# jopohl/urh

Measured on NVIDIA H100. Metric: MSamples/s IQ demod+digitize (complex64), higher is better.
Workload: dtype f32

## Files before the change

### urh_b200/csrc/center.cu

```cuda
#include "dense.cuh"
#include "tilescan.cuh"

#include <math.h>
#include <stdlib.h>

int urh_window_var_bitwise(urh_ctx* ctx, const float* d_x, int64_t n, const int64_t* d_prefix, int64_t t0, int64_t t1, int64_t r0,
                           int64_t r1, float* h_out2);

struct CenStats {
    double sum, sumsq;
    float mn, mx;
    long long cnt;
};

__global__ void __launch_bounds__(URH_WARPS_PER_BLOCK * 32)
k_tile_stats_f32(const float* __restrict__ x, int64_t n, int64_t ntiles, UrhTileStats* __restrict__ ts) {
    const int lane = threadIdx.x & 31;
    const int64_t tile = (int64_t)blockIdx.x * URH_WARPS_PER_BLOCK + (threadIdx.x >> 5);
    if (tile >= ntiles) return;
    const int64_t base = tile * URH_TILE;
    UrhStatAcc acc;
    acc.init();
    acc.all_noise = false;
    if (base + URH_TILE <= n && (((uintptr_t)x) & 15) == 0) {
        const float4* p = (const float4*)(x + base) + lane;
        constexpr int ITERS = URH_TILE / 128;
        float4 cur[4], nxt[4];
#pragma unroll
        for (int j = 0; j < 4; j++) cur[j] = __ldg(p + j * 32);
        for (int it = 0; it < ITERS; it += 4) {
            if (it + 4 < ITERS) {
#pragma unroll
                for (int j = 0; j < 4; j++) nxt[j] = __ldg(p + (it + 4 + j) * 32);
            }
#pragma unroll
            for (int j = 0; j < 4; j++) {
                acc.add(cur[j].x); acc.add(cur[j].y); acc.add(cur[j].z); acc.add(cur[j].w);
            }
#pragma unroll
            for (int j = 0; j < 4; j++) cur[j] = nxt[j];
        }
    } else {
        for (int j = lane; j < URH_TILE; j += 32)
            if (base + j < n) acc.add(x[base + j]);
    }
    acc.store(ts + tile, lane);
}

struct ScanKept {
    const UrhTileStats* ts;
    int64_t* prefix;
    __device__ __forceinline__ int64_t load(int64_t t) const { return ts[t].cnt; }
    __device__ __forceinline__ void post(int64_t t, const int64_t& excl, const int64_t&) const { prefix[t] = excl; }
};
struct CenAddI64 {
    __device__ __forceinline__ int64_t operator()(int64_t a, int64_t b) const { return a + b; }
};

static int kept_prefix(urh_ctx* ctx, const UrhTileStats* ts, int64_t ntiles, int64_t* prefix) {
    ScanKept fk;
    fk.ts = ts; fk.prefix = prefix;
    return urhts::scan<int64_t, CenAddI64, ScanKept>(ctx, ntiles, (int64_t)0, CenAddI64(), fk, prefix + ntiles);
}

__global__ void k_find_window_tiles(const int64_t* __restrict__ prefix, int64_t ntiles, int64_t r0, int64_t r1, int64_t* __restrict__ win) {
    const int64_t t = (int64_t)blockIdx.x * blockDim.x + threadIdx.x;
    if (t >= ntiles) return;
    const int64_t a = prefix[t], b = prefix[t + 1];
    if (b <= a) return;
    const bool covered = a >= r0 && b <= r1;
    const bool has_r0 = a <= r0 && r0 < b, has_r1 = a <= r1 - 1 && r1 - 1 < b;
    if (has_r0) { win[0] = t; win[2] = covered ? -1 : t; }
    if (has_r1) { win[1] = t; win[3] = (covered || has_r0) ? -1 : t; }
}

#define CEN_PER (URH_TILE / 256)
__device__ __forceinline__ int64_t cen_tile_ranks(const float* __restrict__ x, int64_t n, int64_t t, int64_t tile_rank0, float (&v)[CEN_PER],
                                                  int* s_pre) {
    const int64_t base = t * URH_TILE + (int64_t)threadIdx.x * CEN_PER;
    int mine = 0;
#pragma unroll
    for (int j = 0; j < CEN_PER; j++) {
        v[j] = (base + j < n) ? x[base + j] : -5.0f;
        mine += (v[j] > -4.0f) ? 1 : 0;
    }
    s_pre[threadIdx.x] = mine;
    __syncthreads();
    for (int off = 1; off < 256; off <<= 1) {
        int add = 0;
        if (threadIdx.x >= off) add = s_pre[threadIdx.x - off];
        __syncthreads();
        s_pre[threadIdx.x] += add;
        __syncthreads();
    }
    return tile_rank0 + s_pre[threadIdx.x] - mine;
}

__device__ __forceinline__ void cen_block_fold(double sum, double sq, float mn, float mx, long long cnt, CenStats* out) {
    __shared__ double s_sum[256], s_sq[256];
    __shared__ float s_mn[256], s_mx[256];
    __shared__ long long s_cnt[256];
    __syncthreads();
    s_sum[threadIdx.x] = sum; s_sq[threadIdx.x] = sq; s_mn[threadIdx.x] = mn; s_mx[threadIdx.x] = mx; s_cnt[threadIdx.x] = cnt;
    __syncthreads();
    for (int off = 128; off > 0; off >>= 1) {
        if (threadIdx.x < off) {
            s_sum[threadIdx.x] += s_sum[threadIdx.x + off];
            s_sq[threadIdx.x] += s_sq[threadIdx.x + off];
            s_mn[threadIdx.x] = fminf(s_mn[threadIdx.x], s_mn[threadIdx.x + off]);
            s_mx[threadIdx.x] = fmaxf(s_mx[threadIdx.x], s_mx[threadIdx.x + off]);
            s_cnt[threadIdx.x] += s_cnt[threadIdx.x + off];
        }
        __syncthreads();
    }
    if (threadIdx.x == 0) {
        CenStats r;
        r.sum = s_sum[0]; r.sumsq = s_sq[0]; r.mn = s_mn[0]; r.mx = s_mx[0]; r.cnt = s_cnt[0];
        *out = r;
    }
}

__global__ void __launch_bounds__(256) k_cut_tile_stats(const float* __restrict__ x, int64_t n, const int64_t* __restrict__ prefix,
                                                       const int64_t* __restrict__ win, int64_t r0, int64_t r1, CenStats* __restrict__ out) {
    __shared__ int s_pre[256];
    const int64_t t = win[2 + blockIdx.x];
    double sum = 0.0, sq = 0.0;
    float mn = INFINITY, mx = -INFINITY;
    long long cnt = 0;
    if (t >= 0) {
        float v[CEN_PER];
        int64_t rank = cen_tile_ranks(x, n, t, prefix[t], v, s_pre);
#pragma unroll
        for (int j = 0; j < CEN_PER; j++) {
            if (v[j] > -4.0f) {
                if (rank >= r0 && rank < r1) {
                    sum += (double)v[j];
                    sq += (double)v[j] * (double)v[j];
                    mn = fminf(mn, v[j]);
                    mx = fmaxf(mx, v[j]);
                    cnt++;
                }
                rank++;
            }
        }
    }
    cen_block_fold(sum, sq, mn, mx, cnt, out + blockIdx.x);
}

__global__ void __launch_bounds__(256) k_interior_tile_stats(const UrhTileStats* __restrict__ ts, const int64_t* __restrict__ prefix,
                                                            int64_t ntiles, int64_t r0, int64_t r1, CenStats* __restrict__ partial) {
    double sum = 0.0, sq = 0.0;
    float mn = INFINITY, mx = -INFINITY;
    long long cnt = 0;
    for (int64_t t = (int64_t)blockIdx.x * 256 + threadIdx.x; t < ntiles; t += (int64_t)gridDim.x * 256) {
        const int64_t a = prefix[t], b = prefix[t + 1];
        if (b > a && a >= r0 && b <= r1) {
            const UrhTileStats v = ts[t];
            sum += v.sum; sq += v.sumsq; mn = fminf(mn, v.mn); mx = fmaxf(mx, v.mx); cnt += v.cnt;
        }
    }
    cen_block_fold(sum, sq, mn, mx, cnt, partial + blockIdx.x);
}

__global__ void __launch_bounds__(256) k_center_fold(const CenStats* __restrict__ partial, int64_t count, CenStats* __restrict__ out) {
    double sum = 0.0, sq = 0.0;
    float mn = INFINITY, mx = -INFINITY;
    long long cnt = 0;
    for (int64_t t = threadIdx.x; t < count; t += 256) {
        const CenStats p = partial[t];
        sum += p.sum; sq += p.sumsq; mn = fminf(mn, p.mn); mx = fmaxf(mx, p.mx); cnt += p.cnt;
    }
    cen_block_fold(sum, sq, mn, mx, cnt, out);
}

int urh_center_tiles_begin(urh_ctx* ctx, const float* d_x, const UrhTileStats* ts, int64_t n, int64_t* h_total) {
    const int64_t ntiles = urh_div_up(n, URH_TILE);
    int64_t* prefix;
    URH_CHECK(urh_arena(ctx, (size_t)ntiles + 1, &prefix));
    URH_CHECK(kept_prefix(ctx, ts, ntiles, prefix));
    URH_CHECK(urh_read_i64(ctx, prefix + ntiles, 1, h_total));
    ctx->center_prefix = prefix;
    ctx->center_ts = ts;
    ctx->center_n = n;
    ctx->center_x = d_x;
    return URH_OK;
}

static int tiles_from_array(urh_ctx* ctx, const float* d_x, int64_t n, int64_t* h_total) {
    urh_arena_reset(ctx);
    ctx->center_prefix = nullptr;
    const int64_t ntiles = urh_div_up(n, URH_TILE);
    UrhTileStats* ts;
    URH_CHECK(urh_arena(ctx, (size_t)ntiles, &ts));
    URH_LAUNCH(ctx, k_tile_stats_f32, (unsigned)urh_div_up(ntiles, URH_WARPS_PER_BLOCK), URH_WARPS_PER_BLOCK * 32, 0, d_x, n, ntiles, ts);
    return urh_center_tiles_begin(ctx, d_x, ts, n, h_total);
}

static bool tiles_match(const urh_ctx* ctx, const float* d_x, int64_t n) {
    return ctx->center_prefix && ctx->center_n == n && ctx->center_x == (const void*)d_x;
}

extern "C" int urh_center_window_stats(urh_ctx* ctx, const float* d_qad, int64_t n, int64_t r0, int64_t r1, double* h_out5) {
    h_out5[0] = 0.0; h_out5[1] = INFINITY; h_out5[2] = -INFINITY; h_out5[3] = 0.0; h_out5[4] = 0.0;
    if (!tiles_match(ctx, d_qad, n)) URH_FAIL(ctx, URH_ERR_INVALID, "urh_afp_demod_tiles (same qad, same n) must precede urh_center_window_stats");
    if (r1 <= r0) return URH_OK;
    const int64_t ntiles = urh_div_up(n, URH_TILE);
    const int64_t* prefix = (const int64_t*)ctx->center_prefix;
    const UrhTileStats* ts = (const UrhTileStats*)ctx->center_ts;
    int64_t* d_win;
    CenStats* partial;
    CenStats* folded;
    const int nb = ctx->sm_count * 2;
    URH_CHECK(urh_arena(ctx, 4, &d_win));
    URH_CHECK(urh_arena(ctx, (size_t)nb + 4, &partial));
    URH_CHECK(urh_arena(ctx, 2, &folded));
    URH_CUDA(ctx, cudaMemsetAsync(d_win, 0xff, 4 * sizeof(int64_t), ctx->stream));
    URH_LAUNCH(ctx, k_find_window_tiles, (unsigned)urh_div_up(ntiles, 256), 256, 0, prefix, ntiles, r0, r1, d_win);
    URH_LAUNCH(ctx, k_interior_tile_stats, nb, 256, 0, ts, prefix, ntiles, r0, r1, partial);
    URH_LAUNCH(ctx, k_cut_tile_stats, 2, 256, 0, d_qad, n, prefix, d_win, r0, r1, partial + nb);
    URH_LAUNCH(ctx, k_center_fold, 1, 256, 0, partial, (int64_t)nb + 2, folded);
    CenStats st;
    URH_CUDA(ctx, cudaMemcpyAsync(ctx->h_mail, folded, sizeof(CenStats), cudaMemcpyDeviceToHost, ctx->stream));
    URH_CUDA(ctx, cudaStreamSynchronize(ctx->stream));
    memcpy(&st, ctx->h_mail, sizeof(st));
    h_out5[0] = (double)st.cnt; h_out5[1] = (double)st.mn; h_out5[2] = (double)st.mx; h_out5[3] = st.sum; h_out5[4] = st.sumsq;
    return URH_OK;
}

extern "C" int urh_center_window_var(urh_ctx* ctx, const float* d_qad, int64_t n, int64_t r0, int64_t r1, double* h_out2) {
    h_out2[0] = h_out2[1] = 0.0;
    if (!tiles_match(ctx, d_qad, n)) URH_FAIL(ctx, URH_ERR_INVALID, "the tile table of this array must precede urh_center_window_var");
    if (r1 <= r0) return URH_OK;
    float mv[2];
    URH_CHECK(urh_window_var_bitwise(ctx, d_qad, n, (const int64_t*)ctx->center_prefix, 0, urh_div_up(n, URH_TILE) - 1, r0, r1, mv));
    h_out2[0] = (double)mv[0];
    h_out2[1] = (double)mv[1];
    return URH_OK;
}

extern "C" int urh_center_stats(urh_ctx* ctx, const float* d_x, int64_t n, int64_t max_size, double* h_out) {
    for (int i = 0; i < 7; i++) h_out[i] = 0.0;
    if (n <= 0) return URH_OK;
    int64_t total = 0;
    URH_CHECK(tiles_from_array(ctx, d_x, n, &total));
    int64_t r0 = (int64_t)(0.05 * (double)total), r1 = (int64_t)(0.95 * (double)total);
    if (max_size >= 0 && r1 - r0 > max_size) r1 = r0 + max_size;
    h_out[0] = (double)total; h_out[1] = (double)r0; h_out[2] = (double)r1;
    if (r1 <= r0) return URH_OK;
    double w[5];
    URH_CHECK(urh_center_window_stats(ctx, d_x, n, r0, r1, w));
    if (w[0] <= 0.0) return URH_OK;
    h_out[3] = w[1]; h_out[4] = w[2];
    float mv[2];
    URH_CHECK(urh_window_var_bitwise(ctx, d_x, n, (const int64_t*)ctx->center_prefix, 0, urh_div_up(n, URH_TILE) - 1, r0, r1, mv));
    h_out[5] = (double)mv[0];
    h_out[6] = (double)mv[1];
    return URH_OK;
}

__global__ void k_hist_edges(double hmin, double hstep, int64_t nbins, float* __restrict__ fe) {
    const int64_t k = (int64_t)blockIdx.x * blockDim.x + threadIdx.x;
    if (k <= nbins) fe[k] = __double2float_ru(__dadd_rn(hmin, __dmul_rn((double)k, hstep)));
    if (k == nbins) {
        fe[nbins + 1] = __double2float_rd(__dadd_rn(hmin, __dmul_rn((double)nbins, hstep)));
        fe[nbins + 2] = fmaxf(__double2float_ru(hmin), nextafterf(-4.0f, 0.0f));
    }
}

struct HistBins {
    const float* fe;
    float f_min, f_hi, scale, off;
    int nbins;
    __device__ __forceinline__ void load(const float* fe_, float scale_, int nbins_) {
        fe = fe_; nbins = nbins_; scale = scale_;
        f_hi = fe[nbins + 1];
        f_min = fe[nbins + 2];
        off = -fe[0] * scale;
    }
    template <bool FAST>
    __device__ __forceinline__ int bin_of(float f) const {
        const bool valid = f >= f_min && f <= f_hi;
        if (FAST) {
            const float t = fmaf(f, scale, off);
            int r = __float_as_int(t + 12582912.0f) - 0x4B400000;
            r = max(0, min(r, nbins));
            int k = r - ((f < fe[r]) ? 1 : 0);
            k = min(k, nbins - 1);
            return valid ? k : -1;
        }
        if (!valid) return -1;
        int k = (int)((f - fe[0]) * scale);
        k = max(0, min(k, nbins - 1));
        while (k > 0 && f < fe[k]) k--;
        while (k < nbins - 1 && f >= fe[k + 1]) k++;
        return k;
    }
};

struct HistCache {
    float lo0, hi0, lo1, hi1, lo2, hi2, lo3, hi3;
    int h0, h1, h2, h3;
    unsigned c0, c1, c2, c3;
    __device__ __forceinline__ void init() {
        lo0 = lo1 = lo2 = lo3 = INFINITY;
        hi0 = hi1 = hi2 = hi3 = -INFINITY;
        h0 = h1 = h2 = h3 = 0;
        c0 = c1 = c2 = c3 = 0u;
    }
};

template <bool SMEM>
__device__ __forceinline__ void hist_bump(unsigned int* s_hist, unsigned long long* hist, int k, unsigned c) {
    if (SMEM) atomicAdd(&s_hist[k], c);
    else atomicAdd(&hist[k], (unsigned long long)c);
}

template <bool SMEM, bool FAST>
__device__ __forceinline__ void hist_miss(HistCache& hc, const HistBins& hb, unsigned int* s_hist, unsigned long long* hist, float f) {
    const int k = hb.bin_of<FAST>(f);
    if (k < 0) return;
    const float lo = fmaxf(hb.fe[k], hb.f_min);
    const float hi = (k == hb.nbins - 1) ? nextafterf(hb.f_hi, INFINITY) : hb.fe[k + 1];
    unsigned cm = hc.c0; int which = 0;
    if (hc.c1 < cm) { cm = hc.c1; which = 1; }
    if (hc.c2 < cm) { cm = hc.c2; which = 2; }
    if (hc.c3 < cm) { cm = hc.c3; which = 3; }
    const int old = which == 0 ? hc.h0 : which == 1 ? hc.h1 : which == 2 ? hc.h2 : hc.h3;
    if (cm) hist_bump<SMEM>(s_hist, hist, old, cm);
    if (which == 0) { hc.h0 = k; hc.c0 = 1u; hc.lo0 = lo; hc.hi0 = hi; }
    else if (which == 1) { hc.h1 = k; hc.c1 = 1u; hc.lo1 = lo; hc.hi1 = hi; }
    else if (which == 2) { hc.h2 = k; hc.c2 = 1u; hc.lo2 = lo; hc.hi2 = hi; }
    else { hc.h3 = k; hc.c3 = 1u; hc.lo3 = lo; hc.hi3 = hi; }
}

template <bool SMEM, bool FAST>
__device__ __forceinline__ void hist_put(HistCache& hc, const HistBins& hb, unsigned int* s_hist, unsigned long long* hist, float f,
                                         unsigned one) {
    unsigned miss;
    asm("{\n\t.reg .pred p0, p1, p2, p3, pv;\n\t"
        "setp.ge.f32 p0, %5, %6;\n\tsetp.lt.and.f32 p0, %5, %7, p0;\n\t@p0 mad.lo.u32 %0, %0, %15, %15;\n\t"
        "setp.ge.f32 p1, %5, %8;\n\tsetp.lt.and.f32 p1, %5, %9, p1;\n\t@p1 mad.lo.u32 %1, %1, %15, %15;\n\t"
        "setp.ge.f32 p2, %5, %10;\n\tsetp.lt.and.f32 p2, %5, %11, p2;\n\t@p2 mad.lo.u32 %2, %2, %15, %15;\n\t"
        "setp.ge.f32 p3, %5, %12;\n\tsetp.lt.and.f32 p3, %5, %13, p3;\n\t@p3 mad.lo.u32 %3, %3, %15, %15;\n\t"
        "or.pred p0, p0, p1;\n\tor.pred p2, p2, p3;\n\tor.pred p0, p0, p2;\n\t"
        "setp.ge.f32 pv, %5, %14;\n\t"
        "and.pred pv, pv, !p0;\n\t"
        "selp.u32 %4, 1, 0, pv;\n\t}"
        : "+r"(hc.c0), "+r"(hc.c1), "+r"(hc.c2), "+r"(hc.c3), "=r"(miss)
        : "f"(f), "f"(hc.lo0), "f"(hc.hi0), "f"(hc.lo1), "f"(hc.hi1), "f"(hc.lo2), "f"(hc.hi2), "f"(hc.lo3), "f"(hc.hi3),
          "f"(hb.f_min), "r"(one));
    if (miss) hist_miss<SMEM, FAST>(hc, hb, s_hist, hist, f);
}

template <bool SMEM>
__device__ __forceinline__ void hist_flush(HistCache& hc, unsigned int* s_hist, unsigned long long* hist) {
    if (hc.c0) hist_bump<SMEM>(s_hist, hist, hc.h0, hc.c0);
    if (hc.c1) hist_bump<SMEM>(s_hist, hist, hc.h1, hc.c1);
    if (hc.c2) hist_bump<SMEM>(s_hist, hist, hc.h2, hc.c2);
    if (hc.c3) hist_bump<SMEM>(s_hist, hist, hc.h3, hc.c3);
}

template <bool SMEM, bool FAST>
__device__ __forceinline__ void hist_interior_body(const float* __restrict__ x, int64_t n, int64_t t_first, int64_t t_end, int blk, int nblk,
                                                   const float* __restrict__ g_fe, float scale, int nbins,
                                                   unsigned long long* __restrict__ hist, int edges_in_smem,
                                                   const int64_t* __restrict__ prefix) {
    extern __shared__ unsigned int s_dyn[];
    unsigned int* s_hist = s_dyn;
    float* s_fe = (float*)(s_dyn + (SMEM ? nbins : 0));
    const int lane = threadIdx.x & 31;
    if (SMEM)
        for (int b = threadIdx.x; b < nbins; b += 256) s_hist[b] = 0u;
    if (edges_in_smem)
        for (int b = threadIdx.x; b < nbins + 3; b += 256) s_fe[b] = g_fe[b];
    __syncthreads();
    HistBins hb;
    if (FAST) hb.load(s_fe, scale, nbins);
    else hb.load(edges_in_smem ? s_fe : g_fe, scale, nbins);
    HistCache hc;
    hc.init();
    const int64_t gw = (int64_t)blk * 8 + (threadIdx.x >> 5), nw = (int64_t)nblk * 8;
    const bool vec = (((uintptr_t)x) & 15) == 0;
    const unsigned one = blockDim.x >> 8;
    {
        for (int64_t t = t_first + gw; t < t_end; t += nw) {
            if (prefix[t + 1] == prefix[t]) continue;
            const int64_t base = t * URH_TILE;
            if (vec) {
                const float4* p = (const float4*)(x + base) + lane;
                constexpr int ITERS = URH_TILE / 128, DEPTH = 4;
                float4 buf[DEPTH];
#pragma unroll
                for (int j = 0; j < DEPTH; j++) buf[j] = __ldg(p + j * 32);
#pragma unroll 1
                for (int it = 0; it < ITERS; it += DEPTH) {
                    const bool more = it + DEPTH < ITERS;
#pragma unroll
                    for (int j = 0; j < DEPTH; j++) {
                        const float4 v = buf[j];
                        if (more) buf[j] = __ldg(p + (it + DEPTH + j) * 32);
                        hist_put<SMEM, FAST>(hc, hb, s_hist, hist, v.x, one);
                        hist_put<SMEM, FAST>(hc, hb, s_hist, hist, v.y, one);
                        hist_put<SMEM, FAST>(hc, hb, s_hist, hist, v.z, one);
                        hist_put<SMEM, FAST>(hc, hb, s_hist, hist, v.w, one);
                    }
                }
            } else {
                for (int j = lane; j < URH_TILE; j += 32) hist_put<SMEM, FAST>(hc, hb, s_hist, hist, x[base + j], one);
            }
        }
    }
    hist_flush<SMEM>(hc, s_hist, hist);
    if (SMEM) {
        __syncthreads();
        for (int b = threadIdx.x; b < nbins; b += 256)
            if (s_hist[b]) atomicAdd(&hist[b], (unsigned long long)s_hist[b]);
    }
}

template <bool SMEM, bool FAST>
__global__ void __launch_bounds__(256, 4) k_hist_interior(const float* __restrict__ x, int64_t n, const int64_t* __restrict__ win,
                                                      const float* __restrict__ g_fe, float scale, int nbins,
                                                      unsigned long long* __restrict__ hist, int edges_in_smem,
                                                      const int64_t* __restrict__ prefix) {
    const int64_t w0 = win[0];
    hist_interior_body<SMEM, FAST>(x, n, w0 + 1, w0 >= 0 ? win[1] : 0, blockIdx.x, gridDim.x, g_fe, scale, nbins, hist, edges_in_smem, prefix);
}

__device__ __forceinline__ void hist_window_ends_body(const float* __restrict__ x, int64_t n, const int64_t* __restrict__ prefix,
                                                      const int64_t* __restrict__ win, int64_t r0, int64_t r1,
                                                      const float* __restrict__ g_fe, float scale, int nbins,
                                                      unsigned long long* __restrict__ hist, unsigned long long* __restrict__ hist2 = nullptr) {
    __shared__ int s_pre[256];
    const int64_t t = win[blockIdx.x];
    if (t < 0 || (blockIdx.x == 1 && t == win[0])) return;
    HistBins hb;
    hb.load(g_fe, scale, nbins);
    float v[CEN_PER];
    int64_t rank = cen_tile_ranks(x, n, t, prefix[t], v, s_pre);
#pragma unroll
    for (int j = 0; j < CEN_PER; j++) {
        const bool kept = v[j] > -4.0f;
        const int k = hb.bin_of<false>(v[j]);
        if (k >= 0 && rank >= r0 && rank < r1) {
            atomicAdd(&hist[k], 1ull);
            if (hist2) atomicAdd(&hist2[k], 1ull);
        }
        rank += kept ? 1 : 0;
    }
}

__global__ void __launch_bounds__(256) k_hist_window_ends(const float* __restrict__ x, int64_t n, const int64_t* __restrict__ prefix,
                                                         const int64_t* __restrict__ win, int64_t r0, int64_t r1,
                                                         const float* __restrict__ g_fe, float scale, int nbins,
                                                         unsigned long long* __restrict__ hist) {
    hist_window_ends_body(x, n, prefix, win, r0, r1, g_fe, scale, nbins, hist);
}

extern "C" int urh_center_histogram_tiles(urh_ctx* ctx, const float* d_qad, int64_t n, int64_t r0, int64_t r1, double hmin,
                                          double hstep, int64_t nbins, int64_t* h_hist) {
    if (nbins <= 0) return URH_OK;
    if (!tiles_match(ctx, d_qad, n)) URH_FAIL(ctx, URH_ERR_INVALID, "urh_afp_demod_tiles (same qad, same n) must precede urh_center_histogram_tiles");
    if (nbins > (int64_t)1 << 30) URH_FAIL(ctx, URH_ERR_INVALID, "too many histogram bins");
    const int64_t ntiles = urh_div_up(n, URH_TILE);
    const int64_t* prefix = (const int64_t*)ctx->center_prefix;
    unsigned long long* hist;
    float* fe;
    int64_t* d_win;
    URH_CHECK(urh_arena(ctx, (size_t)nbins, &hist));
    URH_CHECK(urh_arena(ctx, (size_t)nbins + 3, &fe));
    URH_CHECK(urh_arena(ctx, 4, &d_win));
    URH_CUDA(ctx, cudaMemsetAsync(hist, 0, (size_t)nbins * sizeof(unsigned long long), ctx->stream));
    URH_CUDA(ctx, cudaMemsetAsync(d_win, 0xff, 4 * sizeof(int64_t), ctx->stream));
    if (r1 > r0) {
        URH_LAUNCH(ctx, k_hist_edges, (unsigned)urh_div_up(nbins + 1, 256), 256, 0, hmin, hstep, nbins, fe);
        URH_LAUNCH(ctx, k_find_window_tiles, (unsigned)urh_div_up(ntiles, 256), 256, 0, prefix, ntiles, r0, r1, d_win);
        const bool in_smem = nbins <= 12000;
        const int edges_smem = (in_smem && nbins <= 6000) ? 1 : 0;
        const size_t dyn = (in_smem ? (size_t)nbins * 4 : 0) + (edges_smem ? (size_t)(nbins + 3) * 4 : 0);
        const float scale = (float)(1.0 / hstep);
        const double edge_abs = fmax(fabs(hmin), fabs(hmin + (double)nbins * hstep));
        const bool fast = edges_smem && hstep > 0.0 && edge_abs / hstep < 1048576.0;
        const unsigned gs = (unsigned)min(urh_div_up(ntiles, 8), (int64_t)ctx->sm_count * 8);
        const int64_t* cw = d_win;
        const float* cfe = fe;
        if (in_smem && fast) URH_LAUNCH(ctx, (k_hist_interior<true, true>), gs, 256, dyn, d_qad, n, cw, cfe, scale, (int)nbins, hist, edges_smem, prefix);
        else if (in_smem) URH_LAUNCH(ctx, (k_hist_interior<true, false>), gs, 256, dyn, d_qad, n, cw, cfe, scale, (int)nbins, hist, edges_smem, prefix);
        else URH_LAUNCH(ctx, (k_hist_interior<false, false>), gs, 256, dyn, d_qad, n, cw, cfe, scale, (int)nbins, hist, edges_smem, prefix);
        URH_LAUNCH(ctx, k_hist_window_ends, 2, 256, 0, d_qad, n, prefix, (const int64_t*)d_win, r0, r1, (const float*)fe, scale, (int)nbins, hist);
    }
    URH_CUDA(ctx, cudaMemcpyAsync(h_hist, hist, (size_t)nbins * sizeof(int64_t), cudaMemcpyDeviceToHost, ctx->stream));
    URH_CUDA(ctx, cudaStreamSynchronize(ctx->stream));
    return URH_OK;
}

extern "C" int urh_center_histogram(urh_ctx* ctx, const float* d_x, int64_t n, int64_t r0, int64_t r1, double hmin,
                                    double hstep, int64_t nbins, int64_t* h_hist) {
    if (nbins <= 0 || n <= 0) return URH_OK;
    if (!tiles_match(ctx, d_x, n)) {
        int64_t total = 0;
        URH_CHECK(tiles_from_array(ctx, d_x, n, &total));
    }
    return urh_center_histogram_tiles(ctx, d_x, n, r0, r1, hmin, hstep, nbins, h_hist);
}

#define CEN_MAX_BINS 6000
#define CEN_VAR_MIN_RATIO 0x1p-14

struct __align__(16) CenterPlan {
    long long total, offset;
    long long r0, r1;
    long long lr0, lr1;
    long long win[4];
    CenStats local;
    double hmin, edge1, delta;
    long long nbins;
    double center;
    float centerf;
    float scale;
    int fast;
    int state;
    unsigned int ticket;
    int certified;
    long long straddle;
    long long pad;
};

__global__ void k_center_ranks(const int64_t* __restrict__ counts, int rank, int world, int64_t max_size, CenterPlan* __restrict__ plan) {
    long long total = 0, offset = 0;
    for (int q = 0; q < world; q++) {
        if (q < rank) offset += counts[q];
        total += counts[q];
    }
    const long long kept = counts[rank];
    long long r0 = (long long)(0.05 * (double)total), r1 = (long long)(0.95 * (double)total);
    if (max_size >= 0 && r1 - r0 > max_size) r1 = r0 + max_size;
    plan->total = total; plan->offset = offset; plan->r0 = r0; plan->r1 = r1;
    long long a = r0 - offset, b = r1 - offset;
    a = a < 0 ? 0 : (a > kept ? kept : a);
    b = b < 0 ? 0 : (b > kept ? kept : b);
    plan->lr0 = a; plan->lr1 = b;
    plan->ticket = 0u;
    plan->state = 1;
    plan->certified = 0;
    plan->straddle = 0;
}

__device__ __forceinline__ int64_t cen_tile_of_rank(const int64_t* __restrict__ prefix, int64_t ntiles, int64_t r) {
    int64_t lo = 0, hi = ntiles;
    while (hi - lo > 1) {
        const int64_t mid = (lo + hi) >> 1;
        if (prefix[mid] <= r) lo = mid; else hi = mid;
    }
    return lo;
}

__global__ void __launch_bounds__(256) k_center_window(const float* __restrict__ x, int64_t n, const UrhTileStats* __restrict__ ts,
                                                      const int64_t* __restrict__ prefix, int64_t ntiles, CenterPlan* __restrict__ plan,
                                                      CenStats* __restrict__ partial) {
    __shared__ long long s_win[4];
    __shared__ int s_pre[256];
    __shared__ bool s_last;
    const long long r0 = plan->lr0, r1 = plan->lr1;
    if (threadIdx.x == 0) {
        long long w0 = -1, w1 = -1, w2 = -1, w3 = -1;
        if (r1 > r0) {
            w0 = cen_tile_of_rank(prefix, ntiles, r0);
            w1 = cen_tile_of_rank(prefix, ntiles, r1 - 1);
            const bool cov0 = prefix[w0] >= r0 && prefix[w0 + 1] <= r1;
            const bool cov1 = prefix[w1] >= r0 && prefix[w1 + 1] <= r1;
            w2 = cov0 ? -1 : w0;
            w3 = (cov1 || w1 == w0) ? -1 : w1;
        }
        s_win[0] = w0; s_win[1] = w1; s_win[2] = w2; s_win[3] = w3;
        if (blockIdx.x == 0) { plan->win[0] = w0; plan->win[1] = w1; plan->win[2] = w2; plan->win[3] = w3; }
    }
    __syncthreads();
    double sum = 0.0, sq = 0.0;
    float mn = INFINITY, mx = -INFINITY;
    long long cnt = 0;
    if (s_win[0] >= 0) {
        for (int64_t t = s_win[0] + (int64_t)blockIdx.x * 256 + threadIdx.x; t <= s_win[1]; t += (int64_t)gridDim.x * 256) {
            const int64_t a = prefix[t], b = prefix[t + 1];
            if (b > a && a >= r0 && b <= r1) {
                const UrhTileStats v = ts[t];
                sum += v.sum; sq += v.sumsq; mn = fminf(mn, v.mn); mx = fmaxf(mx, v.mx); cnt += v.cnt;
            }
        }
    }
    cen_block_fold(sum, sq, mn, mx, cnt, partial + blockIdx.x);
    if (blockIdx.x < 2) {
        const int64_t t = s_win[2 + blockIdx.x];
        sum = 0.0; sq = 0.0; mn = INFINITY; mx = -INFINITY; cnt = 0;
        if (t >= 0) {
            float v[CEN_PER];
            int64_t rank = cen_tile_ranks(x, n, t, prefix[t], v, s_pre);
#pragma unroll
            for (int j = 0; j < CEN_PER; j++) {
                if (v[j] > -4.0f) {
                    if (rank >= r0 && rank < r1) {
                        sum += (double)v[j];
                        sq += (double)v[j] * (double)v[j];
                        mn = fminf(mn, v[j]);
                        mx = fmaxf(mx, v[j]);
                        cnt++;
                    }
                    rank++;
                }
            }
        }
        cen_block_fold(sum, sq, mn, mx, cnt, partial + gridDim.x + blockIdx.x);
    }
    __threadfence();
    __syncthreads();
    if (threadIdx.x == 0) s_last = atomicAdd(&plan->ticket, 1u) == gridDim.x - 1;
    __syncthreads();
    if (!s_last) return;
    __threadfence();
    sum = 0.0; sq = 0.0; mn = INFINITY; mx = -INFINITY; cnt = 0;
    for (int64_t t = threadIdx.x; t < (int64_t)gridDim.x + 2; t += 256) {
        CenStats p;
        {
            const int4* src = (const int4*)(partial + t);
            int4 w0 = __ldcg(src), w1 = __ldcg(src + 1);
            memcpy(&p, &w0, 16);
            memcpy((char*)&p + 16, &w1, 16);
        }
        sum += p.sum; sq += p.sumsq; mn = fminf(mn, p.mn); mx = fmaxf(mx, p.mx); cnt += p.cnt;
    }
    cen_block_fold(sum, sq, mn, mx, cnt, &plan->local);
}

__global__ void __launch_bounds__(256) k_center_plan(const CenStats* __restrict__ parts, int world, CenterPlan* __restrict__ plan,
                                                    float* __restrict__ fe, unsigned long long* __restrict__ hist,
                                                    unsigned long long* __restrict__ xhist) {
    __shared__ int s_state;
    __shared__ long long s_nbins;
    __shared__ double s_hmin, s_edge1, s_delta;
    if (threadIdx.x == 0) {
        double cnt = 0.0, sum = 0.0, sq = 0.0;
        float mn = INFINITY, mx = -INFINITY;
        for (int q = 0; q < world; q++) {
            cnt += (double)parts[q].cnt;
            mn = fminf(mn, parts[q].mn);
            mx = fmaxf(mx, parts[q].mx);
            sum = __dadd_rn(sum, parts[q].sum);
            sq = __dadd_rn(sq, parts[q].sumsq);
        }
        int state = 0;
        long long nbins = 0;
        double hmin = 0.0, edge1 = 0.0, delta = 0.0;
        if (plan->r1 > plan->r0 && cnt > 0.0) {
            const double mean = __ddiv_rn(sum, cnt);
            double ss = __dsub_rn(sq, __dmul_rn(__dmul_rn(cnt, mean), mean));
            if (ss < 0.0) ss = 0.0;
            const double var = __ddiv_rn(ss, cnt);
            const double hstep = (double)__double2float_rn(var);
            hmin = (double)mn;
            const double stop = __dadd_rn((double)mx, hstep);
            if (!(var >= __dmul_rn(__dmul_rn(mean, mean), CEN_VAR_MIN_RATIO))) state = 2;
            else if (hstep != 0.0) {
                const double val = __ddiv_rn(__dsub_rn(stop, hmin), hstep);
                if (val == val && fabs(val) < 9.0e18) {
                    const long long len = (long long)ceil(val);
                    if (len >= 2) {
                        nbins = len - 1;
                        edge1 = __dadd_rn(hmin, hstep);
                        delta = __dsub_rn(edge1, hmin);
                        state = (nbins <= CEN_MAX_BINS && delta > 0.0) ? 1 : 2;
                    }
                }
            }
        }
        plan->hmin = hmin; plan->edge1 = edge1; plan->delta = delta; plan->nbins = nbins;
        plan->state = state;
        plan->center = 0.0; plan->centerf = 0.0f;
        if (state == 1) {
            plan->scale = (float)(1.0 / delta);
            const double edge_abs = fmax(fabs(hmin), fabs(hmin + (double)nbins * delta));
            plan->fast = (edge_abs / delta < 1048576.0) ? 1 : 0;
        }
        s_state = state; s_nbins = nbins; s_hmin = hmin; s_edge1 = edge1; s_delta = delta;
    }
    __syncthreads();
    if (s_state != 1) return;
    const long long nbins = s_nbins;
    for (long long k = threadIdx.x; k <= nbins; k += 256) {
        const double e = (k == 0) ? s_hmin : (k == 1 ? s_edge1 : __dadd_rn(s_hmin, __dmul_rn((double)k, s_delta)));
        fe[k] = __double2float_ru(e);
        if (k == nbins) {
            fe[nbins + 1] = __double2float_rd(e);
            fe[nbins + 2] = fmaxf(__double2float_ru(s_hmin), nextafterf(-4.0f, 0.0f));
        }
        if (k < nbins) {
            hist[k] = 0ull;
            if (xhist) xhist[k] = 0ull;
        }
    }
}

template <bool FAST>
__global__ void __launch_bounds__(256, 3) k_hist_interior_dev(const float* __restrict__ x, int64_t n, const CenterPlan* __restrict__ plan,
                                                          const float* __restrict__ g_fe, unsigned long long* __restrict__ hist,
                                                          const int64_t* __restrict__ prefix) {
    if (plan->state != 1 || plan->certified || (plan->fast != 0) != FAST) return;
    hist_interior_body<true, FAST>(x, n, plan->win[0] + 1, plan->win[1], blockIdx.x, gridDim.x, g_fe, plan->scale, (int)plan->nbins, hist, 1,
                                   prefix);
}

__device__ __forceinline__ void cen_full_slabs(int64_t win0, int64_t win1, int64_t slab_tiles, int64_t* sf, int64_t* se) {
    *sf = (win0 + slab_tiles) / slab_tiles;
    *se = win1 / slab_tiles;
}

__global__ void __launch_bounds__(256) k_hist_window_ends_dev(const float* __restrict__ x, int64_t n, const int64_t* __restrict__ prefix,
                                                             const CenterPlan* __restrict__ plan, const float* __restrict__ g_fe,
                                                             unsigned long long* __restrict__ hist, unsigned long long* __restrict__ xhist,
                                                             int64_t slab_tiles) {
    if (plan->state != 1) return;
    if (blockIdx.x < 2) {
        hist_window_ends_body(x, n, prefix, (const int64_t*)plan->win, plan->lr0, plan->lr1, g_fe, plan->scale, (int)plan->nbins, hist, xhist);
        return;
    }
    const int64_t w0 = plan->win[0], w1 = plan->win[1];
    int64_t sf, se;
    cen_full_slabs(w0, w1, slab_tiles, &sf, &se);
    int64_t a_end = w1, b_begin = w1;
    if (sf < se) { a_end = sf * slab_tiles; b_begin = se * slab_tiles; }
    const int blk = blockIdx.x - 2, nblk = gridDim.x - 2, nbins = (int)plan->nbins;
    const float scale = plan->scale;
    if (plan->fast) {
        hist_interior_body<true, true>(x, n, w0 + 1, a_end, blk, nblk, g_fe, scale, nbins, xhist, 1, prefix);
        hist_interior_body<true, true>(x, n, b_begin, w1, blk, nblk, g_fe, scale, nbins, xhist, 1, prefix);
    } else {
        hist_interior_body<true, false>(x, n, w0 + 1, a_end, blk, nblk, g_fe, scale, nbins, xhist, 1, prefix);
        hist_interior_body<true, false>(x, n, b_begin, w1, blk, nblk, g_fe, scale, nbins, xhist, 1, prefix);
    }
}

__device__ __forceinline__ double cen_left_edge(const CenterPlan* plan, int k) {
    return (k == 0) ? plan->hmin : (k == 1 ? plan->edge1 : __dadd_rn(plan->hmin, __dmul_rn((double)k, plan->delta)));
}

#define CERT_THREADS 512
__global__ void __launch_bounds__(CERT_THREADS) k_center_certify(const UrhFine fine, CenterPlan* __restrict__ plan, const float* __restrict__ fe,
                                                                 const unsigned long long* __restrict__ xhist, unsigned long long* __restrict__ lo,
                                                                 unsigned long long* __restrict__ hi) {
    __shared__ unsigned long long s_ge[URH_FINE_NB + 1];
    __shared__ unsigned long long s_part[CERT_THREADS];
    __shared__ unsigned char s_flag[CEN_MAX_BINS];
    __shared__ unsigned long long s_key[3];
    __shared__ unsigned int s_certain;
    if (plan->state != 1) return;
    const int tid = threadIdx.x;
    constexpr int PER = URH_FINE_NB / CERT_THREADS;
    int64_t sf, se;
    cen_full_slabs(plan->win[0], plan->win[1], fine.slab_tiles, &sf, &se);
    unsigned long long b[PER], tot = 0;
#pragma unroll
    for (int j = 0; j < PER; j++) {
        unsigned long long v = 0;
        for (int64_t sl = sf; sl < se; sl++) v += fine.gh[sl * URH_FINE_NB + tid * PER + j];
        b[j] = v;
        tot += v;
    }
    s_part[tid] = tot;
    if (tid < 3) s_key[tid] = 0ull;
    if (tid == 0) s_certain = 0u;
    __syncthreads();
    for (int off = 1; off < CERT_THREADS; off <<= 1) {
        const unsigned long long add = (tid + off < CERT_THREADS) ? s_part[tid + off] : 0ull;
        __syncthreads();
        s_part[tid] += add;
        __syncthreads();
    }
    unsigned long long run = (tid + 1 < CERT_THREADS) ? s_part[tid + 1] : 0ull;
#pragma unroll
    for (int j = PER - 1; j >= 0; j--) {
        run += b[j];
        s_ge[tid * PER + j] = run;
    }
    if (tid == 0) s_ge[URH_FINE_NB] = 0ull;
    __syncthreads();
    const int nbins = (int)plan->nbins;
    const float f_hi = fe[nbins + 1], f_min = fe[nbins + 2], top = nextafterf(f_hi, INFINITY);
    auto ge = [&](float t, unsigned long long& glo, unsigned long long& ghi) {
        const int bt = urh_fine_bucket(t, fine.scale, fine.off);
        const bool straddles = urh_fine_bucket(nextafterf(t, -INFINITY), fine.scale, fine.off) == bt;
        ghi = s_ge[bt];
        glo = straddles ? s_ge[bt + 1] : s_ge[bt];
    };
    for (int k = tid; k < nbins; k += CERT_THREADS) {
        const float a = fmaxf(fe[k], f_min), e = (k == nbins - 1) ? top : fminf(fe[k + 1], top);
        unsigned long long l = 0, u = 0;
        if (a < e) {
            unsigned long long alo, ahi, elo, ehi;
            ge(a, alo, ahi);
            ge(e, elo, ehi);
            l = alo > ehi ? alo - ehi : 0ull;
            u = ahi - elo;
        }
        lo[k] = xhist[k] + l;
        hi[k] = xhist[k] + u;
    }
    __syncthreads();
    int window = (int)(0.05 * (double)nbins) + 1;
    if (window < 2) window = 2;
    for (int k = tid; k < nbins; k += CERT_THREADS) {
        const unsigned long long l = lo[k], u = hi[k];
        bool certain = l > 0ull, possible = u > 0ull;
        for (int d = -(window - 1); d < window && (certain || possible); d++) {
            const int j = k + d;
            if (d == 0 || j < 0 || j >= nbins) continue;
            certain = certain && l > hi[j];
            possible = possible && u > lo[j];
        }
        s_flag[k] = certain ? 1 : (possible ? 2 : 0);
        if (certain) atomicAdd(&s_certain, 1u);
    }
    __syncthreads();
    for (int pass = 0; pass < 3; pass++) {
        const long long p0 = pass > 0 ? (long long)(8191 - (s_key[0] & 8191)) : -1, p1 = pass > 1 ? (long long)(8191 - (s_key[1] & 8191)) : -1;
        for (int k = tid; k < nbins; k += CERT_THREADS) {
            if (k == p0 || k == p1) continue;
            if (pass < 2 && s_flag[k] == 1) atomicMax(&s_key[pass], (lo[k] << 13) | (unsigned long long)(8191 - k));
            if (pass == 2 && s_flag[k] != 0) atomicMax(&s_key[2], hi[k]);
        }
        __syncthreads();
    }
    if (tid != 0 || s_certain < 2u) return;
    const int k1 = 8191 - (int)(s_key[0] & 8191), k2 = 8191 - (int)(s_key[1] & 8191);
    plan->straddle = (long long)((hi[k1] - lo[k1]) + (hi[k2] - lo[k2]));
    if (!(lo[k2] > s_key[2])) return;
    const double c = __ddiv_rn(__dadd_rn(cen_left_edge(plan, k1), cen_left_edge(plan, k2)), 2.0);
    plan->center = c;
    plan->centerf = __double2float_rn(c);
    plan->certified = 1;
}

__global__ void __launch_bounds__(256) k_center_pick(const unsigned long long* __restrict__ y, CenterPlan* __restrict__ plan) {
    __shared__ unsigned long long s_best[256];
    __shared__ int s_idx[256];
    __shared__ int s_cnt[256];
    if (plan->state != 1 || plan->certified) return;
    const int nbins = (int)plan->nbins;
    int window = (int)(0.05 * (double)nbins) + 1;
    if (window < 2) window = 2;
    unsigned long long top_val[2] = {0ull, 0ull};
    int top_idx[2] = {-1, -1};
    int found = 0;
    bool undecided = false;
    for (int pass = 0; pass < 2 && !undecided; pass++) {
        unsigned long long best = 0ull;
        int bi = -1, ties = 0;
        for (int i = threadIdx.x; i < nbins; i += 256) {
            if (pass == 1 && i == top_idx[0]) continue;
            const unsigned long long v = y[i];
            if (v == 0ull || v < best) continue;
            bool peak = true;
            for (int d = 1; d < window && peak; d++) {
                const unsigned long long a = (i + d < nbins) ? y[i + d] : 0ull;
                const unsigned long long b = (i - d >= 0) ? y[i - d] : 0ull;
                peak = v > a && v > b;
            }
            if (!peak) continue;
            if (v > best) { best = v; bi = i; ties = 1; }
            else ties++;
        }
        s_best[threadIdx.x] = best; s_idx[threadIdx.x] = bi; s_cnt[threadIdx.x] = ties;
        __syncthreads();
        if (threadIdx.x == 0) {
            unsigned long long b = 0ull;
            int idx = -1, t = 0;
            for (int j = 0; j < 256; j++) {
                if (s_idx[j] < 0) continue;
                if (s_best[j] > b) { b = s_best[j]; idx = s_idx[j]; t = s_cnt[j]; }
                else if (s_best[j] == b) t += s_cnt[j];
            }
            s_best[0] = b; s_idx[0] = idx; s_cnt[0] = t;
        }
        __syncthreads();
        const unsigned long long b = s_best[0];
        const int idx = s_idx[0], t = s_cnt[0];
        __syncthreads();
        if (idx < 0) break;
        if (pass == 0) {
            top_val[0] = b; top_idx[0] = idx; found = 1;
            if (t == 2) {
                int other = -1;
                for (int i = threadIdx.x; i < nbins; i += 256) {
                    if (i == idx || y[i] != b) continue;
                    bool peak = true;
                    for (int d = 1; d < window && peak; d++) {
                        const unsigned long long a = (i + d < nbins) ? y[i + d] : 0ull;
                        const unsigned long long c = (i - d >= 0) ? y[i - d] : 0ull;
                        peak = b > a && b > c;
                    }
                    if (peak) other = i;
                }
                s_idx[threadIdx.x] = other;
                __syncthreads();
                if (threadIdx.x == 0) {
                    int o = -1;
                    for (int j = 0; j < 256; j++) if (s_idx[j] >= 0) o = s_idx[j];
                    s_idx[0] = o;
                }
                __syncthreads();
                top_idx[1] = s_idx[0]; top_val[1] = b; found = 2;
                __syncthreads();
                break;
            }
            if (t > 2) undecided = true;
        } else {
            if (t > 1) undecided = true;
            else { top_val[1] = b; top_idx[1] = idx; found = 2; }
        }
    }
    if (threadIdx.x != 0) return;
    if (undecided) { plan->state = 2; return; }
    if (found == 0) { plan->state = 0; return; }
    double c;
    if (found == 1) c = cen_left_edge(plan, top_idx[0]);
    else c = __ddiv_rn(__dadd_rn(cen_left_edge(plan, top_idx[0]), cen_left_edge(plan, top_idx[1])), 2.0);
    plan->center = c;
    plan->centerf = __double2float_rn(c);
    plan->state = 1;
    (void)top_val;
}

int urh_center_chain(urh_ctx* ctx, const float* d_qad, int64_t n, const UrhTileStats* ts, int64_t max_size, int rank, int world,
                     const UrhFine* fine, CenterPlan** d_plan_out) {
    const int64_t ntiles = urh_div_up(n, URH_TILE);
    int64_t* prefix;
    CenterPlan* plan;
    CenStats* partial;
    float* fe;
    unsigned long long* hist;
    int64_t* d_counts;
    CenStats* d_parts;
    unsigned long long *xhist = nullptr, *cert_lo = nullptr, *cert_hi = nullptr;
    const int nb = ctx->sm_count * 2;
    URH_CHECK(urh_arena(ctx, (size_t)ntiles + 1, &prefix));
    URH_CHECK(urh_arena(ctx, 1, &plan));
    URH_CHECK(urh_arena(ctx, (size_t)nb + 2, &partial));
    URH_CHECK(urh_arena(ctx, (size_t)CEN_MAX_BINS + 3, &fe));
    URH_CHECK(urh_arena(ctx, (size_t)CEN_MAX_BINS, &hist));
    URH_CHECK(urh_arena(ctx, (size_t)world, &d_counts));
    URH_CHECK(urh_arena(ctx, (size_t)world, &d_parts));
    if (fine) {
        URH_CHECK(urh_arena(ctx, (size_t)CEN_MAX_BINS, &xhist));
        URH_CHECK(urh_arena(ctx, (size_t)CEN_MAX_BINS, &cert_lo));
        URH_CHECK(urh_arena(ctx, (size_t)CEN_MAX_BINS, &cert_hi));
    }
    URH_CHECK(kept_prefix(ctx, ts, ntiles, prefix));
    const int64_t* counts = prefix + ntiles;
    if (world > 1) {
        URH_TL_MARK(ctx, "x1 kept counts: enter");
        URH_CHECK(urh_nccl_allgather(ctx, prefix + ntiles, d_counts, sizeof(int64_t)));
        URH_TL_MARK(ctx, "x1 kept counts: done");
        counts = d_counts;
    }
    URH_LAUNCH(ctx, k_center_ranks, 1, 1, 0, counts, rank, world, max_size, plan);
    URH_LAUNCH(ctx, k_center_window, nb, 256, 0, d_qad, n, ts, (const int64_t*)prefix, ntiles, plan, partial);
    const CenStats* parts = &plan->local;
    if (world > 1) {
        URH_TL_MARK(ctx, "x2 window partials: enter");
        URH_CHECK(urh_nccl_allgather(ctx, &plan->local, d_parts, sizeof(CenStats)));
        URH_TL_MARK(ctx, "x2 window partials: done");
        parts = d_parts;
    }
    URH_LAUNCH(ctx, k_center_plan, 1, 256, 0, parts, world, plan, fe, hist, xhist);
    const size_t dyn = (size_t)CEN_MAX_BINS * 4 + (size_t)(CEN_MAX_BINS + 3) * 4;
    const unsigned gs = (unsigned)min(urh_div_up(ntiles, 8), (int64_t)ctx->sm_count * 8);
    URH_LAUNCH(ctx, k_hist_window_ends_dev, fine ? 2 + ctx->sm_count * 4 : 2, 256, fine ? dyn : 0, d_qad, n, (const int64_t*)prefix,
               (const CenterPlan*)plan, (const float*)fe, hist, xhist, fine ? fine->slab_tiles : (int64_t)1);
    if (fine) URH_LAUNCH(ctx, k_center_certify, 1, CERT_THREADS, 0, *fine, plan, (const float*)fe, (const unsigned long long*)xhist, cert_lo, cert_hi);
    URH_LAUNCH(ctx, (k_hist_interior_dev<true>), gs, 256, dyn, d_qad, n, (const CenterPlan*)plan, (const float*)fe, hist, (const int64_t*)prefix);
    URH_LAUNCH(ctx, (k_hist_interior_dev<false>), gs, 256, dyn, d_qad, n, (const CenterPlan*)plan, (const float*)fe, hist, (const int64_t*)prefix);
    if (world > 1) {
        URH_TL_MARK(ctx, "x3 histogram sum: enter");
        URH_CHECK(urh_nccl_allreduce_i64(ctx, (int64_t*)hist, CEN_MAX_BINS, 0));
        URH_TL_MARK(ctx, "x3 histogram sum: done");
    }
    URH_LAUNCH(ctx, k_center_pick, 1, 256, 0, (const unsigned long long*)hist, plan);
    ctx->center_prefix = prefix;
    ctx->center_ts = ts;
    ctx->center_n = n;
    ctx->center_x = d_qad;
    *d_plan_out = plan;
    return URH_OK;
}

int urh_center_plan_certify_stats(urh_ctx* ctx, const CenterPlan* plan, int64_t* h_dst3) {
    h_dst3[0] = h_dst3[1] = h_dst3[2] = 0;
    URH_CUDA(ctx, cudaMemcpyAsync(h_dst3, &plan->certified, sizeof(int), cudaMemcpyDeviceToHost, ctx->stream));
    URH_CUDA(ctx, cudaMemcpyAsync(h_dst3 + 2, &plan->straddle, sizeof(long long), cudaMemcpyDeviceToHost, ctx->stream));
    return URH_OK;
}

extern "C" int urh_center_certify_stats(urh_ctx* ctx, int64_t* h_out3) {
    for (int i = 0; i < 3; i++) h_out3[i] = ctx->center_cert[i];
    return URH_OK;
}

int urh_center_plan_result(urh_ctx* ctx, const CenterPlan* plan, const float** d_centerf, const double** d_center, const int** d_state) {
    if (d_centerf) *d_centerf = &plan->centerf;
    if (d_center) *d_center = &plan->center;
    if (d_state) *d_state = &plan->state;
    return URH_OK;
}
```

### urh_b200/csrc/digitize.cu

```cuda
#include "dense.cuh"
#include "tilescan.cuh"
#include "sparse.cuh"
#include "fsk_fast.cuh"
#include "dense_f32.cuh"
#include "stream_ring.cuh"

#include <math.h>
#include <stdlib.h>


template <int DT, int MOD, bool DIGITIZE>
__device__ __forceinline__ void dense_iq_tile(const void* __restrict__ iq, int64_t n, const UrhDemodParams& dp, float* __restrict__ qad_out,
                                              int vec_in, int vec_out, const UrhClassify& cls, int tol, UrhTileSummary* __restrict__ tiles,
                                              uint32_t* __restrict__ staging, int stage_cap, int16_t* __restrict__ init_cls, int cls_of_zero,
                                              int64_t tile, int has_halo, UrhTileStats* __restrict__ tile_stats, const UrhFine& fine,
                                              unsigned int* s_fine, unsigned int* g_fine) {
    const int lane = threadIdx.x & 31;
    const int64_t tile_start = tile * URH_TILE;
    const int tile_len = (int)((n - tile_start) < URH_TILE ? (n - tile_start) : URH_TILE);
    const int iters = (tile_len + 63) >> 6;

    UrhRunTracker rt;
    if (DIGITIZE) rt.init(tol, staging + tile * (int64_t)stage_cap);
    UrhStatAcc acc;
    acc.init();

    float cA = 0.0f, cB = 0.0f;
    if (MOD == URH_MOD_FSK && (tile_start > 0 || has_halo) && lane == 0) {
        typedef typename UrhElem<DT>::type E;
        const E* pp = (const E*)iq + 2 * (tile_start - 1);
        const UrhFskTerms t = urh_fsk_terms((float)pp[0], (float)pp[1]);
        cA = t.A; cB = t.B;
    }

    UrhPair cur = urh_load_pair<DT>(iq, tile_start + 2 * lane, n, vec_in != 0);
    for (int it = 0; it < iters; it++) {
        const int64_t pos0 = tile_start + (int64_t)it * 64 + 2 * lane;
        UrhPair nxt;
        if (it + 1 < iters) nxt = urh_load_pair<DT>(iq, pos0 + 64, n, vec_in != 0);

        const float m0 = __fadd_rn(__fmul_rn(cur.r0, cur.r0), __fmul_rn(cur.i0, cur.i0));
        const float m1 = __fadd_rn(__fmul_rn(cur.r1, cur.r1), __fmul_rn(cur.i1, cur.i1));
        float s0 = dp.noise_value, s1 = dp.noise_value;
        if (MOD == URH_MOD_FSK) {
            const UrhFskTerms t0 = urh_fsk_terms(cur.r0, cur.i0);
            const UrhFskTerms t1 = urh_fsk_terms(cur.r1, cur.i1);
            float pA = __shfl_up_sync(URH_FULL_MASK, t1.A, 1);
            float pB = __shfl_up_sync(URH_FULL_MASK, t1.B, 1);
            if (lane == 0) { pA = cA; pB = cB; }
            cA = __shfl_sync(URH_FULL_MASK, t1.A, 31);
            cB = __shfl_sync(URH_FULL_MASK, t1.B, 31);
            if (!(m0 <= dp.noise_sqrd)) s0 = urh_fsk_angle(pA, pB, t0.C, t0.D);
            if (!(m1 <= dp.noise_sqrd)) s1 = urh_fsk_angle(t0.A, t0.B, t1.C, t1.D);
        } else if (MOD == URH_MOD_ASK) {
            if (!(m0 <= dp.noise_sqrd)) s0 = __fdiv_rn(__fsqrt_rn(m0), dp.max_mag);
            if (!(m1 <= dp.noise_sqrd)) s1 = __fdiv_rn(__fsqrt_rn(m1), dp.max_mag);
        }
        if (pos0 == 0 && !has_halo) s0 = dp.noise_value;

        const bool v0 = pos0 < n, v1 = pos0 + 1 < n;
        if (tile_stats) {
            if (v0) { acc.add(s0); acc.all_noise = acc.all_noise && (s0 == dp.noise_value); }
            if (v1) { acc.add(s1); acc.all_noise = acc.all_noise && (s1 == dp.noise_value); }
            if (s_fine) {
                if (v0) urh_fine_add(s0, fine, s_fine, g_fine);
                if (v1) urh_fine_add(s1, fine, s_fine, g_fine);
            }
        }
        if (qad_out) {
            if (v1 && vec_out) urh_stg_f2(qad_out + pos0, s0, s1);
            else {
                if (v0) qad_out[pos0] = s0;
                if (v1) qad_out[pos0 + 1] = s1;
            }
        }
        if (DIGITIZE) {
            const int c0 = urh_classify(s0, cls), c1 = urh_classify(s1, cls);
            if (pos0 == 0) *init_cls = (int16_t)((s0 == cls.noise_value) ? -1 : cls_of_zero);
            rt.feed(it, c0, c1, v0, v1, lane);
        }
        cur = nxt;
    }
    if (tile_stats) acc.store(tile_stats + tile, lane);
    if (DIGITIZE) rt.finish(tile_len, tiles + tile, lane);
}

template <int DT, int MOD, bool DIGITIZE>
__global__ void __launch_bounds__(URH_WARPS_PER_BLOCK * 32)
k_dense_iq(const void* __restrict__ iq, int64_t n, UrhDemodParams dp, float* __restrict__ qad_out, int vec_in,
           int vec_out, const __grid_constant__ UrhClassify cls, int tol, UrhTileSummary* __restrict__ tiles,
           uint32_t* __restrict__ staging, int stage_cap, int16_t* __restrict__ init_cls, int cls_of_zero,
           int64_t tile_begin, int64_t tile_count, int has_halo, UrhTileStats* __restrict__ tile_stats, const UrhFine fine) {
    extern __shared__ unsigned int s_fine[];
    const int64_t tile_rel = (int64_t)blockIdx.x * URH_WARPS_PER_BLOCK + (threadIdx.x >> 5);
    const int64_t block_tile0 = tile_begin + (int64_t)blockIdx.x * URH_WARPS_PER_BLOCK;
    if (fine.gh) urh_fine_zero(s_fine);
    if (tile_rel < tile_count && (tile_begin + tile_rel) * URH_TILE < n)
        dense_iq_tile<DT, MOD, DIGITIZE>(iq, n, dp, qad_out, vec_in, vec_out, cls, tol, tiles, staging, stage_cap, init_cls, cls_of_zero,
                                    tile_begin + tile_rel, has_halo, tile_stats, fine,
                                    fine.gh ? s_fine : nullptr, fine.gh ? urh_fine_row(fine, tile_begin + tile_rel, block_tile0) : nullptr);
    if (fine.gh) urh_fine_flush(fine, s_fine, block_tile0);
}

template <int DT, bool DIGITIZE, bool WRITE, bool STATS>
__global__ void __launch_bounds__(URH_WARPS_PER_BLOCK * 32, (DT == URH_DT_F32) ? 5 : 4)
k_fsk_fifo(const void* __restrict__ iq, int64_t n, UrhDemodParams dp, float* __restrict__ qad_out, float thr0,
           float cls_noise, int tol, UrhTileSummary* __restrict__ tiles, uint32_t* __restrict__ staging, int stage_cap,
           int64_t tile_begin, int64_t tile_count, UrhTileStats* __restrict__ tile_stats, const UrhFine fine,
           const float* __restrict__ d_thr0 = nullptr, float* __restrict__ margin = nullptr) {
    __shared__ __align__(16) unsigned char s_fifo[URH_WARPS_PER_BLOCK][URH_FSK_FIFO + 1][64 * 2 * sizeof(typename UrhElem<DT>::type)];
    extern __shared__ unsigned int s_fine[];
    const bool fine_on = STATS && fine.gh;
    if (DIGITIZE && STATS) thr0 = *d_thr0;
    const int lane = threadIdx.x & 31;
    const int64_t tile_rel = (int64_t)blockIdx.x * URH_WARPS_PER_BLOCK + (threadIdx.x >> 5);
    const int64_t block_tile0 = tile_begin + (int64_t)blockIdx.x * URH_WARPS_PER_BLOCK;
    if (fine_on) urh_fine_zero(s_fine);
    if (tile_rel < tile_count) {
        const int64_t tile = tile_begin + tile_rel;
        UrhRunTracker rt;
        if (DIGITIZE) rt.init(tol, staging + tile * (int64_t)stage_cap);
        UrhOne one;
        one.p = dp.one;
        one.m = dp.mone;
        const uint32_t fifo = (uint32_t)__cvta_generic_to_shared(&s_fifo[threadIdx.x >> 5][0][0]);
        urh_fsk_full_tile<DT, DIGITIZE, WRITE, STATS>(iq, n, tile * URH_TILE, dp, qad_out, thr0, cls_noise, rt, lane, one,
                                                      STATS ? tile_stats + tile : nullptr, fifo, DIGITIZE ? tiles + tile : nullptr, fine,
                                                      fine_on ? s_fine : nullptr, fine_on ? urh_fine_row(fine, tile, block_tile0) : nullptr,
                                                      (DIGITIZE && STATS) ? margin + tile : nullptr);
    }
    if (fine_on) urh_fine_flush(fine, s_fine, block_tile0);
}

#define URH_GUESS_SAMPLES 16384
#define URH_GUESS_BINS 128
#define URH_GUESS_THREADS 1024
__global__ void __launch_bounds__(URH_GUESS_THREADS) k_speculate_guess(const float2* __restrict__ iq, int64_t n, float noise_sqrd, int forced,
                                                                      float forced_tg, float* __restrict__ d_tg, unsigned int* __restrict__ redone) {
    constexpr int PER = URH_GUESS_SAMPLES / URH_GUESS_THREADS;
    __shared__ unsigned int s_hist[URH_GUESS_BINS];
    __shared__ float s_mn[32], s_mx[32];
    if (forced) {
        if (threadIdx.x == 0) { *d_tg = forced_tg; *redone = 0u; }
        return;
    }
    for (int b = threadIdx.x; b < URH_GUESS_BINS; b += blockDim.x) s_hist[b] = 0u;
    float v[PER];
    float mn = INFINITY, mx = -INFINITY;
#pragma unroll
    for (int k = 0; k < PER; k++) {
        const int64_t i = 1 + (int64_t)(k * URH_GUESS_THREADS + threadIdx.x) * (n - 1) / URH_GUESS_SAMPLES;
        const float2 p = iq[i - 1], c = iq[i];
        v[k] = NAN;
        if (!(c.x * c.x + c.y * c.y <= noise_sqrd)) {
            v[k] = atan2f(p.x * c.y - p.y * c.x, p.x * c.x + p.y * c.y);
            mn = fminf(mn, v[k]);
            mx = fmaxf(mx, v[k]);
        }
    }
    for (int off = 16; off > 0; off >>= 1) {
        mn = fminf(mn, __shfl_xor_sync(URH_FULL_MASK, mn, off));
        mx = fmaxf(mx, __shfl_xor_sync(URH_FULL_MASK, mx, off));
    }
    if ((threadIdx.x & 31) == 0) { s_mn[threadIdx.x >> 5] = mn; s_mx[threadIdx.x >> 5] = mx; }
    __syncthreads();
    mn = INFINITY; mx = -INFINITY;
    for (int w = 0; w < URH_GUESS_THREADS / 32; w++) { mn = fminf(mn, s_mn[w]); mx = fmaxf(mx, s_mx[w]); }
    const float width = (mx - mn) / URH_GUESS_BINS;
    if (width > 0.0f) {
#pragma unroll
        for (int k = 0; k < PER; k++)
            if (!isnan(v[k])) atomicAdd(&s_hist[min((int)((v[k] - mn) / width), URH_GUESS_BINS - 1)], 1u);
    }
    __syncthreads();
    if (threadIdx.x != 0) return;
    *redone = 0u;
    if (!(mn <= mx)) { *d_tg = 0.0f; return; }
    if (!(width > 0.0f)) { *d_tg = mn; return; }
    constexpr int WINDOW = (int)(0.05 * URH_GUESS_BINS) + 1;
    int top[2] = {-1, -1};
    for (int b = 0; b < URH_GUESS_BINS; b++) {
        const unsigned int y = s_hist[b];
        bool peak = y > 0u;
        for (int d = 1; d < WINDOW && peak; d++)
            peak = y > (b + d < URH_GUESS_BINS ? s_hist[b + d] : 0u) && y > (b - d >= 0 ? s_hist[b - d] : 0u);
        if (!peak) continue;
        if (top[0] < 0 || y > s_hist[top[0]]) { top[1] = top[0]; top[0] = b; }
        else if (top[1] < 0 || y > s_hist[top[1]]) top[1] = b;
    }
    if (top[0] < 0) *d_tg = 0.5f * (mn + mx);
    else if (top[1] < 0) *d_tg = mn + ((float)top[0] + 0.5f) * width;
    else *d_tg = mn + (0.5f * (float)(top[0] + top[1]) + 0.5f) * width;
}


extern "C" int urh_get_center_thresholds(float center, float spacing, int modulation_order, float* h_out) {
    const int n = modulation_order / 2;
    for (int i = 0; i < n; i++) {
        volatile float t = (float)(n - (i + 1)) * spacing;
        h_out[i] = center - t;
    }
    for (int i = n; i < modulation_order - 1; i++) {
        volatile float t = (float)(i + 1 - n) * spacing;
        h_out[i] = center + t;
    }
    return URH_OK;
}

static int fill_classify(urh_ctx* ctx, UrhClassify* C, int mod_type, float center, uint8_t bits_per_symbol,
                         float spacing) {
    if (bits_per_symbol > 8) URH_FAIL(ctx, URH_ERR_INVALID, "bits_per_symbol %d > 8 not supported", (int)bits_per_symbol);
    memset(C, 0, sizeof(*C));
    C->noise_value = urh_noise_value(mod_type);
    C->order = 1 << bits_per_symbol;
    if (C->order > 1) urh_get_center_thresholds(center, spacing, C->order, C->thr);
    return URH_OK;
}

static int host_classify(float s, const UrhClassify& C) {
    int c = C.order - 1;
    for (int k = 0; k < C.order - 1; k++)
        if (s <= C.thr[k]) { c = k; break; }
    return c;
}

static float max_magnitude_for(int dtype) {
    switch (dtype) {
        case URH_DT_I8: return (float)sqrt(127.0 * 127.0 + 128.0 * 128.0);
        case URH_DT_U8: return (float)sqrt(255.0 * 255.0);
        case URH_DT_I16: return (float)sqrt(32768.0 * 32768.0 + 32767.0 * 32767.0);
        case URH_DT_U16: return (float)sqrt(65535.0 * 65535.0);
        default: return (float)sqrt(2.0);
    }
}

static bool iq_vec_aligned(const void* p, int dtype) { return ((uintptr_t)p % (2 * (size_t)urh_iq_bytes(dtype))) == 0; }

template <int DT, int MOD, bool DIG>
static int launch_dense_iq_t(urh_ctx* ctx, const void* d_iq, int64_t n, const UrhDemodParams& dp, float* d_qad,
                             const UrhClassify& cls, int tol, UrhTileSummary* tiles, uint32_t* staging,
                             int stage_cap, int16_t* init_cls, int cls_of_zero, int has_halo = 0,
                             UrhTileStats* tile_stats = nullptr, int64_t tile_lo = 0, int64_t tile_hi = -1,
                             const UrhFine& fine = UrhFine{}, UrhSpec* spec = nullptr) {
    const int64_t ntiles = urh_div_up(n, URH_TILE);
    const size_t fine_smem = fine.gh ? (size_t)URH_FINE_NB * sizeof(unsigned int) : 0;
    if (tile_hi < 0 || tile_hi > ntiles) tile_hi = ntiles;
    const int vec_in = iq_vec_aligned(d_iq, DT) ? 1 : 0;
    const int vec_out = (d_qad && ((uintptr_t)d_qad % 8) == 0) ? 1 : 0;
    const int threads = URH_WARPS_PER_BLOCK * 32;
    auto generic = [&](int64_t begin, int64_t end) -> int {
        begin = begin < tile_lo ? tile_lo : begin;
        end = end > tile_hi ? tile_hi : end;
        const int64_t count = end - begin;
        if (count <= 0) return URH_OK;
        URH_LAUNCH(ctx, (k_dense_iq<DT, MOD, DIG>), (unsigned)urh_div_up(count, URH_WARPS_PER_BLOCK), threads, fine_smem, d_iq, n, dp,
                   d_qad, vec_in, vec_out, cls, tol, tiles, staging, stage_cap, init_cls, cls_of_zero, begin, count, has_halo,
                   tile_stats, fine);
        return URH_OK;
    };
    const int64_t nfull = n / URH_TILE;
    const bool fast = MOD == URH_MOD_FSK && vec_in && (!d_qad || vec_out) && (!DIG || cls.order == 2) && nfull > 1;
    URH_PROF_BEGIN(ctx);
    if (fast) {
        const int64_t fb = tile_lo > 1 ? tile_lo : 1, fe = tile_hi < nfull ? tile_hi : nfull;
        if (fe > fb) {
            const unsigned grid = (unsigned)urh_div_up(fe - fb, URH_WARPS_PER_BLOCK);
            bool speculated = false;
            if constexpr (DT == URH_DT_F32 && MOD == URH_MOD_FSK && !DIG) {
                if (spec && tile_stats && d_qad) {
                    URH_LAUNCH(ctx, (k_fsk_fifo<DT, true, true, true>), grid, threads, fine_smem, d_iq, n, dp, d_qad, 0.0f, dp.noise_value,
                               tol, tiles, staging, stage_cap, fb, fe - fb, tile_stats, fine, (const float*)spec->tg, spec->margin);
                    spec->lo = fb;
                    spec->hi = fe;
                    speculated = true;
                }
            }
            if (speculated) {
            } else if (tile_stats && d_qad && !DIG) {
                URH_LAUNCH(ctx, (k_fsk_fifo<DT, false, true, true>), grid, threads, fine_smem, d_iq, n, dp, d_qad, cls.thr[0], cls.noise_value,
                           tol, tiles, staging, stage_cap, fb, fe - fb, tile_stats, fine);
            } else if (d_qad) {
                URH_LAUNCH(ctx, (k_fsk_fifo<DT, DIG, true, false>), grid, threads, 0, d_iq, n, dp, d_qad, cls.thr[0], cls.noise_value, tol,
                           tiles, staging, stage_cap, fb, fe - fb, nullptr, UrhFine{});
            } else {
                URH_LAUNCH(ctx, (k_fsk_fifo<DT, DIG, false, false>), grid, threads, 0, d_iq, n, dp, d_qad, cls.thr[0], cls.noise_value, tol,
                           tiles, staging, stage_cap, fb, fe - fb, nullptr, UrhFine{});
            }
        }
        URH_CHECK(generic(0, 1));
        URH_CHECK(generic(nfull, ntiles));
    } else {
        URH_CHECK(generic(0, ntiles));
    }
    URH_PROF_END(ctx);
    return URH_OK;
}

template <int MOD, bool DIG>
static int launch_dense_iq_m(urh_ctx* ctx, int dtype, const void* d_iq, int64_t n, const UrhDemodParams& dp,
                             float* d_qad, const UrhClassify& cls, int tol, UrhTileSummary* tiles,
                             uint32_t* staging, int stage_cap, int16_t* init_cls, int cls_of_zero, int has_halo = 0,
                             UrhTileStats* tile_stats = nullptr, int64_t tile_lo = 0, int64_t tile_hi = -1,
                             const UrhFine& fine = UrhFine{}, UrhSpec* spec = nullptr) {
    switch (dtype) {
        case URH_DT_I8: return launch_dense_iq_t<URH_DT_I8, MOD, DIG>(ctx, d_iq, n, dp, d_qad, cls, tol, tiles, staging, stage_cap, init_cls, cls_of_zero, has_halo, tile_stats, tile_lo, tile_hi, fine);
        case URH_DT_U8: return launch_dense_iq_t<URH_DT_U8, MOD, DIG>(ctx, d_iq, n, dp, d_qad, cls, tol, tiles, staging, stage_cap, init_cls, cls_of_zero, has_halo, tile_stats, tile_lo, tile_hi, fine);
        case URH_DT_I16: return launch_dense_iq_t<URH_DT_I16, MOD, DIG>(ctx, d_iq, n, dp, d_qad, cls, tol, tiles, staging, stage_cap, init_cls, cls_of_zero, has_halo, tile_stats, tile_lo, tile_hi, fine);
        case URH_DT_U16: return launch_dense_iq_t<URH_DT_U16, MOD, DIG>(ctx, d_iq, n, dp, d_qad, cls, tol, tiles, staging, stage_cap, init_cls, cls_of_zero, has_halo, tile_stats, tile_lo, tile_hi, fine);
        case URH_DT_F32: return launch_dense_iq_t<URH_DT_F32, MOD, DIG>(ctx, d_iq, n, dp, d_qad, cls, tol, tiles, staging, stage_cap, init_cls, cls_of_zero, has_halo, tile_stats, tile_lo, tile_hi, fine, spec);
        default: URH_FAIL(ctx, URH_ERR_DTYPE, "Unsupported dtype");
    }
}

int urh_costas_demod(urh_ctx* ctx, const void* d_iq, int dtype, int64_t n, float noise_sqrd, int loop_order,
                     float bandwidth, float* d_out);

static UrhDemodParams make_demod_params(float noise_mag, int mod_type, int dtype) {
    UrhDemodParams dp;
    volatile float nm = noise_mag;
    volatile float sq = nm * nm;
    dp.noise_sqrd = sq;
    dp.noise_value = urh_noise_value(mod_type);
    dp.max_mag = max_magnitude_for(dtype);
    dp.one = 1.0f;
    dp.mone = -1.0f;
    return dp;
}

extern "C" int urh_afp_demod(urh_ctx* ctx, const void* d_iq, int dtype, int64_t n, float noise_mag, int mod_type,
                             int mod_order, float costas_loop_bandwidth, float* d_out) {
    if (n < 0) URH_FAIL(ctx, URH_ERR_INVALID, "negative length");
    if (urh_iq_bytes(dtype) == 0) URH_FAIL(ctx, URH_ERR_DTYPE, "Unsupported dtype");
    if (n == 0) return URH_OK;
    if (n <= 2 || (mod_type != URH_MOD_ASK && mod_type != URH_MOD_FSK && mod_type != URH_MOD_PSK)) {
        URH_CUDA(ctx, cudaMemsetAsync(d_out, 0, (size_t)n * sizeof(float), ctx->stream));
        if (n > 2) {
            const float nv = urh_noise_value(mod_type);
            URH_CUDA(ctx, cudaMemcpyAsync(d_out, &nv, sizeof(float), cudaMemcpyHostToDevice, ctx->stream));
            URH_CUDA(ctx, cudaStreamSynchronize(ctx->stream));
        }
        return URH_OK;
    }
    const UrhDemodParams dp = make_demod_params(noise_mag, mod_type, dtype);
    if (mod_type == URH_MOD_PSK) return urh_costas_demod(ctx, d_iq, dtype, n, dp.noise_sqrd, mod_order, costas_loop_bandwidth, d_out);
    UrhClassify cls;
    memset(&cls, 0, sizeof(cls));
    if (mod_type == URH_MOD_ASK)
        return launch_dense_iq_m<URH_MOD_ASK, false>(ctx, dtype, d_iq, n, dp, d_out, cls, 0, nullptr, nullptr, 0, nullptr, 0);
    return launch_dense_iq_m<URH_MOD_FSK, false>(ctx, dtype, d_iq, n, dp, d_out, cls, 0, nullptr, nullptr, 0, nullptr, 0);
}

int urh_center_tiles_begin(urh_ctx* ctx, const float* d_x, const UrhTileStats* ts, int64_t n, int64_t* h_total);

extern "C" int urh_afp_demod_tiles(urh_ctx* ctx, const void* d_iq, int dtype, int64_t n, float noise_mag, int mod_type,
                                   float* d_qad_out, int halo, int64_t* h_kept) {
    if (n <= 2 || (mod_type != URH_MOD_ASK && mod_type != URH_MOD_FSK) || !d_qad_out)
        URH_FAIL(ctx, URH_ERR_INVALID, "urh_afp_demod_tiles: ASK/FSK, n > 2 and a qad buffer are required");
    if (urh_iq_bytes(dtype) == 0) URH_FAIL(ctx, URH_ERR_DTYPE, "Unsupported dtype");
    urh_arena_reset(ctx);
    const UrhDemodParams dp = make_demod_params(noise_mag, mod_type, dtype);
    UrhClassify cls;
    memset(&cls, 0, sizeof(cls));
    const int64_t ntiles = urh_div_up(n, URH_TILE);
    UrhTileStats* ts;
    URH_CHECK(urh_arena(ctx, (size_t)ntiles, &ts));
    if (mod_type == URH_MOD_ASK)
        URH_CHECK((launch_dense_iq_m<URH_MOD_ASK, false>(ctx, dtype, d_iq, n, dp, d_qad_out, cls, 0, nullptr, nullptr, 0, nullptr, 0, halo, ts)));
    else
        URH_CHECK((launch_dense_iq_m<URH_MOD_FSK, false>(ctx, dtype, d_iq, n, dp, d_qad_out, cls, 0, nullptr, nullptr, 0, nullptr, 0, halo, ts)));
    return urh_center_tiles_begin(ctx, d_qad_out, ts, n, h_kept);
}

int urh_finish_local(urh_ctx* ctx, int64_t n, int tol, bool is_ask, uint32_t sps, const UrhTileSummary* tiles, const uint32_t* staging,
                     int stage_cap, const int16_t* d_init, int64_t* k);
int urh_finish_shard(urh_ctx* ctx, int64_t n, int tol, bool is_ask, uint32_t sps, const UrhTileSummary* tiles, const uint32_t* staging,
                     int stage_cap, const int16_t* d_init, int64_t global_offset, int64_t n_total, int64_t* k);

static int stage_cap_for(int tol) { return URH_TILE / (tol + 1) + 2; }

static int digitizer_tables(urh_ctx* ctx, int64_t ntiles, int cap, UrhTileSummary** tiles, uint32_t** staging, int16_t** d_init) {
    URH_CHECK(urh_arena(ctx, (size_t)ntiles, tiles));
    URH_CHECK(urh_arena(ctx, (size_t)ntiles * cap, staging));
    return urh_arena(ctx, 8, d_init);
}

static int launch_dense_qad(urh_ctx* ctx, const float* x, int64_t n, const UrhClassify& cls, int tol, UrhTileSummary* tiles,
                            uint32_t* staging, int cap, int16_t* init, int c0, const float* d_thr0 = nullptr,
                            const UrhTileStats* ts = nullptr) {
    const unsigned grid = (unsigned)urh_div_up(urh_div_up(n, URH_TILE), URH_WARPS_PER_BLOCK);
    const int vec_in = (((uintptr_t)x % 8) == 0) ? 1 : 0;
    if (cls.order == 2)
        URH_LAUNCH(ctx, (k_dense_f32<SrcQad2, float>), grid, URH_WARPS_PER_BLOCK * 32, 0, x, n, vec_in, cls, tol, tiles, staging, cap, init,
                   c0, d_thr0, ts);
    else
        URH_LAUNCH(ctx, (k_dense_f32<SrcQad, float>), grid, URH_WARPS_PER_BLOCK * 32, 0, x, n, vec_in, cls, tol, tiles, staging, cap, init,
                   c0, d_thr0, ts);
    return URH_OK;
}

extern "C" int urh_grab_pulse_lens(urh_ctx* ctx, const float* d_qad, int64_t n, float center, uint16_t tolerance,
                                   int mod_type, uint32_t samples_per_symbol, uint8_t bits_per_symbol,
                                   float center_spacing, int64_t* k) {
    if (!k) return URH_ERR_INVALID;
    *k = 0;
    ctx->pulses_k = 0;
    if (n < 0) URH_FAIL(ctx, URH_ERR_INVALID, "negative length");
    if (n == 0) return URH_OK;
    urh_arena_reset(ctx);
    UrhClassify cls;
    URH_CHECK(fill_classify(ctx, &cls, mod_type, center, bits_per_symbol, center_spacing));
    const int tol = tolerance;
    const int64_t ntiles = urh_div_up(n, URH_TILE);
    const int cap = stage_cap_for(tol);
    UrhTileSummary* tiles;
    uint32_t* staging;
    int16_t* d_init;
    URH_CHECK(digitizer_tables(ctx, ntiles, cap, &tiles, &staging, &d_init));
    URH_PROF_BEGIN(ctx);
    URH_CHECK(launch_dense_qad(ctx, d_qad, n, cls, tol, tiles, staging, cap, d_init, host_classify(0.0f, cls)));
    URH_PROF_END(ctx);
    return urh_finish_local(ctx, n, tol, mod_type == URH_MOD_ASK, samples_per_symbol, tiles, staging, cap, d_init, k);
}

extern "C" int urh_demod_digitize(urh_ctx* ctx, const void* d_iq, int dtype, int64_t n, float noise_mag,
                                  int mod_type, float center, uint16_t tolerance, uint32_t samples_per_symbol,
                                  uint8_t bits_per_symbol, float center_spacing, float* d_qad_out, int64_t* k) {
    if (!k) return URH_ERR_INVALID;
    *k = 0;
    ctx->pulses_k = 0;
    if (n < 0) URH_FAIL(ctx, URH_ERR_INVALID, "negative length");
    if (urh_iq_bytes(dtype) == 0) URH_FAIL(ctx, URH_ERR_DTYPE, "Unsupported dtype");
    if (n == 0) return URH_OK;
    if (n <= 2 || (mod_type != URH_MOD_ASK && mod_type != URH_MOD_FSK)) {
        float* q = d_qad_out;
        if (!q) URH_CUDA(ctx, cudaMalloc((void**)&q, (size_t)n * sizeof(float)));
        int rc = urh_afp_demod(ctx, d_iq, dtype, n, noise_mag, mod_type, 1 << bits_per_symbol, 0.1f, q);
        if (rc == URH_OK)
            rc = urh_grab_pulse_lens(ctx, q, n, center, tolerance, mod_type, samples_per_symbol, bits_per_symbol,
                                     center_spacing, k);
        if (!d_qad_out) {
            cudaStreamSynchronize(ctx->stream);
            cudaFree(q);
        }
        return rc;
    }
    urh_arena_reset(ctx);
    UrhClassify cls;
    URH_CHECK(fill_classify(ctx, &cls, mod_type, center, bits_per_symbol, center_spacing));
    const UrhDemodParams dp = make_demod_params(noise_mag, mod_type, dtype);
    const int tol = tolerance;
    const int64_t ntiles = urh_div_up(n, URH_TILE);
    const int cap = stage_cap_for(tol);
    UrhTileSummary* tiles;
    uint32_t* staging;
    int16_t* d_init;
    URH_CHECK(digitizer_tables(ctx, ntiles, cap, &tiles, &staging, &d_init));
    const int c0 = host_classify(0.0f, cls);
    if (mod_type == URH_MOD_ASK)
        URH_CHECK((launch_dense_iq_m<URH_MOD_ASK, true>(ctx, dtype, d_iq, n, dp, d_qad_out, cls, tol, tiles, staging, cap, d_init, c0)));
    else
        URH_CHECK((launch_dense_iq_m<URH_MOD_FSK, true>(ctx, dtype, d_iq, n, dp, d_qad_out, cls, tol, tiles, staging, cap, d_init, c0)));
    return urh_finish_local(ctx, n, tol, mod_type == URH_MOD_ASK, samples_per_symbol, tiles, staging, cap, d_init, k);
}

int urh_finish_chunk(urh_ctx* ctx, int64_t n, int tol, bool is_ask, uint32_t sps, const UrhTileSummary* tiles, const uint32_t* staging,
                     int stage_cap, const int16_t* d_init, UrhChain* chain, int64_t global_offset, int64_t n_total, int64_t row_base,
                     int64_t rows_cap, int64_t* k);

static int64_t rows_bound(int64_t n, int tol) { return n / (tol + 1) + 3; }

struct StreamSizes {
    int64_t cs;
    int64_t src_slot;
    int64_t qad_slot;
    int64_t ring_bytes;
    int64_t arena;
    int64_t scan_items;
    int64_t rows_chunk;
};
static int64_t scan_workspace_bytes(int64_t items) {
    const int64_t nb = 2 * (items / 256 + 1);
    return 256 + (nb > 8192 ? nb : 8192) * (4 + 2 * (int64_t)urhts::SLOT);
}
static int64_t finish_arena_bytes(int64_t tiles, int64_t rows_cap, bool ask) {
    return r256(tiles * (int64_t)sizeof(RunCarry)) + 2 * r256(tiles * 4) + 2 * r256(tiles * 8) + r256((32 + 8) * 8) +
           (ask ? r256(rows_cap * 16) : 0);
}
static int psk_order_of(int entry) { return (entry & URH_STREAM_PSK) ? ((entry & URH_STREAM_PSK4) ? 4 : 2) : 0; }
static int psk_entry_flags(int mod_order) { return URH_STREAM_PSK | (mod_order >= 4 ? URH_STREAM_PSK4 : 0); }

static StreamSizes stream_sizes(int64_t n, int dtype, int tol, int64_t chunk_samples, int ring, int entry) {
    StreamSizes z;
    const int kind = entry & 0xf;
    const int psk = psk_order_of(entry);
    const bool resident = entry & URH_STREAM_RESIDENT;
    const int64_t ntiles = urh_div_up(n, URH_TILE);
    z.cs = resident ? ntiles * URH_TILE : stream_chunk_samples(n, chunk_samples);
    const int64_t ct = z.cs / URH_TILE;
    const int64_t cap = stage_cap_for(tol);
    const bool iq = kind != URH_STREAM_ENTRY_GRAB_PULSE_LENS;
    const bool digitize = kind != URH_STREAM_ENTRY_AFP_DEMOD;
    z.rows_chunk = rows_bound(z.cs, tol);
    if (resident) {
        z.src_slot = iq ? n * urh_iq_bytes(dtype) : n * 4;
        z.qad_slot = (kind == URH_STREAM_ENTRY_GRAB_PULSE_LENS) ? 0 : n * 4;
        z.ring_bytes = r256(z.src_slot) + r256(z.qad_slot);
    } else {
        z.src_slot = (kind == URH_STREAM_ENTRY_GRAB_PULSE_LENS && (entry & URH_STREAM_QAD_ON_DEVICE)) ? 0
                     : URH_STREAM_PAD + z.cs * (iq ? urh_iq_bytes(dtype) : 4);
        const bool qad_ring = kind == URH_STREAM_ENTRY_AFP_DEMOD ||
                              (kind == URH_STREAM_ENTRY_DEMOD_DIGITIZE && ((entry & URH_STREAM_QAD_OUT) || psk));
        z.qad_slot = qad_ring ? z.cs * 4 : 0;
        z.ring_bytes = ring * (r256(z.src_slot) + r256(z.qad_slot));
        if (kind == URH_STREAM_ENTRY_DEMOD_CENTER_DIGITIZE) z.ring_bytes += r256(n * 4);
    }
    z.arena = 0;
    z.scan_items = ct > z.rows_chunk ? ct : z.rows_chunk;
    if (digitize) z.arena += r256(ct * (int64_t)sizeof(UrhTileSummary)) + r256(ct * cap * 4) + r256(16) + r256(sizeof(UrhChain)) +
                             finish_arena_bytes(ct, z.rows_chunk, true);
    if (psk && !resident) z.arena += urh_costas_arena_bytes(z.cs, psk) + r256(16) + r256(6 * 8);
    if (kind == URH_STREAM_ENTRY_DEMOD_CENTER_DIGITIZE) {
        z.arena += r256(ntiles * (int64_t)sizeof(UrhTileStats)) + r256((int64_t)URH_FINE_SLABS * URH_FINE_NB * 4) + r256((ntiles + 1) * 8) +
                   ((int64_t)2 << 20);
        if (ntiles > z.scan_items) z.scan_items = ntiles;
    }
    return z;
}

static int64_t segment_arena_bytes(int64_t tiles) {
    const int64_t cap = URH_TILE / 10 + 2, cand = tiles * URH_TILE / 10 + 3;
    return r256(tiles * (int64_t)sizeof(UrhTileSummary)) + r256(tiles * cap * 4) + 2 * r256(2 * (int64_t)sizeof(RunCarry)) +
           r256(tiles * 4) + r256(tiles * 8) + r256(32) + r256(cand * 8) + r256(cand * 2);
}
SegmentStreamSizes urh_segment_stream_sizes(int64_t n, int dtype, int64_t chunk_samples) {
    SegmentStreamSizes z;
    z.cs = stream_chunk_samples(n, chunk_samples);
    z.src_slot = r256(URH_STREAM_PAD + z.cs * urh_iq_bytes(dtype));
    z.mag_bytes = r256(z.cs * 8);
    z.arena = segment_arena_bytes(z.cs / URH_TILE);
    return z;
}

extern "C" int urh_stream_footprint(int64_t n, int dtype, int tolerance, int64_t chunk_samples, int ring, int entry, int64_t rows,
                                    int64_t* bytes) {
    if (!bytes || n < 0 || tolerance < 0 || tolerance > 0xffff || (entry & 0xf) > URH_STREAM_ENTRY_ESTIMATE) return URH_ERR_INVALID;
    if ((entry & 0xf) == URH_STREAM_ENTRY_SEGMENT_MESSAGES) {
        if (urh_iq_bytes(dtype) == 0) return URH_ERR_DTYPE;
        if (entry & URH_STREAM_RESIDENT) {
            const int64_t ntiles = urh_div_up(n, URH_TILE);
            *bytes = r256(n * urh_iq_bytes(dtype)) + r256(n * 8) + segment_arena_bytes(ntiles) + URH_ARENA_BLOCK + scan_workspace_bytes(ntiles);
            return URH_OK;
        }
        if (ring < 2 || ring > URH_STREAM_MAX_RING) return URH_ERR_INVALID;
        const SegmentStreamSizes z = urh_segment_stream_sizes(n, dtype, chunk_samples);
        *bytes = ring * z.src_slot + z.mag_bytes + stream_arena_bytes(z.arena) + scan_workspace_bytes(z.cs / URH_TILE);
        return URH_OK;
    }
    if ((entry & 0xf) == URH_STREAM_ENTRY_ESTIMATE) {
        if (!(entry & URH_STREAM_RESIDENT)) return URH_ERR_INVALID;
        if (urh_iq_bytes(dtype) == 0) return URH_ERR_DTYPE;
        int64_t demod = 0;
        URH_CHECK(urh_stream_footprint(n, dtype, 0, chunk_samples, ring, URH_STREAM_ENTRY_AFP_DEMOD | URH_STREAM_PSK | URH_STREAM_RESIDENT,
                                       -1, &demod));
        *bytes = r256(n * 8) + demod;
        return URH_OK;
    }
    if (!(entry & URH_STREAM_RESIDENT) && (ring < 2 || ring > URH_STREAM_MAX_RING)) return URH_ERR_INVALID;
    if ((entry & 0xf) != URH_STREAM_ENTRY_GRAB_PULSE_LENS && urh_iq_bytes(dtype) == 0) return URH_ERR_DTYPE;
    if ((entry & URH_STREAM_PSK) && (entry & 0xf) != URH_STREAM_ENTRY_AFP_DEMOD && (entry & 0xf) != URH_STREAM_ENTRY_DEMOD_DIGITIZE)
        return URH_ERR_INVALID;
    const StreamSizes z = stream_sizes(n, dtype, tolerance, chunk_samples, ring, entry);
    const bool digitize = (entry & 0xf) != URH_STREAM_ENTRY_AFP_DEMOD;
    const int64_t r = rows == -2 ? n / 64 + 1024 : (rows < 0 ? rows_bound(n, tolerance) : rows);
    if (entry & URH_STREAM_RESIDENT) {
        const int64_t ntiles = urh_div_up(n, URH_TILE);
        int64_t b = z.ring_bytes + URH_ARENA_BLOCK;
        if (digitize)
            b += r256(ntiles * (int64_t)sizeof(UrhTileSummary)) + r256(ntiles * (int64_t)stage_cap_for(tolerance) * 4) +
                 finish_arena_bytes(ntiles, r + r / 4, true) + 16 * (r + r / 4);
        if ((entry & 0xf) == URH_STREAM_ENTRY_DEMOD_CENTER_DIGITIZE)
            b += r256(ntiles * (int64_t)sizeof(UrhTileStats)) + r256((int64_t)URH_FINE_SLABS * URH_FINE_NB * 4) + r256((ntiles + 1) * 8);
        if (psk_order_of(entry)) b += urh_costas_arena_bytes(n, psk_order_of(entry));
        *bytes = b;
        return URH_OK;
    }
    int64_t b = z.ring_bytes + stream_arena_bytes(z.arena);
    b += scan_workspace_bytes(z.scan_items);
    if (digitize) b += 3 * 16 * (r + z.rows_chunk);
    *bytes = b;
    return URH_OK;
}

extern "C" int urh_stream_stats(urh_ctx* ctx, int64_t* h_out3) {
    h_out3[0] = ctx->stream_free_low;
    h_out3[1] = ctx->stream_chunks;
    h_out3[2] = (int64_t)ctx->arena_peak;
    return URH_OK;
}

struct StreamDigitizer {
    UrhTileSummary* tiles;
    uint32_t* staging;
    int16_t* d_init;
    UrhChain* chain;
    int cap, tol;
    bool is_ask;
    uint32_t sps;
    int64_t n, rows, rows_all;
    UrhArenaMark mark;
    int init(urh_ctx* ctx, int64_t n_total, int64_t cs, int tolerance, bool ask, uint32_t samples_per_symbol) {
        n = n_total; tol = tolerance; is_ask = ask; sps = samples_per_symbol; rows = 0;
        cap = stage_cap_for(tol);
        rows_all = rows_bound(n, tol);
        URH_CHECK(digitizer_tables(ctx, cs / URH_TILE, cap, &tiles, &staging, &d_init));
        URH_CHECK(urh_arena(ctx, 1, &chain));
        URH_CUDA(ctx, cudaMemsetAsync(d_init, 0, 16, ctx->stream));
        mark = urh_arena_mark(ctx);
        return URH_OK;
    }
    int finish(urh_ctx* ctx, int64_t s0, int64_t s1) {
        const int64_t rc = rows_bound(s1 - s0, tol);
        const int64_t need = rows + rc;
        if (need > (int64_t)ctx->pulses_cap_rows) {
            int64_t grow = 2 * (int64_t)ctx->pulses_cap_rows;
            if (grow > rows_all + rc) grow = rows_all + rc;
            URH_CHECK(urh_ensure_pulses_keep(ctx, (size_t)(grow > need ? grow : need), (size_t)rows));
        }
        urh_arena_release(ctx, mark);
        int64_t kc = 0;
        URH_CHECK(urh_finish_chunk(ctx, s1 - s0, tol, is_ask, sps, tiles, staging, cap, d_init, chain, s0, n, rows, rc, &kc));
        urh_stream_sample_free(ctx);
        rows += kc;
        return URH_OK;
    }
};

static int stream_check(urh_ctx* ctx, int64_t n, int ring, int mod_type, int dtype, bool iq);
static int psk_stream_check(urh_ctx* ctx, int64_t n, int ring, int dtype) {
    URH_CHECK(stream_check(ctx, n, ring, URH_MOD_PSK, dtype, false));
    if (n <= 2) URH_FAIL(ctx, URH_ERR_INVALID, "streamed PSK demodulation: n > 2");
    if (urh_iq_bytes(dtype) == 0) URH_FAIL(ctx, URH_ERR_DTYPE, "Unsupported dtype");
    return URH_OK;
}

static int stream_check(urh_ctx* ctx, int64_t n, int ring, int mod_type, int dtype, bool iq) {
    if (n <= 0) URH_FAIL(ctx, URH_ERR_INVALID, "streamed call: empty capture");
    if (ring < 2 || ring > URH_STREAM_MAX_RING) URH_FAIL(ctx, URH_ERR_INVALID, "streamed call: ring of %d slots (2..%d)", ring, URH_STREAM_MAX_RING);
    if (iq && (n <= 2 || (mod_type != URH_MOD_ASK && mod_type != URH_MOD_FSK)))
        URH_FAIL(ctx, URH_ERR_INVALID, "streamed demodulation: ASK/FSK and n > 2 (PSK is a serial recurrence)");
    if (iq && urh_iq_bytes(dtype) == 0) URH_FAIL(ctx, URH_ERR_DTYPE, "Unsupported dtype");
    return URH_OK;
}

template <bool DIG>
static int stream_dense_iq(urh_ctx* ctx, int dtype, int mod_type, const char* d_src, int64_t src_slot, int64_t n, const UrhDemodParams& dp,
                           float* qad_global, const UrhClassify& cls, int tol, StreamDigitizer* dz, int64_t s0, int64_t s1, int s,
                           UrhTileStats* ts = nullptr, const UrhFine& fine = UrhFine{}) {
    const int b = urh_iq_bytes(dtype);
    const void* iq = d_src + s * src_slot + URH_STREAM_PAD - s0 * b;
    const int64_t t0 = s0 / URH_TILE, t1 = urh_div_up(s1, URH_TILE);
    UrhTileSummary* tiles = dz ? dz->tiles - t0 : nullptr;
    uint32_t* staging = dz ? dz->staging - t0 * dz->cap : nullptr;
    const int cap = dz ? dz->cap : 0;
    int16_t* init = dz ? dz->d_init : nullptr;
    const int c0 = DIG ? host_classify(0.0f, cls) : 0;
    if (mod_type == URH_MOD_ASK)
        return launch_dense_iq_m<URH_MOD_ASK, DIG>(ctx, dtype, iq, n, dp, qad_global, cls, tol, tiles, staging, cap, init, c0, 0, ts, t0, t1, fine);
    return launch_dense_iq_m<URH_MOD_FSK, DIG>(ctx, dtype, iq, n, dp, qad_global, cls, tol, tiles, staging, cap, init, c0, 0, ts, t0, t1, fine);
}

static int stream_dense_qad(urh_ctx* ctx, const float* x, int64_t s0, int64_t s1, const UrhClassify& cls, StreamDigitizer& dz,
                            const float* d_thr0 = nullptr, const UrhTileStats* ts = nullptr) {
    return launch_dense_qad(ctx, x, s1 - s0, cls, dz.tol, dz.tiles, dz.staging, dz.cap, s0 == 0 ? dz.d_init : nullptr,
                            d_thr0 ? 0 : host_classify(0.0f, cls), d_thr0, ts ? ts + s0 / URH_TILE : nullptr);
}

struct CenterPlan;
int urh_center_chain(urh_ctx* ctx, const float* d_qad, int64_t n, const UrhTileStats* ts, int64_t max_size, int rank, int world,
                     const UrhFine* fine, CenterPlan** d_plan_out);
int urh_center_plan_result(urh_ctx* ctx, const CenterPlan* plan, const float** d_centerf, const double** d_center, const int** d_state);
int urh_center_plan_certify_stats(urh_ctx* ctx, const CenterPlan* plan, int64_t* h_dst3);

extern "C" int urh_shard_digitize(urh_ctx* ctx, const void* d_iq, int dtype, const float* d_qad_in, int64_t n, int has_halo,
                                  float noise_mag, int mod_type, float center, uint16_t tolerance, uint32_t samples_per_symbol,
                                  uint8_t bits_per_symbol, float center_spacing, float* d_qad_out, int64_t global_offset,
                                  int64_t n_total, int64_t* k) {
    if (!k) return URH_ERR_INVALID;
    *k = 0;
    ctx->pulses_k = 0;
    if (n <= 0) URH_FAIL(ctx, URH_ERR_INVALID, "empty shard");
    if (mod_type != URH_MOD_ASK && mod_type != URH_MOD_FSK) URH_FAIL(ctx, URH_ERR_INVALID, "sharded path: ASK / FSK only");
    if (!d_qad_in && urh_iq_bytes(dtype) == 0) URH_FAIL(ctx, URH_ERR_DTYPE, "Unsupported dtype");
    if (!ctx->nccl_comm) URH_FAIL(ctx, URH_ERR_INVALID, "NCCL communicator not initialised (urh_nccl_init)");
    urh_arena_reset(ctx);
    UrhClassify cls;
    URH_CHECK(fill_classify(ctx, &cls, mod_type, center, bits_per_symbol, center_spacing));
    const int tol = tolerance;
    const int64_t ntiles = urh_div_up(n, URH_TILE);
    const int cap = stage_cap_for(tol);
    UrhTileSummary* tiles;
    uint32_t* staging;
    int16_t* d_init;
    URH_CHECK(digitizer_tables(ctx, ntiles, cap, &tiles, &staging, &d_init));
    URH_CUDA(ctx, cudaMemsetAsync(d_init, 0, 16, ctx->stream));
    const int c0 = host_classify(0.0f, cls);
    if (d_qad_in) {
        URH_PROF_BEGIN(ctx);
        URH_CHECK(launch_dense_qad(ctx, d_qad_in, n, cls, tol, tiles, staging, cap, d_init, c0));
        URH_PROF_END(ctx);
    } else {
        const UrhDemodParams dp = make_demod_params(noise_mag, mod_type, dtype);
        if (mod_type == URH_MOD_ASK)
            URH_CHECK((launch_dense_iq_m<URH_MOD_ASK, true>(ctx, dtype, d_iq, n, dp, d_qad_out, cls, tol, tiles, staging, cap, d_init, c0, has_halo)));
        else
            URH_CHECK((launch_dense_iq_m<URH_MOD_FSK, true>(ctx, dtype, d_iq, n, dp, d_qad_out, cls, tol, tiles, staging, cap, d_init, c0, has_halo)));
    }
    return urh_finish_shard(ctx, n, tol, mod_type == URH_MOD_ASK, samples_per_symbol, tiles, staging, cap, d_init, global_offset, n_total, k);
}

struct StreamCenter {
    int ring;
    int64_t chunk_samples;
    const void* h_iq;
    float* h_qad;
    int64_t* kept;
};
static int demod_center_digitize_impl(urh_ctx* ctx, const void* d_iq, int dtype, int64_t n, int has_halo, float noise_mag, int mod_type,
                                      uint16_t tolerance, uint32_t samples_per_symbol, int64_t max_size, float* d_qad_out, bool sharded,
                                      int64_t global_offset, int64_t n_total, double* center, int* center_state, int64_t* k,
                                      const void* h_iq = nullptr, int64_t chunk_samples = 0, const StreamCenter* sc = nullptr) {
    if (!k || !center || !center_state) return URH_ERR_INVALID;
    *k = 0;
    *center = 0.0;
    *center_state = 0;
    ctx->pulses_k = 0;
    if (n <= 2 || (mod_type != URH_MOD_ASK && mod_type != URH_MOD_FSK) || !d_qad_out)
        URH_FAIL(ctx, URH_ERR_INVALID, "demod_center_digitize: ASK/FSK, n > 2 and a qad buffer are required");
    if (urh_iq_bytes(dtype) == 0) URH_FAIL(ctx, URH_ERR_DTYPE, "Unsupported dtype");
    if (sharded && !ctx->nccl_comm) URH_FAIL(ctx, URH_ERR_INVALID, "NCCL communicator not initialised (urh_nccl_init)");
    urh_arena_reset(ctx);
    URH_TL_RESET(ctx);
    URH_TL_MARK(ctx, "step start");
    const UrhDemodParams dp = make_demod_params(noise_mag, mod_type, dtype);
    UrhClassify cls;
    memset(&cls, 0, sizeof(cls));
    const int64_t ntiles = urh_div_up(n, URH_TILE);
    UrhTileStats* ts;
    URH_CHECK(urh_arena(ctx, (size_t)ntiles, &ts));
    const bool no_certify = getenv("URH_B200_CENTER_NO_CERTIFY") != nullptr;
    UrhFine fine = {};
    if (!sharded && !no_certify) {
        fine.slab_tiles = urh_div_up(ntiles, URH_FINE_SLABS);
        if (fine.slab_tiles < URH_WARPS_PER_BLOCK) fine.slab_tiles = URH_WARPS_PER_BLOCK;
        const int64_t nslabs = urh_div_up(ntiles, fine.slab_tiles);
        URH_CHECK(urh_arena(ctx, (size_t)(nslabs * URH_FINE_NB), &fine.gh));
        URH_CUDA(ctx, cudaMemsetAsync(fine.gh, 0, (size_t)(nslabs * URH_FINE_NB) * sizeof(unsigned int), ctx->stream));
        fine.scale = (mod_type == URH_MOD_FSK) ? 512.0f : 4096.0f;
        fine.off = (mod_type == URH_MOD_FSK) ? 2048.0f : 0.0f;
    }
    const int64_t chunk_tiles = (h_iq && chunk_samples > 0) ? (chunk_samples >= URH_TILE ? chunk_samples / URH_TILE : 1) : ntiles;
    const size_t sample_bytes = (size_t)urh_iq_bytes(dtype);
    StreamRing ring;
    int64_t scs = 0;
    if (sc) {
        const StreamSizes z = stream_sizes(n, dtype, tolerance, sc->chunk_samples, sc->ring, URH_STREAM_ENTRY_DEMOD_CENTER_DIGITIZE);
        scs = z.cs;
        URH_CHECK(ring.init(ctx, sc->ring, sc->ring * r256(z.src_slot)));
        const int64_t slot = r256(z.src_slot);
        std::vector<UrhWindow> win;
        URH_CHECK(urh_filter_windows(URH_FILTER_TILES, n, n, 1, 0, sc->chunk_samples, nullptr, nullptr, 0, win));
        URH_CHECK(stream_run(ctx, win, ring, (const char*)sc->h_iq, urh_iq_bytes(dtype), ring.mem, slot, sc->h_qad != nullptr,
                             [&](int64_t, const UrhWindow& w, int s) {
                                 return stream_dense_iq<false>(ctx, dtype, mod_type, ring.mem, slot, n, dp, d_qad_out, cls, 0, nullptr, w.k0, w.k1,
                                                               s, ts, fine);
                             },
                             [&](int64_t, const UrhWindow& w, int, cudaStream_t cp) {
                                 URH_CUDA(ctx, cudaMemcpyAsync(sc->h_qad + w.k0, d_qad_out + w.k0, (size_t)(w.k1 - w.k0) * sizeof(float),
                                                               cudaMemcpyDeviceToHost, cp));
                                 return URH_OK;
                             },
                             place_after_pad, true));
    }
    cls.noise_value = urh_noise_value(mod_type);
    cls.order = 2;
    const int tol = tolerance;
    const int cap = stage_cap_for(tol);
    UrhTileSummary* tiles = nullptr;
    uint32_t* staging = nullptr;
    int16_t* d_init = nullptr;
    if (!sc) URH_CHECK(digitizer_tables(ctx, ntiles, cap, &tiles, &staging, &d_init));
    const bool speculate = !sharded && !h_iq && !sc && mod_type == URH_MOD_FSK && dtype == URH_DT_F32 &&
                           getenv("URH_B200_NO_SPECULATE") == nullptr;
    UrhSpec spec = {};
    if (speculate) {
        float* tg;
        URH_CHECK(urh_arena(ctx, 1, &tg));
        URH_CHECK(urh_arena(ctx, 1, &spec.redone));
        URH_CHECK(urh_arena(ctx, (size_t)ntiles, &spec.margin));
        spec.tg = tg;
        const char* forced = getenv("URH_B200_SPECULATE_GUESS");
        URH_LAUNCH(ctx, k_speculate_guess, 1, URH_GUESS_THREADS, 0, (const float2*)d_iq, n, dp.noise_sqrd, forced ? 1 : 0,
                   forced ? strtof(forced, nullptr) : 0.0f, tg, spec.redone);
    }
    int chunk_no = 0;
    for (int64_t t0 = 0; t0 < (sc ? 0 : ntiles); t0 += chunk_tiles, chunk_no++) {
        const int64_t t1 = (t0 + chunk_tiles < ntiles) ? t0 + chunk_tiles : ntiles;
        if (h_iq) {
            const int64_t s0 = t0 * URH_TILE, s1 = (t1 * URH_TILE < n) ? t1 * URH_TILE : n;
            cudaEvent_t ev = ctx->ev_copy[chunk_no & 1];
            URH_CUDA(ctx, cudaMemcpyAsync((char*)d_iq + (size_t)s0 * sample_bytes, (const char*)h_iq + (size_t)s0 * sample_bytes,
                                          (size_t)(s1 - s0) * sample_bytes, cudaMemcpyHostToDevice, ctx->copy_stream[0]));
            URH_CUDA(ctx, cudaEventRecord(ev, ctx->copy_stream[0]));
            URH_CUDA(ctx, cudaStreamWaitEvent(ctx->stream, ev, 0));
        }
        if (mod_type == URH_MOD_ASK)
            URH_CHECK((launch_dense_iq_m<URH_MOD_ASK, false>(ctx, dtype, d_iq, n, dp, d_qad_out, cls, 0, nullptr, nullptr, 0, nullptr, 0, has_halo, ts, t0, t1, fine)));
        else
            URH_CHECK((launch_dense_iq_m<URH_MOD_FSK, false>(ctx, dtype, d_iq, n, dp, d_qad_out, cls, tol, tiles, staging, cap, nullptr, 0, has_halo,
                                                             ts, t0, t1, fine, speculate ? &spec : nullptr)));
    }
    CenterPlan* plan = nullptr;
    URH_CHECK(urh_center_chain(ctx, d_qad_out, n, ts, max_size, sharded ? ctx->nccl_rank : 0, sharded ? ctx->nccl_world : 1,
                               fine.gh ? &fine : nullptr, &plan));
    const float* d_centerf;
    const double* d_center;
    const int* d_state;
    urh_center_plan_result(ctx, plan, &d_centerf, &d_center, &d_state);
    int64_t rows = 0;
    if (sc) {
        URH_CUDA(ctx, cudaMemcpyAsync(ctx->h_mail + 40, d_center, sizeof(double), cudaMemcpyDeviceToHost, ctx->stream));
        URH_CUDA(ctx, cudaMemcpyAsync(ctx->h_mail + 41, d_state, sizeof(int), cudaMemcpyDeviceToHost, ctx->stream));
        URH_CHECK(urh_center_plan_certify_stats(ctx, plan, ctx->h_mail + 42));
        URH_CUDA(ctx, cudaMemcpyAsync(ctx->h_mail + 45, (const int64_t*)ctx->center_prefix + ntiles, sizeof(int64_t), cudaMemcpyDeviceToHost,
                                      ctx->stream));
        URH_CUDA(ctx, cudaStreamSynchronize(ctx->stream));
        int st0 = 0;
        memcpy(&st0, ctx->h_mail + 41, sizeof(int));
        if (st0 == 1) {
            StreamDigitizer dz;
            URH_CHECK(dz.init(ctx, n, scs, tol, mod_type == URH_MOD_ASK, samples_per_symbol));
            for (int64_t s0 = 0; s0 < n; s0 += scs) {
                const int64_t s1 = s0 + scs < n ? s0 + scs : n;
                URH_CHECK(stream_dense_qad(ctx, d_qad_out + s0, s0, s1, cls, dz, d_centerf, ts));
                URH_CHECK(dz.finish(ctx, s0, s1));
            }
            rows = dz.rows;
        }
        *sc->kept = ctx->h_mail[45];
    } else {
        URH_CUDA(ctx, cudaMemsetAsync(d_init, 0, 16, ctx->stream));
        const int vec_in = (((uintptr_t)d_qad_out % 8) == 0) ? 1 : 0;
        int64_t grid = urh_div_up(ntiles, URH_WARPS_PER_BLOCK);
        if (speculate) {
            int per_sm = 0;
            URH_CUDA(ctx, cudaOccupancyMaxActiveBlocksPerMultiprocessor(&per_sm, k_dense_f32<SrcQad2, float>, URH_WARPS_PER_BLOCK * 32, 0));
            const int64_t resident = (int64_t)ctx->sm_count * (per_sm > 0 ? per_sm : 1);
            if (grid > resident) grid = resident;
        }
        URH_LAUNCH(ctx, (k_dense_f32<SrcQad2, float>), (unsigned)grid, URH_WARPS_PER_BLOCK * 32, 0,
                   (const float*)d_qad_out, n, vec_in, cls, tol, tiles, staging, cap, d_init, 0, d_centerf, (const UrhTileStats*)ts, spec);
        URH_CUDA(ctx, cudaMemcpyAsync(ctx->h_mail + 40, d_center, sizeof(double), cudaMemcpyDeviceToHost, ctx->stream));
        URH_CUDA(ctx, cudaMemcpyAsync(ctx->h_mail + 41, d_state, sizeof(int), cudaMemcpyDeviceToHost, ctx->stream));
        URH_CHECK(urh_center_plan_certify_stats(ctx, plan, ctx->h_mail + 42));
        ctx->h_mail[46] = 0;
        if (speculate) URH_CUDA(ctx, cudaMemcpyAsync(ctx->h_mail + 46, spec.redone, sizeof(unsigned int), cudaMemcpyDeviceToHost, ctx->stream));
        if (sharded)
            URH_CHECK(urh_finish_shard(ctx, n, tol, mod_type == URH_MOD_ASK, samples_per_symbol, tiles, staging, cap, d_init, global_offset, n_total, &rows));
        else
            URH_CHECK(urh_finish_local(ctx, n, tol, mod_type == URH_MOD_ASK, samples_per_symbol, tiles, staging, cap, d_init, &rows));
    }
    memcpy(center, ctx->h_mail + 40, sizeof(double));
    int st = 0;
    memcpy(&st, ctx->h_mail + 41, sizeof(int));
    *center_state = st;
    ctx->center_cert[0] = ctx->h_mail[42];
    ctx->center_cert[1] = fine.gh ? URH_FINE_NB : 0;
    ctx->center_cert[2] = ctx->h_mail[44];
    const int64_t redone = (spec.hi > spec.lo) ? ctx->h_mail[46] : 0;
    ctx->spec_stats[0] = spec.hi - spec.lo;
    ctx->spec_stats[1] = spec.hi - spec.lo - redone;
    ctx->spec_stats[2] = redone;
    if (st != 1) {
        ctx->pulses_k = 0;
        rows = 0;
    }
    *k = rows;
    return URH_OK;
}

extern "C" int urh_speculate_stats(urh_ctx* ctx, int64_t* h_out3) {
    for (int i = 0; i < 3; i++) h_out3[i] = ctx->spec_stats[i];
    return URH_OK;
}

extern "C" int urh_demod_center_digitize(urh_ctx* ctx, const void* d_iq, int dtype, int64_t n, float noise_mag, int mod_type,
                                         uint16_t tolerance, uint32_t samples_per_symbol, int64_t max_size, float* d_qad_out,
                                         double* center, int* center_state, int64_t* k) {
    return demod_center_digitize_impl(ctx, d_iq, dtype, n, 0, noise_mag, mod_type, tolerance, samples_per_symbol, max_size, d_qad_out, false,
                                      0, n, center, center_state, k);
}

extern "C" int urh_demod_center_digitize_host(urh_ctx* ctx, const void* h_iq, int dtype, int64_t n, float noise_mag, int mod_type,
                                              uint16_t tolerance, uint32_t samples_per_symbol, int64_t max_size, int64_t chunk_samples,
                                              void* d_iq_scratch, float* d_qad_out, double* center, int* center_state, int64_t* k) {
    if (!h_iq || !d_iq_scratch) return URH_ERR_INVALID;
    URH_CUDA(ctx, cudaEventRecord(ctx->ev_comp[0], ctx->stream));
    URH_CUDA(ctx, cudaStreamWaitEvent(ctx->copy_stream[0], ctx->ev_comp[0], 0));
    return demod_center_digitize_impl(ctx, d_iq_scratch, dtype, n, 0, noise_mag, mod_type, tolerance, samples_per_symbol, max_size, d_qad_out,
                                      false, 0, n, center, center_state, k, h_iq, chunk_samples > 0 ? chunk_samples : ((int64_t)1 << 24));
}

extern "C" int urh_shard_demod_center_digitize_host(urh_ctx* ctx, const void* h_iq, int dtype, int64_t n, int has_halo, float noise_mag,
                                                    int mod_type, uint16_t tolerance, uint32_t samples_per_symbol, int64_t max_size,
                                                    int64_t chunk_samples, void* d_iq_scratch, float* d_qad_out, int64_t global_offset,
                                                    int64_t n_total, double* center, int* center_state, int64_t* k) {
    if (!h_iq || !d_iq_scratch) return URH_ERR_INVALID;
    URH_CUDA(ctx, cudaEventRecord(ctx->ev_comp[0], ctx->stream));
    URH_CUDA(ctx, cudaStreamWaitEvent(ctx->copy_stream[0], ctx->ev_comp[0], 0));
    return demod_center_digitize_impl(ctx, d_iq_scratch, dtype, n, has_halo, noise_mag, mod_type, tolerance, samples_per_symbol, max_size,
                                      d_qad_out, true, global_offset, n_total, center, center_state, k, h_iq,
                                      chunk_samples > 0 ? chunk_samples : ((int64_t)1 << 24));
}

extern "C" int urh_shard_demod_center_digitize(urh_ctx* ctx, const void* d_iq, int dtype, int64_t n, int has_halo, float noise_mag,
                                               int mod_type, uint16_t tolerance, uint32_t samples_per_symbol, int64_t max_size,
                                               float* d_qad_out, int64_t global_offset, int64_t n_total, double* center,
                                               int* center_state, int64_t* k) {
    return demod_center_digitize_impl(ctx, d_iq, dtype, n, has_halo, noise_mag, mod_type, tolerance, samples_per_symbol, max_size, d_qad_out,
                                      true, global_offset, n_total, center, center_state, k);
}

extern "C" int urh_afp_demod_stream(urh_ctx* ctx, const void* h_iq, int dtype, int64_t n, float noise_mag, int mod_type, int64_t chunk_samples,
                                    int ring, float* h_qad) {
    if (!h_iq || !h_qad) return URH_ERR_INVALID;
    URH_CHECK(stream_check(ctx, n, ring, mod_type, dtype, true));
    urh_arena_reset(ctx);
    const StreamSizes z = stream_sizes(n, dtype, 0, chunk_samples, ring, URH_STREAM_ENTRY_AFP_DEMOD);
    StreamRing R;
    URH_CHECK(R.init(ctx, ring, z.ring_bytes));
    char* d_src = R.mem;
    float* d_qad = (float*)(R.mem + ring * r256(z.src_slot));
    const UrhDemodParams dp = make_demod_params(noise_mag, mod_type, dtype);
    UrhClassify cls;
    memset(&cls, 0, sizeof(cls));
    std::vector<UrhWindow> win;
    URH_CHECK(urh_filter_windows(URH_FILTER_TILES, n, n, 1, 0, chunk_samples, nullptr, nullptr, 0, win));
    return stream_run(ctx, win, R, (const char*)h_iq, urh_iq_bytes(dtype), d_src, r256(z.src_slot), true,
                      [&](int64_t, const UrhWindow& w, int s) {
                          return stream_dense_iq<false>(ctx, dtype, mod_type, d_src, r256(z.src_slot), n, dp, d_qad + s * z.cs - w.k0, cls, 0,
                                                        nullptr, w.k0, w.k1, s);
                      },
                      contiguous_download(ctx, (const char*)d_qad, z.cs * 4, (char*)h_qad, 4), place_after_pad);
}

extern "C" int urh_grab_pulse_lens_stream(urh_ctx* ctx, const float* qad, int qad_on_device, int64_t n, float center, uint16_t tolerance,
                                          int mod_type, uint32_t samples_per_symbol, uint8_t bits_per_symbol, float center_spacing,
                                          int64_t chunk_samples, int ring, int64_t* k) {
    if (!k || !qad) return URH_ERR_INVALID;
    *k = 0;
    ctx->pulses_k = 0;
    URH_CHECK(stream_check(ctx, n, ring, mod_type, 0, false));
    urh_arena_reset(ctx);
    UrhClassify cls;
    URH_CHECK(fill_classify(ctx, &cls, mod_type, center, bits_per_symbol, center_spacing));
    const StreamSizes z = stream_sizes(n, 0, tolerance, chunk_samples, ring,
                                       URH_STREAM_ENTRY_GRAB_PULSE_LENS | (qad_on_device ? URH_STREAM_QAD_ON_DEVICE : 0));
    StreamRing R;
    URH_CHECK(R.init(ctx, ring, z.ring_bytes));
    StreamDigitizer dz;
    URH_CHECK(dz.init(ctx, n, z.cs, tolerance, mod_type == URH_MOD_ASK, samples_per_symbol));
    char* d_src = R.mem;
    std::vector<UrhWindow> win;
    URH_CHECK(urh_filter_windows(URH_FILTER_TILES, n, n, 0, 0, chunk_samples, nullptr, nullptr, 0, win));
    URH_CHECK(stream_run(ctx, win, R, qad_on_device ? nullptr : (const char*)qad, 4, d_src, r256(z.src_slot), false,
                         [&](int64_t, const UrhWindow& w, int s) {
                             const float* x = qad_on_device ? qad + w.k0 : (const float*)(d_src + s * r256(z.src_slot) + URH_STREAM_PAD);
                             URH_CHECK(stream_dense_qad(ctx, x, w.k0, w.k1, cls, dz));
                             return dz.finish(ctx, w.k0, w.k1);
                         },
                         no_download, place_after_pad));
    *k = dz.rows;
    return URH_OK;
}

extern "C" int urh_demod_digitize_stream(urh_ctx* ctx, const void* h_iq, int dtype, int64_t n, float noise_mag, int mod_type, float center,
                                         uint16_t tolerance, uint32_t samples_per_symbol, uint8_t bits_per_symbol, float center_spacing,
                                         int64_t chunk_samples, int ring, float* h_qad_out, int64_t* k) {
    if (!k || !h_iq) return URH_ERR_INVALID;
    *k = 0;
    ctx->pulses_k = 0;
    URH_CHECK(stream_check(ctx, n, ring, mod_type, dtype, true));
    urh_arena_reset(ctx);
    UrhClassify cls;
    URH_CHECK(fill_classify(ctx, &cls, mod_type, center, bits_per_symbol, center_spacing));
    const UrhDemodParams dp = make_demod_params(noise_mag, mod_type, dtype);
    const StreamSizes z = stream_sizes(n, dtype, tolerance, chunk_samples, ring,
                                       URH_STREAM_ENTRY_DEMOD_DIGITIZE | (h_qad_out ? URH_STREAM_QAD_OUT : 0));
    StreamRing R;
    URH_CHECK(R.init(ctx, ring, z.ring_bytes));
    StreamDigitizer dz;
    URH_CHECK(dz.init(ctx, n, z.cs, tolerance, mod_type == URH_MOD_ASK, samples_per_symbol));
    char* d_src = R.mem;
    float* d_qad = h_qad_out ? (float*)(R.mem + ring * r256(z.src_slot)) : nullptr;
    std::vector<UrhWindow> win;
    URH_CHECK(urh_filter_windows(URH_FILTER_TILES, n, n, 1, 0, chunk_samples, nullptr, nullptr, 0, win));
    URH_CHECK(stream_run(ctx, win, R, (const char*)h_iq, urh_iq_bytes(dtype), d_src, r256(z.src_slot), h_qad_out != nullptr,
                         [&](int64_t, const UrhWindow& w, int s) {
                             URH_CHECK(stream_dense_iq<true>(ctx, dtype, mod_type, d_src, r256(z.src_slot), n, dp,
                                                             d_qad ? d_qad + s * z.cs - w.k0 : nullptr, cls, tolerance, &dz, w.k0, w.k1, s));
                             return dz.finish(ctx, w.k0, w.k1);
                         },
                         contiguous_download(ctx, (const char*)d_qad, z.cs * 4, (char*)h_qad_out, 4), place_after_pad));
    *k = dz.rows;
    return URH_OK;
}

extern "C" int urh_demod_center_digitize_stream(urh_ctx* ctx, const void* h_iq, int dtype, int64_t n, float noise_mag, int mod_type,
                                                uint16_t tolerance, uint32_t samples_per_symbol, int64_t max_size, int64_t chunk_samples,
                                                int ring, float* d_qad_out, float* h_qad_out, double* center, int* center_state,
                                                int64_t* kept, int64_t* k) {
    if (!h_iq || !d_qad_out || !kept) return URH_ERR_INVALID;
    URH_CHECK(stream_check(ctx, n, ring, mod_type, dtype, true));
    StreamCenter sc;
    sc.ring = ring; sc.chunk_samples = chunk_samples; sc.h_iq = h_iq; sc.h_qad = h_qad_out; sc.kept = kept;
    return demod_center_digitize_impl(ctx, nullptr, dtype, n, 0, noise_mag, mod_type, tolerance, samples_per_symbol, max_size, d_qad_out,
                                      false, 0, n, center, center_state, k, nullptr, 0, &sc);
}

extern "C" int urh_afp_demod_psk_stream(urh_ctx* ctx, const void* h_iq, int dtype, int64_t n, float noise_mag, int mod_order,
                                        float costas_loop_bandwidth, int64_t chunk_samples, int ring, float* h_qad) {
    if (!h_iq || !h_qad) return URH_ERR_INVALID;
    URH_CHECK(psk_stream_check(ctx, n, ring, dtype));
    urh_arena_reset(ctx);
    const StreamSizes z = stream_sizes(n, dtype, 0, chunk_samples, ring, URH_STREAM_ENTRY_AFP_DEMOD | psk_entry_flags(mod_order));
    StreamRing R;
    URH_CHECK(R.init(ctx, ring, z.ring_bytes));
    const int64_t slot = r256(z.src_slot);
    char* d_src = R.mem;
    float* d_qad = (float*)(R.mem + ring * slot);
    const UrhDemodParams dp = make_demod_params(noise_mag, URH_MOD_PSK, dtype);
    UrhCostasStream cs;
    URH_CHECK(urh_costas_stream_begin(ctx, &cs));
    const UrhArenaMark mark = urh_arena_mark(ctx);
    std::vector<UrhWindow> win;
    URH_CHECK(urh_filter_windows(URH_FILTER_TILES, n, n, 0, 0, chunk_samples, nullptr, nullptr, 0, win));
    URH_CHECK(stream_run(ctx, win, R, (const char*)h_iq, urh_iq_bytes(dtype), d_src, slot, true,
                         [&](int64_t c, const UrhWindow& w, int s) {
                             urh_arena_release(ctx, mark);
                             return urh_costas_stream_chunk(ctx, &cs, c, d_src + s * slot + URH_STREAM_PAD, dtype, w.k1 - w.k0, dp.noise_sqrd,
                                                            mod_order, costas_loop_bandwidth, d_qad + s * z.cs);
                         },
                         contiguous_download(ctx, (const char*)d_qad, z.cs * 4, (char*)h_qad, 4), place_after_pad));
    return urh_costas_stream_end(ctx, &cs);
}

extern "C" int urh_demod_digitize_psk_stream(urh_ctx* ctx, const void* h_iq, int dtype, int64_t n, float noise_mag, float center,
                                             uint16_t tolerance, uint32_t samples_per_symbol, uint8_t bits_per_symbol, float center_spacing,
                                             int64_t chunk_samples, int ring, float* h_qad_out, int64_t* k) {
    if (!k || !h_iq) return URH_ERR_INVALID;
    *k = 0;
    ctx->pulses_k = 0;
    URH_CHECK(psk_stream_check(ctx, n, ring, dtype));
    urh_arena_reset(ctx);
    UrhClassify cls;
    URH_CHECK(fill_classify(ctx, &cls, URH_MOD_PSK, center, bits_per_symbol, center_spacing));
    const int mod_order = 1 << bits_per_symbol;
    const UrhDemodParams dp = make_demod_params(noise_mag, URH_MOD_PSK, dtype);
    const StreamSizes z = stream_sizes(n, dtype, tolerance, chunk_samples, ring,
                                       URH_STREAM_ENTRY_DEMOD_DIGITIZE | (h_qad_out ? URH_STREAM_QAD_OUT : 0) | psk_entry_flags(mod_order));
    StreamRing R;
    URH_CHECK(R.init(ctx, ring, z.ring_bytes));
    const int64_t slot = r256(z.src_slot);
    char* d_src = R.mem;
    float* d_qad = (float*)(R.mem + ring * slot);
    UrhCostasStream cs;
    URH_CHECK(urh_costas_stream_begin(ctx, &cs));
    StreamDigitizer dz;
    URH_CHECK(dz.init(ctx, n, z.cs, tolerance, false, samples_per_symbol));
    std::vector<UrhWindow> win;
    URH_CHECK(urh_filter_windows(URH_FILTER_TILES, n, n, 0, 0, chunk_samples, nullptr, nullptr, 0, win));
    URH_CHECK(stream_run(ctx, win, R, (const char*)h_iq, urh_iq_bytes(dtype), d_src, slot, h_qad_out != nullptr,
                         [&](int64_t c, const UrhWindow& w, int s) {
                             urh_arena_release(ctx, dz.mark);
                             float* q = d_qad + s * z.cs;
                             URH_CHECK(urh_costas_stream_chunk(ctx, &cs, c, d_src + s * slot + URH_STREAM_PAD, dtype, w.k1 - w.k0, dp.noise_sqrd,
                                                               mod_order, 0.1f, q));
                             URH_CHECK(stream_dense_qad(ctx, q, w.k0, w.k1, cls, dz));
                             return dz.finish(ctx, w.k0, w.k1);
                         },
                         contiguous_download(ctx, (const char*)d_qad, z.cs * 4, (char*)h_qad_out, 4), place_after_pad));
    *k = dz.rows;
    return urh_costas_stream_end(ctx, &cs);
}

struct UrhShardState {
    UrhCandidates cand;
};
static UrhShardState* shard_state(urh_ctx* ctx) {
    if (!ctx->shard_state) ctx->shard_state = calloc(1, sizeof(UrhShardState));
    return (UrhShardState*)ctx->shard_state;
}

extern "C" int urh_shard_candidates(urh_ctx* ctx, int carry_valid, int carry_cls, int64_t carry_len, int64_t global_offset,
                                    int64_t* count, const int64_t** d_pos, const int16_t** d_cls, int* last_cand_cls) {
    if (!ctx->shard_tiles) URH_FAIL(ctx, URH_ERR_INVALID, "urh_segment_shard_pass must precede urh_shard_candidates");
    UrhShardCarry in;
    in.valid = carry_valid; in.cls = carry_cls; in.len = carry_len;
    UrhShardState* S = shard_state(ctx);
    URH_CHECK(urh_collect_candidates_shard(ctx, ctx->shard_n, ctx->shard_tol, (const UrhTileSummary*)ctx->shard_tiles,
                                           (const uint32_t*)ctx->shard_staging, ctx->shard_cap, in, global_offset, &S->cand));
    *count = S->cand.count;
    if (d_pos) *d_pos = S->cand.pos;
    if (d_cls) *d_cls = S->cand.cls;
    if (last_cand_cls) {
        *last_cand_cls = 0;
        if (S->cand.count > 0) {
            int16_t v = 0;
            URH_CUDA(ctx, cudaMemcpyAsync(&v, S->cand.cls + S->cand.count - 1, sizeof(v), cudaMemcpyDeviceToHost, ctx->stream));
            URH_CUDA(ctx, cudaStreamSynchronize(ctx->stream));
            *last_cand_cls = v;
        }
    }
    ctx->shard_tiles = nullptr;
    return URH_OK;
}

extern "C" int urh_fetch_candidates(urh_ctx* ctx, int64_t* h_pos, int16_t* h_cls, int64_t count) {
    UrhShardState* S = shard_state(ctx);
    if (count < 0 || count > S->cand.count) URH_FAIL(ctx, URH_ERR_INVALID, "fetch_candidates: count exceeds the table");
    if (count == 0) return URH_OK;
    URH_CUDA(ctx, cudaMemcpyAsync(h_pos, S->cand.pos, (size_t)count * sizeof(int64_t), cudaMemcpyDeviceToHost, ctx->stream));
    URH_CUDA(ctx, cudaMemcpyAsync(h_cls, S->cand.cls, (size_t)count * sizeof(int16_t), cudaMemcpyDeviceToHost, ctx->stream));
    URH_CUDA(ctx, cudaStreamSynchronize(ctx->stream));
    return URH_OK;
}

extern "C" int urh_fetch_pulses(urh_ctx* ctx, int64_t* h_rows, int64_t k) {
    if (k < 0 || k > ctx->pulses_k) URH_FAIL(ctx, URH_ERR_INVALID, "fetch_pulses: k=%lld exceeds last result %lld", (long long)k, (long long)ctx->pulses_k);
    if (k == 0) return URH_OK;
    URH_CUDA(ctx, cudaMemcpyAsync(h_rows, ctx->pulses, (size_t)k * 2 * sizeof(int64_t), cudaMemcpyDeviceToHost, ctx->stream));
    URH_CUDA(ctx, cudaStreamSynchronize(ctx->stream));
    return URH_OK;
}

extern "C" int urh_pulses_device_ptr(urh_ctx* ctx, const int64_t** d_rows, int64_t* k) {
    if (d_rows) *d_rows = ctx->pulses;
    if (k) *k = ctx->pulses_k;
    return URH_OK;
}


__global__ void k_selftest_div(uint64_t seed, int64_t count, unsigned long long* mismatches, unsigned long long* tested) {
    const int64_t stride = (int64_t)gridDim.x * blockDim.x;
    unsigned long long bad = 0, ok = 0;
    for (int64_t i = (int64_t)blockIdx.x * blockDim.x + threadIdx.x; i < count; i += stride) {
        uint64_t h = seed + (uint64_t)i * 0x9E3779B97F4A7C15ull;
        h = (h ^ (h >> 30)) * 0xBF58476D1CE4E5B9ull;
        h = (h ^ (h >> 27)) * 0x94D049BB133111EBull;
        h ^= h >> 31;
        uint64_t g = h * 0xD6E8FEB86659FD93ull + 0x632BE59BD9B4E019ull;
        g ^= g >> 29;
        const uint32_t span = URH_DIVWIN_HI - URH_DIVWIN_LO;
        uint32_t ea = URH_DIVWIN_LO + (uint32_t)((h >> 40) % span), eb = URH_DIVWIN_LO + (uint32_t)((g >> 40) % span);
        uint32_t ma = (uint32_t)h & 0x7fffff, mb = (uint32_t)g & 0x7fffff;
        if ((i & 15) == 1) ma = 0;
        if ((i & 15) == 2) mb = 0;
        if ((i & 15) == 3) { ma = 0x7fffff; }
        if ((i & 15) == 4) { mb = 0x7fffff; }
        if ((i & 15) == 5) { eb = ea; }
        float a0 = __uint_as_float((ea << 23) | ma), b0 = __uint_as_float((eb << 23) | mb);
        float a1 = __uint_as_float(((URH_DIVWIN_LO + (uint32_t)((g >> 12) % span)) << 23) | ((uint32_t)(h >> 9) & 0x7fffff));
        float b1 = __uint_as_float(((URH_DIVWIN_LO + (uint32_t)((h >> 12) % span)) << 23) | ((uint32_t)(g >> 9) & 0x7fffff));
        if ((i & 15) == 6) { a1 = __uint_as_float((URH_DIVWIN_LO << 23)); b1 = __uint_as_float(((URH_DIVWIN_HI - 1) << 23) | 0x7fffff); }
        if ((i & 15) == 8) { b1 = __uint_as_float((URH_DIVWIN_LO << 23)); a1 = __uint_as_float(((URH_DIVWIN_HI - 1) << 23) | 0x7fffff); }
        if ((i & 63) == 7) a1 = 0.0f;
        const float2 q = urh_div2_window(make_float2(a0, a1), make_float2(b0, b1));
        const float r0 = __fdiv_rn(a0, b0), r1 = __fdiv_rn(a1, b1);
        bad += (__float_as_uint(q.x) != __float_as_uint(r0)) + (__float_as_uint(q.y) != __float_as_uint(r1));
        ok += 2;
    }
    atomicAdd(mismatches, bad);
    atomicAdd(tested, ok);
}

extern "C" int urh_selftest_packed_div(urh_ctx* ctx, uint64_t seed, int64_t count, int64_t* mismatches, int64_t* tested) {
    urh_arena_reset(ctx);
    unsigned long long* d;
    URH_CHECK(urh_arena(ctx, 2, &d));
    URH_CUDA(ctx, cudaMemsetAsync(d, 0, 16, ctx->stream));
    URH_LAUNCH(ctx, k_selftest_div, (unsigned)(ctx->sm_count * 8), 256, 0, seed, count, d, d + 1);
    int64_t h[2];
    URH_CHECK(urh_read_i64(ctx, (const int64_t*)d, 2, h));
    *mismatches = h[0];
    *tested = h[1];
    return URH_OK;
}
```

### urh_b200/csrc/finish.cu

```cuda
#include "sparse.cuh"
#include "tilescan.cuh"

#include <limits.h>

#define CLS_NONE INT_MIN

struct __align__(16) CandAgg {
    int64_t cnt;
    int32_t last_cls;
    int32_t pad;
};
struct CandOp {
    __device__ __forceinline__ CandAgg operator()(const CandAgg& a, const CandAgg& b) const {
        CandAgg r;
        r.cnt = a.cnt + b.cnt;
        r.last_cls = (b.last_cls != CLS_NONE) ? b.last_cls : a.last_cls;
        r.pad = 0;
        return r;
    }
};
struct __align__(16) FireAgg {
    int64_t fired;
    int64_t last_pos;
};
struct FireOp {
    __device__ __forceinline__ FireAgg operator()(const FireAgg& a, const FireAgg& b) const {
        FireAgg r;
        r.fired = a.fired + b.fired;
        r.last_pos = (b.last_pos >= 0) ? b.last_pos : a.last_pos;
        return r;
    }
};

struct ScanRunCarry : TileRuns {
    RunCarry* carry;
    __device__ __forceinline__ void post(int64_t t, const RunCarry& excl, const RunCarry&) const { carry[t] = excl; }
};

struct __align__(16) TileFire {
    int32_t first_cls;
    int32_t first_rel;
    int32_t fired;
    int32_t last_rel;
};
struct ScanCandidates {
    const UrhTileSummary* tiles;
    const uint32_t* staging;
    int stage_cap;
    const RunCarry* carry;
    const RunCarry* xcarry;
    int tol;
    int32_t* head_rel;
    int32_t* prev_cls;
    TileFire* fire;
    __device__ __forceinline__ CandAgg load(int64_t t) const {
        const UrhTileSummary s = tiles[t];
        RunCarry c = carry[t];
        if (xcarry) c = RunCarryOp()(*xcarry, c);
        int64_t start_len = 0;
        if (!(c.flags & 2) && c.cls == s.first_cls) start_len = c.len;
        int32_t rel = -1;
        if (start_len <= tol && (int64_t)tol < start_len + s.head_len) rel = (int32_t)(tol - start_len);
        head_rel[t] = rel;
        TileFire f;
        f.first_cls = CLS_NONE; f.first_rel = -1; f.fired = 0; f.last_rel = -1;
        int prev = CLS_NONE;
        if (rel >= 0) {
            prev = s.first_cls;
            f.first_cls = prev;
            f.first_rel = rel;
        }
        const uint32_t* st = staging + t * (int64_t)stage_cap;
        for (int j = 0; j < s.ncand; j += 4) {
            uint32_t w[4];
#pragma unroll
            for (int u = 0; u < 4; u++) w[u] = (j + u < s.ncand) ? st[j + u] : 0u;
#pragma unroll
            for (int u = 0; u < 4; u++) {
                if (j + u < s.ncand) {
                    const int cl = (int)(w[u] & 0xffffu) - 1;
                    const int p = (int)(w[u] >> 16);
                    if (prev == CLS_NONE) {
                        f.first_cls = cl;
                        f.first_rel = p;
                    } else if (cl != prev) {
                        f.fired++;
                        f.last_rel = p;
                    }
                    prev = cl;
                }
            }
        }
        fire[t] = f;
        CandAgg r;
        r.cnt = (int64_t)s.ncand + (rel >= 0 ? 1 : 0);
        r.last_cls = prev;
        r.pad = 0;
        return r;
    }
    __device__ __forceinline__ void post(int64_t t, const CandAgg& excl, const CandAgg&) const { prev_cls[t] = excl.last_cls; }
};

struct ScanFirings {
    const TileFire* fire;
    const int32_t* prev_cls;
    const int16_t* d_prev0;
    int64_t global_offset;
    int64_t* row_off;
    int64_t* prev_fired;
    __device__ __forceinline__ FireAgg load(int64_t t) const {
        const TileFire f = fire[t];
        int prev = prev_cls[t];
        if (prev == CLS_NONE) prev = *d_prev0;
        FireAgg r;
        r.fired = f.fired;
        int32_t last = f.last_rel;
        if (f.first_cls != CLS_NONE && f.first_cls != prev) {
            r.fired++;
            if (last < 0) last = f.first_rel;
        }
        r.last_pos = (last >= 0) ? t * URH_TILE + global_offset + last : -1;
        return r;
    }
    __device__ __forceinline__ void post(int64_t t, const FireAgg& excl, const FireAgg&) const {
        row_off[t] = excl.fired;
        prev_fired[t] = excl.last_pos;
    }
};

constexpr int FIN_TILES = 32;
constexpr int FIN_BATCH = 8;

struct FinRows {
    int64_t* out;
    int64_t cap_rows;
    int tol;
    int is_ask;
    int64_t sps;
};

struct FinWalk {
    int prev;
    int64_t pp;
    int64_t idx;
};

__device__ __forceinline__ void fin_row(const FinRows& R, int64_t idx, int64_t p, int64_t pp, int prev) {
    const int64_t rec = (pp >= 0) ? (p - pp) : (p + 1 - R.tol);
    int64_t st = prev;
    if (R.is_ask && st == -1 && rec < R.sps) st = 0;
    if (idx < R.cap_rows) *((longlong2*)R.out + idx) = make_longlong2(st, rec);
}

__device__ __forceinline__ void fin_chunk(FinWalk& W, uint32_t w, int cnt, int lane, int64_t base, const FinRows& R) {
    const int c = (int)(w & 0xffffu) - 1;
    const int rel = (int)(w >> 16);
    int pc = __shfl_up_sync(URH_FULL_MASK, c, 1);
    if (lane == 0) pc = W.prev;
    const bool fire = lane < cnt && c != pc;
    const unsigned fm = __ballot_sync(URH_FULL_MASK, fire);
    const unsigned lower = fm & ((1u << lane) - 1u);
    const int before = __shfl_sync(URH_FULL_MASK, rel, lower ? 31 - __clz(lower) : 0);
    if (fire) fin_row(R, W.idx + __popc(lower), base + rel, lower ? base + before : W.pp, pc);
    if (fm) W.pp = base + __shfl_sync(URH_FULL_MASK, rel, 31 - __clz(fm));
    W.idx += __popc(fm);
    if (cnt > 0) W.prev = __shfl_sync(URH_FULL_MASK, c, cnt - 1);
}

__global__ void __launch_bounds__(256) k_finish_rows(const UrhTileSummary* __restrict__ tiles, const uint32_t* __restrict__ staging,
                                                    int stage_cap, const int32_t* __restrict__ head_rel, const int32_t* __restrict__ prev_cls,
                                                    const int16_t* __restrict__ d_prev0, const int64_t* __restrict__ row_off,
                                                    const int64_t* __restrict__ prev_fired, const int64_t* __restrict__ d_xprev_fired,
                                                    int64_t ntiles, int64_t global_offset, int64_t n_total, int tol, int is_ask, int64_t sps,
                                                    int emit_tail, int64_t row_base, int64_t* __restrict__ out, int64_t cap_rows,
                                                    int64_t* __restrict__ d_out) {
    const int64_t t0 = ((int64_t)blockIdx.x * blockDim.x + threadIdx.x) / 32 * FIN_TILES;
    if (t0 >= ntiles) return;
    const int lane = threadIdx.x & 31;
    FinRows R;
    R.out = out; R.cap_rows = cap_rows; R.tol = tol; R.is_ask = is_ask; R.sps = sps;
    const int64_t tl = t0 + lane;
    int l_first = 0, l_ncand = 0, l_rel = -1, l_prev = 0;
    int64_t l_idx = 0, l_pp = -1;
    if (tl < ntiles) {
        const UrhTileSummary s = tiles[tl];
        l_first = s.first_cls;
        l_ncand = s.ncand;
        l_rel = head_rel[tl];
        l_prev = prev_cls[tl];
        if (l_prev == CLS_NONE) l_prev = *d_prev0;
        l_idx = row_off[tl];
        l_pp = prev_fired[tl];
        if (l_pp < 0) l_pp = *d_xprev_fired;
    }
    for (int j0 = 0; j0 < FIN_TILES && t0 + j0 < ntiles; j0 += FIN_BATCH) {
        uint32_t w0[FIN_BATCH];
#pragma unroll
        for (int u = 0; u < FIN_BATCH; u++) {
            const int nc = __shfl_sync(URH_FULL_MASK, l_ncand, j0 + u);
            w0[u] = (lane < nc) ? __ldg(staging + (t0 + j0 + u) * (int64_t)stage_cap + lane) : 0u;
        }
#pragma unroll
        for (int u = 0; u < FIN_BATCH; u++) {
            const int j = j0 + u;
            const int64_t t = t0 + j;
            if (t >= ntiles) break;
            const int64_t base = t * URH_TILE + global_offset;
            const int ncand = __shfl_sync(URH_FULL_MASK, l_ncand, j);
            const int rel = __shfl_sync(URH_FULL_MASK, l_rel, j);
            FinWalk W;
            W.prev = __shfl_sync(URH_FULL_MASK, l_prev, j);
            W.pp = __shfl_sync(URH_FULL_MASK, l_pp, j);
            W.idx = __shfl_sync(URH_FULL_MASK, l_idx, j);
            if (rel >= 0) {
                const int c = __shfl_sync(URH_FULL_MASK, l_first, j);
                if (c != W.prev) {
                    if (lane == 0) fin_row(R, W.idx, base + rel, W.pp, W.prev);
                    W.idx++;
                    W.pp = base + rel;
                }
                W.prev = c;
            }
            const uint32_t* st = staging + t * (int64_t)stage_cap;
            for (int k = 0; k < ncand; k += 32) {
                const uint32_t w = (k == 0) ? w0[u] : ((k + lane < ncand) ? __ldg(st + k + lane) : 0u);
                fin_chunk(W, w, min(32, ncand - k), lane, base, R);
            }
            if (t == ntiles - 1 && lane == 0) {
                int64_t idx = W.idx;
                const int64_t fired = idx;
                if (emit_tail && (is_ask || row_base + fired < n_total)) {
                    if (idx < cap_rows) *((longlong2*)out + idx) = make_longlong2(W.prev, (W.pp >= 0) ? (n_total - 1 - W.pp) : (n_total - tol));
                    idx++;
                }
                d_out[0] = idx;
                d_out[1] = fired;
            }
        }
    }
}

struct ScanMergeRows {
    const int64_t* raw;
    int64_t rows;
    int64_t n_total;
    int has_tail;
    int64_t* out;
    int64_t* d_k;
    const int64_t* prev_last;
    int64_t row_base;
    __device__ __forceinline__ int64_t load(int64_t r) const {
        if (r == 0) return (prev_last && raw[0] == *prev_last) ? 0 : 1;
        return raw[2 * r] != raw[2 * r - 2] ? 1 : 0;
    }
    __device__ __forceinline__ void post(int64_t r, const int64_t& excl, const int64_t& head) const {
        const bool is_tail = has_tail && r == rows - 1;
        if (is_tail && row_base + excl >= n_total) {
            *d_k = excl;
            return;
        }
        const int64_t o = excl + head - 1;
        if (head) out[2 * o] = raw[2 * r];
        atomicAdd((unsigned long long*)&out[2 * o + 1], (unsigned long long)raw[2 * r + 1]);
        if (r == rows - 1) *d_k = o + 1;
    }
};
struct AddI64 {
    __device__ __forceinline__ int64_t operator()(int64_t a, int64_t b) const { return a + b; }
};

__global__ void k_pack_stage1(const int16_t* __restrict__ d_init, const RunCarry* __restrict__ total, int64_t* __restrict__ msg) {
    memcpy(msg, total, sizeof(RunCarry));
    msg[2] = *d_init;
    msg[3] = 0;
}
__global__ void k_fold_carry(const int64_t* __restrict__ all, int rank, RunCarry* __restrict__ xcarry) {
    RunCarry acc;
    acc.len = 0; acc.cls = 0; acc.flags = 2 | 1;
    for (int q = 0; q < rank; q++) {
        RunCarry c;
        memcpy(&c, all + 4 * q, sizeof(c));
        acc = RunCarryOp()(acc, c);
    }
    if (rank == 0) acc.flags = 2;
    else acc.flags &= ~1;
    *xcarry = acc;
}
__global__ void k_fold_prev_cls(const int64_t* __restrict__ all, int rank, const int64_t* __restrict__ stage1, int16_t* __restrict__ prev0) {
    int v = (int)stage1[2];
    for (int q = 0; q < rank; q++) {
        CandAgg c;
        memcpy(&c, all + 2 * q, sizeof(c));
        if (c.last_cls != CLS_NONE) v = c.last_cls;
    }
    *prev0 = (int16_t)v;
}
__global__ void k_fold_prev_fired(const int64_t* __restrict__ all, int rank, int64_t* __restrict__ xprev) {
    int64_t v = -1;
    for (int q = 0; q < rank; q++) {
        FireAgg c;
        memcpy(&c, all + 2 * q, sizeof(c));
        if (c.last_pos >= 0) v = c.last_pos;
    }
    *xprev = v;
}

__global__ void k_chain_start(const int16_t* __restrict__ d_init, UrhChain* __restrict__ chain) {
    chain->run.len = 0; chain->run.cls = 0; chain->run.flags = 2 | 1;
    chain->prev_fired = -1;
    chain->last_state = INT64_MIN;
    chain->prev_cls = *d_init;
}
__global__ void k_chain_advance(UrhChain* __restrict__ chain, const RunCarry* __restrict__ tot_run, const CandAgg* __restrict__ tot_cand,
                                const FireAgg* __restrict__ tot_fire) {
    chain->run = RunCarryOp()(chain->run, *tot_run);
    if (tot_cand->last_cls != CLS_NONE) chain->prev_cls = (int16_t)tot_cand->last_cls;
    if (tot_fire->last_pos >= 0) chain->prev_fired = tot_fire->last_pos;
}
__global__ void k_chain_last_row(UrhChain* __restrict__ chain, const int64_t* __restrict__ table, int64_t rows) {
    if (rows > 0) chain->last_state = table[2 * (rows - 1)];
}

struct FinishShard {
    int rank, world;
    int64_t global_offset;
    int64_t n_total;
    int emit_tail;
    UrhChain* chain;
    int64_t row_base, rows_cap;
};

static int finish_tiles(urh_ctx* ctx, int64_t n, int tol, bool is_ask, uint32_t sps, const UrhTileSummary* tiles, const uint32_t* staging,
                        int stage_cap, const int16_t* d_init, const FinishShard& sh, int64_t* k) {
    const int64_t ntiles = urh_div_up(n, URH_TILE);
    const bool sharded = sh.world > 1;
    UrhChain* chain = sh.chain;
    RunCarry* carry;
    int32_t *head_rel, *prev_cls;
    int64_t *row_off, *prev_fired, *d_small;
    URH_CHECK(urh_arena(ctx, (size_t)ntiles, &carry));
    URH_CHECK(urh_arena(ctx, (size_t)ntiles, &head_rel));
    URH_CHECK(urh_arena(ctx, (size_t)ntiles, &prev_cls));
    URH_CHECK(urh_arena(ctx, (size_t)ntiles, &row_off));
    URH_CHECK(urh_arena(ctx, (size_t)ntiles, &prev_fired));
    TileFire* fire;
    URH_CHECK(urh_arena(ctx, (size_t)ntiles, &fire));
    URH_CHECK(urh_arena(ctx, (size_t)(32 + 8 * (sharded ? sh.world : 0)), &d_small));
    URH_CUDA(ctx, cudaMemsetAsync(d_small, 0xff, 4 * sizeof(int64_t), ctx->stream));
    RunCarry* d_tot_run = (RunCarry*)(d_small + 4);
    CandAgg* d_tot_cand = (CandAgg*)(d_small + 6);
    FireAgg* d_tot_fire = (FireAgg*)(d_small + 8);
    RunCarry* d_xcarry = (RunCarry*)(d_small + 10);
    int16_t* d_prev0 = (int16_t*)(d_small + 12);
    int64_t* d_xprev = d_small + 13;
    int64_t* d_msg1 = d_small + 16;
    int64_t* d_all1 = d_small + 32;
    int64_t* d_all2 = d_all1 + 4 * (sharded ? sh.world : 0);
    int64_t* d_all3 = d_all2 + 2 * (sharded ? sh.world : 0);

    if (chain && sh.global_offset == 0) URH_LAUNCH(ctx, k_chain_start, 1, 1, 0, d_init, chain);
    RunCarry rc_ident;
    rc_ident.len = 0; rc_ident.cls = 0; rc_ident.flags = 2 | 1;
    ScanRunCarry fa;
    fa.tiles = tiles; fa.n = n; fa.carry = carry;
    URH_CHECK((urhts::scan<RunCarry, RunCarryOp, ScanRunCarry>(ctx, ntiles, rc_ident, RunCarryOp(), fa, d_tot_run)));
    if (sharded) {
        URH_LAUNCH(ctx, k_pack_stage1, 1, 1, 0, d_init, (const RunCarry*)d_tot_run, d_msg1);
        URH_TL_MARK(ctx, "x4 run carry: enter");
        URH_CHECK(urh_nccl_allgather(ctx, d_msg1, d_all1, 4 * sizeof(int64_t)));
        URH_TL_MARK(ctx, "x4 run carry: done");
        URH_LAUNCH(ctx, k_fold_carry, 1, 1, 0, (const int64_t*)d_all1, sh.rank, d_xcarry);
    }
    ScanCandidates fb;
    fb.tiles = tiles; fb.staging = staging; fb.stage_cap = stage_cap; fb.carry = carry;
    fb.xcarry = sharded ? d_xcarry : (chain ? &chain->run : nullptr);
    fb.tol = tol; fb.head_rel = head_rel; fb.prev_cls = prev_cls; fb.fire = fire;
    CandAgg ca_ident;
    ca_ident.cnt = 0; ca_ident.last_cls = CLS_NONE; ca_ident.pad = 0;
    URH_CHECK((urhts::scan<CandAgg, CandOp, ScanCandidates, 4>(ctx, ntiles, ca_ident, CandOp(), fb, d_tot_cand)));
    const int16_t* prev0 = chain ? &chain->prev_cls : d_init;
    if (sharded) {
        URH_TL_MARK(ctx, "x5 candidates: enter");
        URH_CHECK(urh_nccl_allgather(ctx, d_tot_cand, d_all2, sizeof(CandAgg)));
        URH_TL_MARK(ctx, "x5 candidates: done");
        URH_LAUNCH(ctx, k_fold_prev_cls, 1, 1, 0, (const int64_t*)d_all2, sh.rank, (const int64_t*)d_all1, d_prev0);
        prev0 = d_prev0;
    }
    ScanFirings fc;
    fc.fire = fire; fc.prev_cls = prev_cls; fc.d_prev0 = prev0; fc.global_offset = sh.global_offset; fc.row_off = row_off;
    fc.prev_fired = prev_fired;
    FireAgg fi_ident;
    fi_ident.fired = 0; fi_ident.last_pos = -1;
    URH_CHECK((urhts::scan<FireAgg, FireOp, ScanFirings>(ctx, ntiles, fi_ident, FireOp(), fc, d_tot_fire)));
    const int64_t* xprev = chain ? &chain->prev_fired : d_small + 2;
    if (sharded) {
        URH_TL_MARK(ctx, "x6 firings: enter");
        URH_CHECK(urh_nccl_allgather(ctx, d_tot_fire, d_all3, sizeof(FireAgg)));
        URH_TL_MARK(ctx, "x6 firings: done");
        URH_LAUNCH(ctx, k_fold_prev_fired, 1, 1, 0, (const int64_t*)d_all3, sh.rank, d_xprev);
        xprev = d_xprev;
    }

    int64_t cap_rows = (int64_t)ctx->pulses_cap_rows;
    const int64_t guess = n / 64 + 1024;
    if (!chain && cap_rows < guess) {
        URH_CHECK(urh_ensure_pulses(ctx, (size_t)guess));
        cap_rows = (int64_t)ctx->pulses_cap_rows;
    }
    const int64_t row_base = chain ? sh.row_base : 0;
    int64_t* raw = ctx->pulses + 2 * row_base;
    int64_t raw_cap = chain ? sh.rows_cap : cap_rows;
    if (is_ask) URH_CHECK(urh_arena(ctx, (size_t)raw_cap * 2, &raw));
    int64_t got[2] = {0, 0};
    for (int attempt = 0; attempt < 2; attempt++) {
        URH_LAUNCH(ctx, k_finish_rows, (unsigned)urh_div_up(ntiles, 8 * FIN_TILES), 256, 0, tiles, staging, stage_cap, (const int32_t*)head_rel,
                   (const int32_t*)prev_cls, prev0, (const int64_t*)row_off, (const int64_t*)prev_fired, xprev, ntiles, sh.global_offset,
                   sh.n_total, tol, is_ask ? 1 : 0, (int64_t)sps, sh.emit_tail, row_base, raw, raw_cap, d_small);
        if (sharded && attempt == 0) URH_TL_MARK(ctx, "rows written");
        URH_CHECK(urh_read_i64(ctx, d_small, 2, got));
        if (got[0] <= raw_cap) break;
        if (attempt == 1 || chain) URH_FAIL(ctx, URH_ERR_CUDA, "finish_tiles: row buffer overflow after regrowth");
        if (is_ask) {
            URH_CHECK(urh_arena(ctx, (size_t)got[0] * 2, &raw));
            raw_cap = got[0];
        } else {
            URH_CHECK(urh_ensure_pulses(ctx, (size_t)got[0]));
            raw = ctx->pulses;
            raw_cap = (int64_t)ctx->pulses_cap_rows;
        }
    }
    if (chain) URH_LAUNCH(ctx, k_chain_advance, 1, 1, 0, chain, (const RunCarry*)d_tot_run, (const CandAgg*)d_tot_cand, (const FireAgg*)d_tot_fire);
    int64_t K = got[0];
    if (is_ask && K > 0) {
        if (!chain) URH_CHECK(urh_ensure_pulses(ctx, (size_t)K));
        int64_t* out = ctx->pulses + 2 * row_base;
        URH_CUDA(ctx, cudaMemsetAsync(out, 0, (size_t)K * 2 * sizeof(int64_t), ctx->stream));
        ScanMergeRows fm;
        fm.raw = raw; fm.rows = K; fm.n_total = sh.n_total; fm.has_tail = (sh.emit_tail && K > got[1]) ? 1 : 0; fm.out = out;
        fm.d_k = d_small;
        fm.prev_last = (chain && row_base > 0) ? &chain->last_state : nullptr;
        fm.row_base = row_base;
        URH_CHECK((urhts::scan<int64_t, AddI64, ScanMergeRows>(ctx, K, (int64_t)0, AddI64(), fm, (int64_t*)nullptr)));
        URH_CHECK(urh_read_i64(ctx, d_small, 1, &K));
        if (chain) URH_LAUNCH(ctx, k_chain_last_row, 1, 1, 0, chain, (const int64_t*)ctx->pulses, row_base + K);
    }
    ctx->pulses_k = row_base + K;
    *k = K;
    return URH_OK;
}

int urh_finish_chunk(urh_ctx* ctx, int64_t n, int tol, bool is_ask, uint32_t sps, const UrhTileSummary* tiles, const uint32_t* staging,
                     int stage_cap, const int16_t* d_init, UrhChain* chain, int64_t global_offset, int64_t n_total, int64_t row_base,
                     int64_t rows_cap, int64_t* k) {
    FinishShard sh;
    sh.rank = 0; sh.world = 1; sh.global_offset = global_offset; sh.n_total = n_total;
    sh.emit_tail = (global_offset + n == n_total) ? 1 : 0;
    sh.chain = chain; sh.row_base = row_base; sh.rows_cap = rows_cap;
    return finish_tiles(ctx, n, tol, is_ask, sps, tiles, staging, stage_cap, d_init, sh, k);
}

int urh_finish_local(urh_ctx* ctx, int64_t n, int tol, bool is_ask, uint32_t sps, const UrhTileSummary* tiles, const uint32_t* staging,
                     int stage_cap, const int16_t* d_init, int64_t* k) {
    FinishShard sh;
    sh.rank = 0; sh.world = 1; sh.global_offset = 0; sh.n_total = n; sh.emit_tail = 1;
    sh.chain = nullptr; sh.row_base = 0; sh.rows_cap = 0;
    return finish_tiles(ctx, n, tol, is_ask, sps, tiles, staging, stage_cap, d_init, sh, k);
}

int urh_finish_shard(urh_ctx* ctx, int64_t n, int tol, bool is_ask, uint32_t sps, const UrhTileSummary* tiles, const uint32_t* staging,
                     int stage_cap, const int16_t* d_init, int64_t global_offset, int64_t n_total, int64_t* k) {
    FinishShard sh;
    sh.rank = ctx->nccl_rank; sh.world = ctx->nccl_world; sh.global_offset = global_offset; sh.n_total = n_total;
    sh.emit_tail = (ctx->nccl_rank == ctx->nccl_world - 1) ? 1 : 0;
    sh.chain = nullptr; sh.row_base = 0; sh.rows_cap = 0;
    return finish_tiles(ctx, n, tol, is_ask, sps, tiles, staging, stage_cap, d_init, sh, k);
}
```

Measured before the change: 218,300.

## Fuse candidate and firing scans, parallelize certify, batch plan readback

Merges the separate candidate and firing tile scans into one scan over a combined associative CandFire operator. For sharded runs this removes a scan pass, one allgather and one fold kernel. The certify kernel now spreads the per-slab histogram reduction across several blocks and uses a last-block ticket to do the final step. The speculation guess kernel switches to warp match-based histogram atomics and a parallel top-2 peak search. Plan results are read back with a single contiguous memcpy, and the redone counter moves into the plan struct. The new combined operator is more complex per element, and correctness now depends on the ticket ordering and the fixed struct layout.

```diff
diff --git a/urh_b200/csrc/center.cu b/urh_b200/csrc/center.cu
--- a/urh_b200/csrc/center.cu
+++ b/urh_b200/csrc/center.cu
@@ -523,8 +523,11 @@
     unsigned int ticket;
     int certified;
     long long straddle;
-    long long pad;
+    unsigned int cert_ticket;
+    unsigned int redone;
 };
+constexpr size_t CEN_RESULT_BYTES = offsetof(CenterPlan, redone) + sizeof(unsigned int) - offsetof(CenterPlan, center);
+static_assert(CEN_RESULT_BYTES == 48, "CenterPlan: the step's results are one contiguous 48-byte block");
 
 __global__ void k_center_ranks(const int64_t* __restrict__ counts, int rank, int world, int64_t max_size, CenterPlan* __restrict__ plan) {
     long long total = 0, offset = 0;
@@ -541,6 +544,8 @@
     b = b < 0 ? 0 : (b > kept ? kept : b);
     plan->lr0 = a; plan->lr1 = b;
     plan->ticket = 0u;
+    plan->cert_ticket = 0u;
+    plan->redone = 0u;
     plan->state = 1;
     plan->certified = 0;
     plan->straddle = 0;
@@ -743,27 +748,48 @@
 }
 
 #define CERT_THREADS 512
+#define CERT_SPAN 128
+#define CERT_BLOCKS (URH_FINE_NB / CERT_SPAN)
 __global__ void __launch_bounds__(CERT_THREADS) k_center_certify(const UrhFine fine, CenterPlan* __restrict__ plan, const float* __restrict__ fe,
                                                                  const unsigned long long* __restrict__ xhist, unsigned long long* __restrict__ lo,
-                                                                 unsigned long long* __restrict__ hi) {
+                                                                 unsigned long long* __restrict__ hi, unsigned long long* __restrict__ bsum) {
     __shared__ unsigned long long s_ge[URH_FINE_NB + 1];
     __shared__ unsigned long long s_part[CERT_THREADS];
     __shared__ unsigned char s_flag[CEN_MAX_BINS];
     __shared__ unsigned long long s_key[3];
     __shared__ unsigned int s_certain;
+    __shared__ bool s_last;
     if (plan->state != 1) return;
     const int tid = threadIdx.x;
-    constexpr int PER = URH_FINE_NB / CERT_THREADS;
     int64_t sf, se;
     cen_full_slabs(plan->win[0], plan->win[1], fine.slab_tiles, &sf, &se);
+    {
+        constexpr int STRIDE = CERT_THREADS / CERT_SPAN;
+        const int bucket = blockIdx.x * CERT_SPAN + tid % CERT_SPAN;
+        unsigned long long v = 0;
+        for (int64_t sl = sf + tid / CERT_SPAN; sl < se; sl += STRIDE) v += fine.gh[sl * URH_FINE_NB + bucket];
+        s_part[tid] = v;
+        __syncthreads();
+        if (tid < CERT_SPAN) {
+#pragma unroll
+            for (int k = 1; k < STRIDE; k++) v += s_part[tid + k * CERT_SPAN];
+            bsum[bucket] = v;
+        }
+        __threadfence();
+        __syncthreads();
+        if (tid == 0) s_last = atomicAdd(&plan->cert_ticket, 1u) == gridDim.x - 1;
+        __syncthreads();
+        if (!s_last) return;
+        __threadfence();
+    }
+    constexpr int PER = URH_FINE_NB / CERT_THREADS;
     unsigned long long b[PER], tot = 0;
 #pragma unroll
     for (int j = 0; j < PER; j++) {
-        unsigned long long v = 0;
-        for (int64_t sl = sf; sl < se; sl++) v += fine.gh[sl * URH_FINE_NB + tid * PER + j];
-        b[j] = v;
-        tot += v;
-    }
+        b[j] = __ldcg(bsum + tid * PER + j);
+        tot += b[j];
+    }
+    __syncthreads();
     s_part[tid] = tot;
     if (tid < 3) s_key[tid] = 0ull;
     if (tid == 0) s_certain = 0u;
@@ -938,7 +964,7 @@
     unsigned long long* hist;
     int64_t* d_counts;
     CenStats* d_parts;
-    unsigned long long *xhist = nullptr, *cert_lo = nullptr, *cert_hi = nullptr;
+    unsigned long long *xhist = nullptr, *cert_lo = nullptr, *cert_hi = nullptr, *cert_sum = nullptr;
     const int nb = ctx->sm_count * 2;
     URH_CHECK(urh_arena(ctx, (size_t)ntiles + 1, &prefix));
     URH_CHECK(urh_arena(ctx, 1, &plan));
@@ -951,6 +977,7 @@
         URH_CHECK(urh_arena(ctx, (size_t)CEN_MAX_BINS, &xhist));
         URH_CHECK(urh_arena(ctx, (size_t)CEN_MAX_BINS, &cert_lo));
         URH_CHECK(urh_arena(ctx, (size_t)CEN_MAX_BINS, &cert_hi));
+        URH_CHECK(urh_arena(ctx, (size_t)URH_FINE_NB, &cert_sum));
     }
     URH_CHECK(kept_prefix(ctx, ts, ntiles, prefix));
     const int64_t* counts = prefix + ntiles;
@@ -974,7 +1001,9 @@
     const unsigned gs = (unsigned)min(urh_div_up(ntiles, 8), (int64_t)ctx->sm_count * 8);
     URH_LAUNCH(ctx, k_hist_window_ends_dev, fine ? 2 + ctx->sm_count * 4 : 2, 256, fine ? dyn : 0, d_qad, n, (const int64_t*)prefix,
                (const CenterPlan*)plan, (const float*)fe, hist, xhist, fine ? fine->slab_tiles : (int64_t)1);
-    if (fine) URH_LAUNCH(ctx, k_center_certify, 1, CERT_THREADS, 0, *fine, plan, (const float*)fe, (const unsigned long long*)xhist, cert_lo, cert_hi);
+    if (fine)
+        URH_LAUNCH(ctx, k_center_certify, CERT_BLOCKS, CERT_THREADS, 0, *fine, plan, (const float*)fe, (const unsigned long long*)xhist, cert_lo,
+                   cert_hi, cert_sum);
     URH_LAUNCH(ctx, (k_hist_interior_dev<true>), gs, 256, dyn, d_qad, n, (const CenterPlan*)plan, (const float*)fe, hist, (const int64_t*)prefix);
     URH_LAUNCH(ctx, (k_hist_interior_dev<false>), gs, 256, dyn, d_qad, n, (const CenterPlan*)plan, (const float*)fe, hist, (const int64_t*)prefix);
     if (world > 1) {
@@ -991,12 +1020,21 @@
     return URH_OK;
 }
 
-int urh_center_plan_certify_stats(urh_ctx* ctx, const CenterPlan* plan, int64_t* h_dst3) {
-    h_dst3[0] = h_dst3[1] = h_dst3[2] = 0;
-    URH_CUDA(ctx, cudaMemcpyAsync(h_dst3, &plan->certified, sizeof(int), cudaMemcpyDeviceToHost, ctx->stream));
-    URH_CUDA(ctx, cudaMemcpyAsync(h_dst3 + 2, &plan->straddle, sizeof(long long), cudaMemcpyDeviceToHost, ctx->stream));
+int urh_center_plan_fetch(urh_ctx* ctx, const CenterPlan* plan, int64_t* h_dst) {
+    URH_CUDA(ctx, cudaMemcpyAsync(h_dst, &plan->center, CEN_RESULT_BYTES, cudaMemcpyDeviceToHost, ctx->stream));
     return URH_OK;
 }
+void urh_center_plan_unpack(const int64_t* h, double* center, int* state, int64_t* certified, int64_t* straddle, int64_t* redone) {
+    const char* b = (const char*)h - offsetof(CenterPlan, center);
+    CenterPlan p;
+    memcpy(&p.center, b + offsetof(CenterPlan, center), CEN_RESULT_BYTES);
+    *center = p.center;
+    *state = p.state;
+    *certified = p.certified;
+    *straddle = p.straddle;
+    *redone = p.redone;
+}
+unsigned int* urh_center_plan_redone(CenterPlan* plan) { return &plan->redone; }
 
 extern "C" int urh_center_certify_stats(urh_ctx* ctx, int64_t* h_out3) {
     for (int i = 0; i < 3; i++) h_out3[i] = ctx->center_cert[i];
diff --git a/urh_b200/csrc/digitize.cu b/urh_b200/csrc/digitize.cu
--- a/urh_b200/csrc/digitize.cu
+++ b/urh_b200/csrc/digitize.cu
@@ -136,12 +136,13 @@
 #define URH_GUESS_BINS 128
 #define URH_GUESS_THREADS 1024
 __global__ void __launch_bounds__(URH_GUESS_THREADS) k_speculate_guess(const float2* __restrict__ iq, int64_t n, float noise_sqrd, int forced,
-                                                                      float forced_tg, float* __restrict__ d_tg, unsigned int* __restrict__ redone) {
+                                                                      float forced_tg, float* __restrict__ d_tg) {
     constexpr int PER = URH_GUESS_SAMPLES / URH_GUESS_THREADS;
     __shared__ unsigned int s_hist[URH_GUESS_BINS];
     __shared__ float s_mn[32], s_mx[32];
+    __shared__ unsigned int s_key[2][URH_GUESS_BINS / 32];
     if (forced) {
-        if (threadIdx.x == 0) { *d_tg = forced_tg; *redone = 0u; }
+        if (threadIdx.x == 0) *d_tg = forced_tg;
         return;
     }
     for (int b = threadIdx.x; b < URH_GUESS_BINS; b += blockDim.x) s_hist[b] = 0u;
@@ -168,29 +169,44 @@
     for (int w = 0; w < URH_GUESS_THREADS / 32; w++) { mn = fminf(mn, s_mn[w]); mx = fmaxf(mx, s_mx[w]); }
     const float width = (mx - mn) / URH_GUESS_BINS;
     if (width > 0.0f) {
+        const unsigned lane_lt = (1u << (threadIdx.x & 31)) - 1u;
 #pragma unroll
-        for (int k = 0; k < PER; k++)
-            if (!isnan(v[k])) atomicAdd(&s_hist[min((int)((v[k] - mn) / width), URH_GUESS_BINS - 1)], 1u);
+        for (int k = 0; k < PER; k++) {
+            const int b = isnan(v[k]) ? -1 : min((int)((v[k] - mn) / width), URH_GUESS_BINS - 1);
+            const unsigned same = __match_any_sync(URH_FULL_MASK, b);
+            if (b >= 0 && !(same & lane_lt)) atomicAdd(&s_hist[b], (unsigned)__popc(same));
+        }
     }
     __syncthreads();
-    if (threadIdx.x != 0) return;
-    *redone = 0u;
-    if (!(mn <= mx)) { *d_tg = 0.0f; return; }
-    if (!(width > 0.0f)) { *d_tg = mn; return; }
     constexpr int WINDOW = (int)(0.05 * URH_GUESS_BINS) + 1;
-    int top[2] = {-1, -1};
-    for (int b = 0; b < URH_GUESS_BINS; b++) {
+    unsigned int key = 0u;
+    if (width > 0.0f && threadIdx.x < URH_GUESS_BINS) {
+        const int b = threadIdx.x;
         const unsigned int y = s_hist[b];
         bool peak = y > 0u;
         for (int d = 1; d < WINDOW && peak; d++)
             peak = y > (b + d < URH_GUESS_BINS ? s_hist[b + d] : 0u) && y > (b - d >= 0 ? s_hist[b - d] : 0u);
-        if (!peak) continue;
-        if (top[0] < 0 || y > s_hist[top[0]]) { top[1] = top[0]; top[0] = b; }
-        else if (top[1] < 0 || y > s_hist[top[1]]) top[1] = b;
-    }
-    if (top[0] < 0) *d_tg = 0.5f * (mn + mx);
-    else if (top[1] < 0) *d_tg = mn + ((float)top[0] + 0.5f) * width;
-    else *d_tg = mn + (0.5f * (float)(top[0] + top[1]) + 0.5f) * width;
+        if (peak) key = (y << 8) | (unsigned int)(255 - b);
+    }
+    constexpr int KW = URH_GUESS_BINS / 32;
+    unsigned int top[2];
+#pragma unroll
+    for (int r = 0; r < 2; r++) {
+        if (r == 1 && key == top[0]) key = 0u;
+        const unsigned int wk = __reduce_max_sync(URH_FULL_MASK, key);
+        if (threadIdx.x < URH_GUESS_BINS && (threadIdx.x & 31) == 0) s_key[r][threadIdx.x >> 5] = wk;
+        __syncthreads();
+        top[r] = 0u;
+#pragma unroll
+        for (int w = 0; w < KW; w++) top[r] = max(top[r], s_key[r][w]);
+    }
+    if (threadIdx.x != 0) return;
+    if (!(mn <= mx)) { *d_tg = 0.0f; return; }
+    if (!(width > 0.0f)) { *d_tg = mn; return; }
+    const int b0 = 255 - (int)(top[0] & 255u), b1 = 255 - (int)(top[1] & 255u);
+    if (top[0] == 0u) *d_tg = 0.5f * (mn + mx);
+    else if (top[1] == 0u) *d_tg = mn + ((float)b0 + 0.5f) * width;
+    else *d_tg = mn + (0.5f * (float)(b0 + b1) + 0.5f) * width;
 }
 
 
@@ -679,7 +695,9 @@
 int urh_center_chain(urh_ctx* ctx, const float* d_qad, int64_t n, const UrhTileStats* ts, int64_t max_size, int rank, int world,
                      const UrhFine* fine, CenterPlan** d_plan_out);
 int urh_center_plan_result(urh_ctx* ctx, const CenterPlan* plan, const float** d_centerf, const double** d_center, const int** d_state);
-int urh_center_plan_certify_stats(urh_ctx* ctx, const CenterPlan* plan, int64_t* h_dst3);
+int urh_center_plan_fetch(urh_ctx* ctx, const CenterPlan* plan, int64_t* h_dst);
+void urh_center_plan_unpack(const int64_t* h, double* center, int* state, int64_t* certified, int64_t* straddle, int64_t* redone);
+unsigned int* urh_center_plan_redone(CenterPlan* plan);
 
 extern "C" int urh_shard_digitize(urh_ctx* ctx, const void* d_iq, int dtype, const float* d_qad_in, int64_t n, int has_halo,
                                   float noise_mag, int mod_type, float center, uint16_t tolerance, uint32_t samples_per_symbol,
@@ -795,12 +813,11 @@
     if (speculate) {
         float* tg;
         URH_CHECK(urh_arena(ctx, 1, &tg));
-        URH_CHECK(urh_arena(ctx, 1, &spec.redone));
         URH_CHECK(urh_arena(ctx, (size_t)ntiles, &spec.margin));
         spec.tg = tg;
         const char* forced = getenv("URH_B200_SPECULATE_GUESS");
         URH_LAUNCH(ctx, k_speculate_guess, 1, URH_GUESS_THREADS, 0, (const float2*)d_iq, n, dp.noise_sqrd, forced ? 1 : 0,
-                   forced ? strtof(forced, nullptr) : 0.0f, tg, spec.redone);
+                   forced ? strtof(forced, nullptr) : 0.0f, tg);
     }
     int chunk_no = 0;
     for (int64_t t0 = 0; t0 < (sc ? 0 : ntiles); t0 += chunk_tiles, chunk_no++) {
@@ -823,20 +840,19 @@
     URH_CHECK(urh_center_chain(ctx, d_qad_out, n, ts, max_size, sharded ? ctx->nccl_rank : 0, sharded ? ctx->nccl_world : 1,
                                fine.gh ? &fine : nullptr, &plan));
     const float* d_centerf;
-    const double* d_center;
-    const int* d_state;
-    urh_center_plan_result(ctx, plan, &d_centerf, &d_center, &d_state);
+    urh_center_plan_result(ctx, plan, &d_centerf, nullptr, nullptr);
+    if (speculate) spec.redone = urh_center_plan_redone(plan);
+    double h_center = 0.0;
+    int st = 0;
+    int64_t certified = 0, straddle = 0, redone = 0;
     int64_t rows = 0;
     if (sc) {
-        URH_CUDA(ctx, cudaMemcpyAsync(ctx->h_mail + 40, d_center, sizeof(double), cudaMemcpyDeviceToHost, ctx->stream));
-        URH_CUDA(ctx, cudaMemcpyAsync(ctx->h_mail + 41, d_state, sizeof(int), cudaMemcpyDeviceToHost, ctx->stream));
-        URH_CHECK(urh_center_plan_certify_stats(ctx, plan, ctx->h_mail + 42));
-        URH_CUDA(ctx, cudaMemcpyAsync(ctx->h_mail + 45, (const int64_t*)ctx->center_prefix + ntiles, sizeof(int64_t), cudaMemcpyDeviceToHost,
+        URH_CHECK(urh_center_plan_fetch(ctx, plan, ctx->h_mail + 40));
+        URH_CUDA(ctx, cudaMemcpyAsync(ctx->h_mail + 46, (const int64_t*)ctx->center_prefix + ntiles, sizeof(int64_t), cudaMemcpyDeviceToHost,
                                       ctx->stream));
         URH_CUDA(ctx, cudaStreamSynchronize(ctx->stream));
-        int st0 = 0;
-        memcpy(&st0, ctx->h_mail + 41, sizeof(int));
-        if (st0 == 1) {
+        urh_center_plan_unpack(ctx->h_mail + 40, &h_center, &st, &certified, &straddle, &redone);
+        if (st == 1) {
             StreamDigitizer dz;
             URH_CHECK(dz.init(ctx, n, scs, tol, mod_type == URH_MOD_ASK, samples_per_symbol));
             for (int64_t s0 = 0; s0 < n; s0 += scs) {
@@ -846,7 +862,7 @@
             }
             rows = dz.rows;
         }
-        *sc->kept = ctx->h_mail[45];
+        *sc->kept = ctx->h_mail[46];
     } else {
         URH_CUDA(ctx, cudaMemsetAsync(d_init, 0, 16, ctx->stream));
         const int vec_in = (((uintptr_t)d_qad_out % 8) == 0) ? 1 : 0;
@@ -859,24 +875,19 @@
         }
         URH_LAUNCH(ctx, (k_dense_f32<SrcQad2, float>), (unsigned)grid, URH_WARPS_PER_BLOCK * 32, 0,
                    (const float*)d_qad_out, n, vec_in, cls, tol, tiles, staging, cap, d_init, 0, d_centerf, (const UrhTileStats*)ts, spec);
-        URH_CUDA(ctx, cudaMemcpyAsync(ctx->h_mail + 40, d_center, sizeof(double), cudaMemcpyDeviceToHost, ctx->stream));
-        URH_CUDA(ctx, cudaMemcpyAsync(ctx->h_mail + 41, d_state, sizeof(int), cudaMemcpyDeviceToHost, ctx->stream));
-        URH_CHECK(urh_center_plan_certify_stats(ctx, plan, ctx->h_mail + 42));
-        ctx->h_mail[46] = 0;
-        if (speculate) URH_CUDA(ctx, cudaMemcpyAsync(ctx->h_mail + 46, spec.redone, sizeof(unsigned int), cudaMemcpyDeviceToHost, ctx->stream));
+        URH_CHECK(urh_center_plan_fetch(ctx, plan, ctx->h_mail + 40));
         if (sharded)
             URH_CHECK(urh_finish_shard(ctx, n, tol, mod_type == URH_MOD_ASK, samples_per_symbol, tiles, staging, cap, d_init, global_offset, n_total, &rows));
         else
             URH_CHECK(urh_finish_local(ctx, n, tol, mod_type == URH_MOD_ASK, samples_per_symbol, tiles, staging, cap, d_init, &rows));
     }
-    memcpy(center, ctx->h_mail + 40, sizeof(double));
-    int st = 0;
-    memcpy(&st, ctx->h_mail + 41, sizeof(int));
+    if (!sc) urh_center_plan_unpack(ctx->h_mail + 40, &h_center, &st, &certified, &straddle, &redone);
+    *center = h_center;
     *center_state = st;
-    ctx->center_cert[0] = ctx->h_mail[42];
+    ctx->center_cert[0] = certified;
     ctx->center_cert[1] = fine.gh ? URH_FINE_NB : 0;
-    ctx->center_cert[2] = ctx->h_mail[44];
-    const int64_t redone = (spec.hi > spec.lo) ? ctx->h_mail[46] : 0;
+    ctx->center_cert[2] = straddle;
+    if (!(spec.hi > spec.lo)) redone = 0;
     ctx->spec_stats[0] = spec.hi - spec.lo;
     ctx->spec_stats[1] = spec.hi - spec.lo - redone;
     ctx->spec_stats[2] = redone;
diff --git a/urh_b200/csrc/finish.cu b/urh_b200/csrc/finish.cu
--- a/urh_b200/csrc/finish.cu
+++ b/urh_b200/csrc/finish.cu
@@ -5,55 +5,57 @@
 
 #define CLS_NONE INT_MIN
 
-struct __align__(16) CandAgg {
-    int64_t cnt;
+struct __align__(16) CandFire {
+    int64_t fired;
+    int64_t first_pos;
+    int64_t last_pos;
+    int32_t first_cls;
     int32_t last_cls;
-    int32_t pad;
-};
-struct CandOp {
-    __device__ __forceinline__ CandAgg operator()(const CandAgg& a, const CandAgg& b) const {
-        CandAgg r;
-        r.cnt = a.cnt + b.cnt;
-        r.last_cls = (b.last_cls != CLS_NONE) ? b.last_cls : a.last_cls;
-        r.pad = 0;
+};
+struct CandFireOp {
+    __device__ __forceinline__ CandFire operator()(const CandFire& a, const CandFire& b) const {
+        if (a.first_cls == CLS_NONE) return b;
+        if (b.first_cls == CLS_NONE) return a;
+        const bool j = b.first_cls != a.last_cls;
+        CandFire r;
+        r.fired = a.fired + b.fired + (j ? 1 : 0);
+        r.first_pos = a.first_pos;
+        r.last_pos = (b.last_pos >= 0) ? b.last_pos : (j ? b.first_pos : a.last_pos);
+        r.first_cls = a.first_cls;
+        r.last_cls = b.last_cls;
         return r;
     }
 };
-struct __align__(16) FireAgg {
-    int64_t fired;
-    int64_t last_pos;
-};
-struct FireOp {
-    __device__ __forceinline__ FireAgg operator()(const FireAgg& a, const FireAgg& b) const {
-        FireAgg r;
-        r.fired = a.fired + b.fired;
-        r.last_pos = (b.last_pos >= 0) ? b.last_pos : a.last_pos;
-        return r;
-    }
-};
+__host__ __device__ __forceinline__ CandFire cand_fire_none() {
+    CandFire r;
+    r.fired = 0; r.first_pos = -1; r.last_pos = -1; r.first_cls = CLS_NONE; r.last_cls = CLS_NONE;
+    return r;
+}
+__device__ __forceinline__ void cand_fire_advance(int& cls, int64_t& pos, const CandFire& tot) {
+    if (tot.first_cls == CLS_NONE) return;
+    if (tot.last_pos >= 0) pos = tot.last_pos;
+    else if (tot.first_cls != cls) pos = tot.first_pos;
+    cls = tot.last_cls;
+}
 
 struct ScanRunCarry : TileRuns {
     RunCarry* carry;
     __device__ __forceinline__ void post(int64_t t, const RunCarry& excl, const RunCarry&) const { carry[t] = excl; }
 };
 
-struct __align__(16) TileFire {
-    int32_t first_cls;
-    int32_t first_rel;
-    int32_t fired;
-    int32_t last_rel;
-};
-struct ScanCandidates {
+struct ScanCandFire {
     const UrhTileSummary* tiles;
     const uint32_t* staging;
     int stage_cap;
     const RunCarry* carry;
     const RunCarry* xcarry;
     int tol;
+    int64_t global_offset;
     int32_t* head_rel;
     int32_t* prev_cls;
-    TileFire* fire;
-    __device__ __forceinline__ CandAgg load(int64_t t) const {
+    int64_t* row_off;
+    int64_t* prev_fired;
+    __device__ __forceinline__ CandFire load(int64_t t) const {
         const UrhTileSummary s = tiles[t];
         RunCarry c = carry[t];
         if (xcarry) c = RunCarryOp()(*xcarry, c);
@@ -62,13 +64,11 @@
         int32_t rel = -1;
         if (start_len <= tol && (int64_t)tol < start_len + s.head_len) rel = (int32_t)(tol - start_len);
         head_rel[t] = rel;
-        TileFire f;
-        f.first_cls = CLS_NONE; f.first_rel = -1; f.fired = 0; f.last_rel = -1;
-        int prev = CLS_NONE;
+        int32_t first_rel = -1, last_rel = -1, fired = 0;
+        int first = CLS_NONE, prev = CLS_NONE;
         if (rel >= 0) {
-            prev = s.first_cls;
-            f.first_cls = prev;
-            f.first_rel = rel;
+            first = prev = s.first_cls;
+            first_rel = rel;
         }
         const uint32_t* st = staging + t * (int64_t)stage_cap;
         for (int j = 0; j < s.ncand; j += 4) {
@@ -81,48 +81,27 @@
                     const int cl = (int)(w[u] & 0xffffu) - 1;
                     const int p = (int)(w[u] >> 16);
                     if (prev == CLS_NONE) {
-                        f.first_cls = cl;
-                        f.first_rel = p;
+                        first = cl;
+                        first_rel = p;
                     } else if (cl != prev) {
-                        f.fired++;
-                        f.last_rel = p;
+                        fired++;
+                        last_rel = p;
                     }
                     prev = cl;
                 }
             }
         }
-        fire[t] = f;
-        CandAgg r;
-        r.cnt = (int64_t)s.ncand + (rel >= 0 ? 1 : 0);
+        const int64_t base = t * URH_TILE + global_offset;
+        CandFire r;
+        r.fired = fired;
+        r.first_pos = (first_rel >= 0) ? base + first_rel : -1;
+        r.last_pos = (last_rel >= 0) ? base + last_rel : -1;
+        r.first_cls = first;
         r.last_cls = prev;
-        r.pad = 0;
         return r;
     }
-    __device__ __forceinline__ void post(int64_t t, const CandAgg& excl, const CandAgg&) const { prev_cls[t] = excl.last_cls; }
-};
-
-struct ScanFirings {
-    const TileFire* fire;
-    const int32_t* prev_cls;
-    const int16_t* d_prev0;
-    int64_t global_offset;
-    int64_t* row_off;
-    int64_t* prev_fired;
-    __device__ __forceinline__ FireAgg load(int64_t t) const {
-        const TileFire f = fire[t];
-        int prev = prev_cls[t];
-        if (prev == CLS_NONE) prev = *d_prev0;
-        FireAgg r;
-        r.fired = f.fired;
-        int32_t last = f.last_rel;
-        if (f.first_cls != CLS_NONE && f.first_cls != prev) {
-            r.fired++;
-            if (last < 0) last = f.first_rel;
-        }
-        r.last_pos = (last >= 0) ? t * URH_TILE + global_offset + last : -1;
-        return r;
-    }
-    __device__ __forceinline__ void post(int64_t t, const FireAgg& excl, const FireAgg&) const {
+    __device__ __forceinline__ void post(int64_t t, const CandFire& excl, const CandFire&) const {
+        prev_cls[t] = excl.last_cls;
         row_off[t] = excl.fired;
         prev_fired[t] = excl.last_pos;
     }
@@ -171,6 +150,7 @@
                                                     int stage_cap, const int32_t* __restrict__ head_rel, const int32_t* __restrict__ prev_cls,
                                                     const int16_t* __restrict__ d_prev0, const int64_t* __restrict__ row_off,
                                                     const int64_t* __restrict__ prev_fired, const int64_t* __restrict__ d_xprev_fired,
+                                                    const CandFire* __restrict__ d_tot,
                                                     int64_t ntiles, int64_t global_offset, int64_t n_total, int tol, int is_ask, int64_t sps,
                                                     int emit_tail, int64_t row_base, int64_t* __restrict__ out, int64_t cap_rows,
                                                     int64_t* __restrict__ d_out) {
@@ -187,11 +167,16 @@
         l_first = s.first_cls;
         l_ncand = s.ncand;
         l_rel = head_rel[tl];
-        l_prev = prev_cls[tl];
-        if (l_prev == CLS_NONE) l_prev = *d_prev0;
-        l_idx = row_off[tl];
-        l_pp = prev_fired[tl];
-        if (l_pp < 0) l_pp = *d_xprev_fired;
+        CandFire e;
+        e.fired = row_off[tl];
+        e.first_pos = d_tot->first_pos;
+        e.last_pos = prev_fired[tl];
+        e.last_cls = prev_cls[tl];
+        e.first_cls = (e.last_cls == CLS_NONE) ? CLS_NONE : d_tot->first_cls;
+        l_prev = *d_prev0;
+        l_pp = *d_xprev_fired;
+        if (e.first_cls != CLS_NONE) l_idx = e.fired + (e.first_cls != l_prev ? 1 : 0);
+        cand_fire_advance(l_prev, l_pp, e);
     }
     for (int j0 = 0; j0 < FIN_TILES && t0 + j0 < ntiles; j0 += FIN_BATCH) {
         uint32_t w0[FIN_BATCH];
@@ -286,23 +271,17 @@
     else acc.flags &= ~1;
     *xcarry = acc;
 }
-__global__ void k_fold_prev_cls(const int64_t* __restrict__ all, int rank, const int64_t* __restrict__ stage1, int16_t* __restrict__ prev0) {
-    int v = (int)stage1[2];
+__global__ void k_fold_prev(const int64_t* __restrict__ all, int rank, const int64_t* __restrict__ stage1, int16_t* __restrict__ prev0,
+                            int64_t* __restrict__ xprev) {
+    int cls = (int)stage1[2];
+    int64_t pos = -1;
     for (int q = 0; q < rank; q++) {
-        CandAgg c;
-        memcpy(&c, all + 2 * q, sizeof(c));
-        if (c.last_cls != CLS_NONE) v = c.last_cls;
-    }
-    *prev0 = (int16_t)v;
-}
-__global__ void k_fold_prev_fired(const int64_t* __restrict__ all, int rank, int64_t* __restrict__ xprev) {
-    int64_t v = -1;
-    for (int q = 0; q < rank; q++) {
-        FireAgg c;
-        memcpy(&c, all + 2 * q, sizeof(c));
-        if (c.last_pos >= 0) v = c.last_pos;
-    }
-    *xprev = v;
+        CandFire c;
+        memcpy(&c, all + 4 * q, sizeof(c));
+        cand_fire_advance(cls, pos, c);
+    }
+    *prev0 = (int16_t)cls;
+    *xprev = pos;
 }
 
 __global__ void k_chain_start(const int16_t* __restrict__ d_init, UrhChain* __restrict__ chain) {
@@ -311,11 +290,13 @@
     chain->last_state = INT64_MIN;
     chain->prev_cls = *d_init;
 }
-__global__ void k_chain_advance(UrhChain* __restrict__ chain, const RunCarry* __restrict__ tot_run, const CandAgg* __restrict__ tot_cand,
-                                const FireAgg* __restrict__ tot_fire) {
+__global__ void k_chain_advance(UrhChain* __restrict__ chain, const RunCarry* __restrict__ tot_run, const CandFire* __restrict__ tot_cf) {
     chain->run = RunCarryOp()(chain->run, *tot_run);
-    if (tot_cand->last_cls != CLS_NONE) chain->prev_cls = (int16_t)tot_cand->last_cls;
-    if (tot_fire->last_pos >= 0) chain->prev_fired = tot_fire->last_pos;
+    int cls = chain->prev_cls;
+    int64_t pos = chain->prev_fired;
+    cand_fire_advance(cls, pos, *tot_cf);
+    chain->prev_cls = (int16_t)cls;
+    chain->prev_fired = pos;
 }
 __global__ void k_chain_last_row(UrhChain* __restrict__ chain, const int64_t* __restrict__ table, int64_t rows) {
     if (rows > 0) chain->last_state = table[2 * (rows - 1)];
@@ -343,20 +324,16 @@
     URH_CHECK(urh_arena(ctx, (size_t)ntiles, &prev_cls));
     URH_CHECK(urh_arena(ctx, (size_t)ntiles, &row_off));
     URH_CHECK(urh_arena(ctx, (size_t)ntiles, &prev_fired));
-    TileFire* fire;
-    URH_CHECK(urh_arena(ctx, (size_t)ntiles, &fire));
     URH_CHECK(urh_arena(ctx, (size_t)(32 + 8 * (sharded ? sh.world : 0)), &d_small));
     URH_CUDA(ctx, cudaMemsetAsync(d_small, 0xff, 4 * sizeof(int64_t), ctx->stream));
     RunCarry* d_tot_run = (RunCarry*)(d_small + 4);
-    CandAgg* d_tot_cand = (CandAgg*)(d_small + 6);
-    FireAgg* d_tot_fire = (FireAgg*)(d_small + 8);
-    RunCarry* d_xcarry = (RunCarry*)(d_small + 10);
+    RunCarry* d_xcarry = (RunCarry*)(d_small + 6);
+    CandFire* d_tot_cf = (CandFire*)(d_small + 8);
     int16_t* d_prev0 = (int16_t*)(d_small + 12);
     int64_t* d_xprev = d_small + 13;
     int64_t* d_msg1 = d_small + 16;
     int64_t* d_all1 = d_small + 32;
     int64_t* d_all2 = d_all1 + 4 * (sharded ? sh.world : 0);
-    int64_t* d_all3 = d_all2 + 2 * (sharded ? sh.world : 0);
 
     if (chain && sh.global_offset == 0) URH_LAUNCH(ctx, k_chain_start, 1, 1, 0, d_init, chain);
     RunCarry rc_ident;
@@ -371,33 +348,20 @@
         URH_TL_MARK(ctx, "x4 run carry: done");
         URH_LAUNCH(ctx, k_fold_carry, 1, 1, 0, (const int64_t*)d_all1, sh.rank, d_xcarry);
     }
-    ScanCandidates fb;
+    ScanCandFire fb;
     fb.tiles = tiles; fb.staging = staging; fb.stage_cap = stage_cap; fb.carry = carry;
     fb.xcarry = sharded ? d_xcarry : (chain ? &chain->run : nullptr);
-    fb.tol = tol; fb.head_rel = head_rel; fb.prev_cls = prev_cls; fb.fire = fire;
-    CandAgg ca_ident;
-    ca_ident.cnt = 0; ca_ident.last_cls = CLS_NONE; ca_ident.pad = 0;
-    URH_CHECK((urhts::scan<CandAgg, CandOp, ScanCandidates, 4>(ctx, ntiles, ca_ident, CandOp(), fb, d_tot_cand)));
+    fb.tol = tol; fb.global_offset = sh.global_offset; fb.head_rel = head_rel; fb.prev_cls = prev_cls; fb.row_off = row_off;
+    fb.prev_fired = prev_fired;
+    URH_CHECK((urhts::scan<CandFire, CandFireOp, ScanCandFire, 4>(ctx, ntiles, cand_fire_none(), CandFireOp(), fb, d_tot_cf)));
     const int16_t* prev0 = chain ? &chain->prev_cls : d_init;
+    const int64_t* xprev = chain ? &chain->prev_fired : d_small + 2;
     if (sharded) {
         URH_TL_MARK(ctx, "x5 candidates: enter");
-        URH_CHECK(urh_nccl_allgather(ctx, d_tot_cand, d_all2, sizeof(CandAgg)));
+        URH_CHECK(urh_nccl_allgather(ctx, d_tot_cf, d_all2, sizeof(CandFire)));
         URH_TL_MARK(ctx, "x5 candidates: done");
-        URH_LAUNCH(ctx, k_fold_prev_cls, 1, 1, 0, (const int64_t*)d_all2, sh.rank, (const int64_t*)d_all1, d_prev0);
+        URH_LAUNCH(ctx, k_fold_prev, 1, 1, 0, (const int64_t*)d_all2, sh.rank, (const int64_t*)d_all1, d_prev0, d_xprev);
         prev0 = d_prev0;
-    }
-    ScanFirings fc;
-    fc.fire = fire; fc.prev_cls = prev_cls; fc.d_prev0 = prev0; fc.global_offset = sh.global_offset; fc.row_off = row_off;
-    fc.prev_fired = prev_fired;
-    FireAgg fi_ident;
-    fi_ident.fired = 0; fi_ident.last_pos = -1;
-    URH_CHECK((urhts::scan<FireAgg, FireOp, ScanFirings>(ctx, ntiles, fi_ident, FireOp(), fc, d_tot_fire)));
-    const int64_t* xprev = chain ? &chain->prev_fired : d_small + 2;
-    if (sharded) {
-        URH_TL_MARK(ctx, "x6 firings: enter");
-        URH_CHECK(urh_nccl_allgather(ctx, d_tot_fire, d_all3, sizeof(FireAgg)));
-        URH_TL_MARK(ctx, "x6 firings: done");
-        URH_LAUNCH(ctx, k_fold_prev_fired, 1, 1, 0, (const int64_t*)d_all3, sh.rank, d_xprev);
         xprev = d_xprev;
     }
 
@@ -414,7 +378,7 @@
     int64_t got[2] = {0, 0};
     for (int attempt = 0; attempt < 2; attempt++) {
         URH_LAUNCH(ctx, k_finish_rows, (unsigned)urh_div_up(ntiles, 8 * FIN_TILES), 256, 0, tiles, staging, stage_cap, (const int32_t*)head_rel,
-                   (const int32_t*)prev_cls, prev0, (const int64_t*)row_off, (const int64_t*)prev_fired, xprev, ntiles, sh.global_offset,
+                   (const int32_t*)prev_cls, prev0, (const int64_t*)row_off, (const int64_t*)prev_fired, xprev, (const CandFire*)d_tot_cf, ntiles, sh.global_offset,
                    sh.n_total, tol, is_ask ? 1 : 0, (int64_t)sps, sh.emit_tail, row_base, raw, raw_cap, d_small);
         if (sharded && attempt == 0) URH_TL_MARK(ctx, "rows written");
         URH_CHECK(urh_read_i64(ctx, d_small, 2, got));
@@ -429,7 +393,7 @@
             raw_cap = (int64_t)ctx->pulses_cap_rows;
         }
     }
-    if (chain) URH_LAUNCH(ctx, k_chain_advance, 1, 1, 0, chain, (const RunCarry*)d_tot_run, (const CandAgg*)d_tot_cand, (const FireAgg*)d_tot_fire);
+    if (chain) URH_LAUNCH(ctx, k_chain_advance, 1, 1, 0, chain, (const RunCarry*)d_tot_run, (const CandFire*)d_tot_cf);
     int64_t K = got[0];
     if (is_ask && K > 0) {
         if (!chain) URH_CHECK(urh_ensure_pulses(ctx, (size_t)K));
```

Result: faster. 221,200, median of 6 (+1.3%).
